# JuliaDiffusionBayes/ExtensibleMCMC.jl

Measured on NVIDIA B200. Metric: chain-steps x obs/sec, higher is better.
Workload: dtype f64

## Files before the change

extensiblemcmc.jl_b200/csrc/api.cu:

```cuda
#include <dlfcn.h>
#include <nccl.h>

#include <algorithm>
#include <cmath>
#include <cstdio>
#include <cstdlib>
#include <cstring>
#include <map>
#include <string>
#include <vector>

#include <cuda_runtime.h>

#include "../../include/extmcmc.h"
#include "dev_state.cuh"
#include "block_kernels.h"
#include "step_kernels.h"
#include "sweep.h"
#include "user_law.h"

using namespace extmcmc;

namespace {

std::string g_create_error;

struct NcclApi {
    void *lib = nullptr;
    ncclResult_t (*GetUniqueId)(ncclUniqueId *) = nullptr;
    ncclResult_t (*CommInitRank)(ncclComm_t *, int, ncclUniqueId, int) = nullptr;
    ncclResult_t (*AllReduce)(const void *, void *, size_t, ncclDataType_t, ncclRedOp_t, ncclComm_t,
                              cudaStream_t) = nullptr;
    ncclResult_t (*CommDestroy)(ncclComm_t) = nullptr;
    const char *(*GetErrorString)(ncclResult_t) = nullptr;
    bool load(std::string &err) {
        if (lib) return true;
        lib = dlopen("libnccl.so.2", RTLD_NOW | RTLD_GLOBAL);
        if (!lib) lib = dlopen("libnccl.so", RTLD_NOW | RTLD_GLOBAL);
        if (!lib) { err = std::string("cannot load libnccl: ") + dlerror(); return false; }
        GetUniqueId = (decltype(GetUniqueId))dlsym(lib, "ncclGetUniqueId");
        CommInitRank = (decltype(CommInitRank))dlsym(lib, "ncclCommInitRank");
        AllReduce = (decltype(AllReduce))dlsym(lib, "ncclAllReduce");
        CommDestroy = (decltype(CommDestroy))dlsym(lib, "ncclCommDestroy");
        GetErrorString = (decltype(GetErrorString))dlsym(lib, "ncclGetErrorString");
        if (!GetUniqueId || !CommInitRank || !AllReduce || !CommDestroy) {
            err = "libnccl lacks required symbols";
            return false;
        }
        return true;
    }
} g_nccl;

struct Slot {
    StepDesc *h_descs = nullptr;
    StepDesc *d_descs = nullptr;
    int cap = 0;
    cudaEvent_t done = nullptr;
    bool in_flight = false;
};

}

struct extmcmc_handle {
    extmcmc_config_t cfg{};
    int num_sms = 0;
    size_t l2_bytes = 0;
    cudaStream_t stream = nullptr;
    std::string err;
    DevState d{};
    std::vector<DevUpdate> upd_host;
    std::vector<bool> upd_set;
    bool upd_dirty = true;
    double *obs_dev = nullptr;
    int64_t n_obs_local = 0;
    int64_t n_obs_largest = 0;
    int64_t *goff_dev = nullptr, *glen_dev = nullptr;
    double *y_dev = nullptr;
    UserLaw ulaw;
    int logi_D = 0;
    unsigned int *tail_counter = nullptr;
    bool tail = false;
    bool grad_valid = false;
    bool dcache = false, dc_valid = false;
    double *dsum_buf[2] = {nullptr, nullptr};
    bool any_mala = false;
    bool state_set = false;
    SweepPlan plan{};
    bool plan_valid = false;
    Slot slot[2];
    int next_slot = 0;
    std::map<long long, cudaGraphExec_t> graphs;
    std::map<long long, int64_t> graph_launches;
    int64_t seq_next = 0;
    std::vector<int64_t> ra_iter;
    std::vector<int64_t> acc_tag;
    std::vector<int64_t> haario_M;
    std::vector<double> lambda;
    std::vector<extmcmc_lambda_fn> lambda_fn;
    std::vector<void *> lambda_user;
    int64_t xseq_next = 0;
    bool blk_planned = false;
    bool res_ok = false, obsblk_ok = false;
    TeamPlan res_plan{};
    ObsBlockPlan obsblk_plan{};
    unsigned long long *blk_go = nullptr;
    unsigned int *blk_counter = nullptr;
    unsigned int *team_sync = nullptr;
    long long *team_prof = nullptr;
    size_t team_sync_cap = 0;
    double *rp_prop = nullptr, *rp_exp = nullptr;
    size_t rp_prop_cap = 0, rp_exp_cap = 0;
    std::vector<std::pair<cudaEvent_t, cudaEvent_t>> ev_pending, ev_free;
    float sweep_ms = 0.f;
    int64_t sweep_launches = 0;
    cudaEvent_t t0 = nullptr, t1 = nullptr;
    std::vector<cudaEvent_t> ev_pool;
    int64_t launches = 0;
    double *flush_buf = nullptr;
    int64_t flush_n = 0;
    double *scratch_ll = nullptr;
    double *gsum = nullptr;
    cudaStream_t copy_stream = nullptr;
    cudaEvent_t fetch_ready = nullptr, fetch_done = nullptr;
    unsigned char *stage = nullptr;
    size_t stage_cap = 0;
    int64_t fetch_lo = 0, fetch_hi = 0;
    bool fetch_active = false;
    void *p2p_region = nullptr;
    std::vector<void *> p2p_opened;
    ncclComm_t comm = nullptr;
    int64_t *n_obs_dev = nullptr;
    bool n_total_known = false;
    std::vector<void *> allocs;
};

namespace {

#define CK(h, call)                                                                      \
    do {                                                                                 \
        cudaError_t e_ = (call);                                                         \
        if (e_ != cudaSuccess) {                                                         \
            (h)->err = std::string(#call) + ": " + cudaGetErrorString(e_);               \
            return e_ == cudaErrorMemoryAllocation ? EXTMCMC_EOOM : EXTMCMC_ECUDA;       \
        }                                                                                \
    } while (0)

#define NK(h, call)                                                                      \
    do {                                                                                 \
        ncclResult_t r_ = (call);                                                        \
        if (r_ != ncclSuccess) {                                                         \
            (h)->err = std::string(#call) + ": " +                                       \
                       (g_nccl.GetErrorString ? g_nccl.GetErrorString(r_) : "nccl error"); \
            return EXTMCMC_ENCCL;                                                        \
        }                                                                                \
    } while (0)

int32_t fail(extmcmc_t h, int32_t code, const std::string &msg) {
    if (h) h->err = msg; else g_create_error = msg;
    return code;
}

template <typename T>
int32_t dev_alloc(extmcmc_t h, T **out, size_t n) {
    void *p = nullptr;
    cudaError_t e = cudaMalloc(&p, std::max<size_t>(n, 1) * sizeof(T));
    if (e != cudaSuccess) {
        h->err = std::string("cudaMalloc: ") + cudaGetErrorString(e);
        return EXTMCMC_EOOM;
    }
    h->allocs.push_back(p);
    *out = (T *)p;
    return EXTMCMC_OK;
}

void invalidate_graphs(extmcmc_t h) {
    for (auto &kv : h->graphs) cudaGraphExecDestroy(kv.second);
    h->graphs.clear();
    h->graph_launches.clear();
}

bool obs_sharded(extmcmc_t h) {
    return h->cfg.shard_mode == EXTMCMC_SHARD_OBS && h->cfg.world_size > 1;
}

int32_t ensure_plan(extmcmc_t h) {
    if (h->plan_valid) return EXTMCMC_OK;
    if (h->cfg.law == EXTMCMC_LAW_GSN_IID_1D || h->cfg.law == EXTMCMC_LAW_HIER_NORMAL)
        h->plan = plan_sweep_gsn1d(h->d.C, h->n_obs_largest, h->cfg.sweep_variant, h->num_sms, h->d.G);
    else if (h->cfg.law == EXTMCMC_LAW_GSN_MV)
        h->plan = plan_sweep_gsnmv(h->cfg.obs_dim, h->d.C, h->n_obs_local, h->cfg.sweep_variant, h->num_sms);
    else if (h->cfg.law == EXTMCMC_LAW_LOGISTIC)
        h->plan = plan_sweep_logistic(h->cfg.obs_dim, h->d.C, h->n_obs_local, h->num_sms);
    else if (h->cfg.law == EXTMCMC_LAW_USER) {
        if (!h->ulaw.loaded) return fail(h, EXTMCMC_EINVAL, "no user law: call extmcmc_set_user_law first");
        h->plan = plan_sweep_user(h->ulaw, h->d.C, h->n_obs_local, h->cfg.sweep_variant, h->num_sms);
    } else
        return fail(h, EXTMCMC_EUNSUPPORTED, "law not implemented on the GPU path");
    h->d.S = h->plan.S;
    h->tail = h->cfg.law == EXTMCMC_LAW_GSN_IID_1D && h->plan.variant == SWEEP_VARIANT_OBS;
    if (const char *e = getenv("EXTMCMC_TAIL")) h->tail = h->tail && atoi(e) != 0;
    if (h->tail && !h->tail_counter) {
        int32_t rct = dev_alloc(h, &h->tail_counter, 1);
        if (rct) return rct;
        CK(h, cudaMemset(h->tail_counter, 0, sizeof(unsigned int)));
    }
    h->d.use_ssum = (obs_sharded(h) || law_self_finished(h->cfg.law) || h->tail) ? 1 : 0;
    size_t part_rows = law_self_finished(h->cfg.law) ? (size_t)h->plan.S * (h->cfg.n_params + 1)
                                                     : (size_t)2 * h->d.G * h->plan.S;
    part_rows = std::max(part_rows, (size_t)h->num_sms * 3);
    part_rows = std::max(part_rows, (size_t)2 * h->d.G * 4);
    int32_t rc = dev_alloc(h, &h->d.partial, part_rows * h->d.C);
    if (rc) return rc;
    if (obs_sharded(h) && !h->gsum &&
        (h->cfg.law == EXTMCMC_LAW_GSN_IID_1D || h->cfg.law == EXTMCMC_LAW_HIER_NORMAL))
        if ((rc = dev_alloc(h, &h->gsum, (size_t)2 * h->d.G * h->d.C))) return rc;
    {
        const char *e = getenv("EXTMCMC_DATA_CACHE");
        const bool on = !e || atoi(e) != 0;
        h->dcache = on && h->cfg.law == EXTMCMC_LAW_HIER_NORMAL && !obs_sharded(h) && h->d.G <= kDataCacheMaxG;
        if (h->dcache && !h->dsum_buf[0])
            if ((rc = dev_alloc(h, &h->dsum_buf[0], (size_t)2 * h->d.G * h->d.C)) ||
                (rc = dev_alloc(h, &h->dsum_buf[1], (size_t)2 * h->d.G * h->d.C)))
                return rc;
        h->d.dsum_cur = h->dcache ? h->dsum_buf[0] : nullptr;
        h->d.dsum_prop = h->dcache ? h->dsum_buf[1] : nullptr;
        h->dc_valid = false;
    }
    h->plan_valid = true;
    h->blk_planned = false;
    invalidate_graphs(h);
    return EXTMCMC_OK;
}

constexpr int kDataFree = 0x100;
int step_kind(extmcmc_t h, int u) {
    const DevUpdate &t = h->upd_host[u];
    int kind = t.kernel;
    if (h->dcache && kind != EXTMCMC_KERNEL_MALA && t.n_coords <= kMaxCoords) {
        bool moves_data = false;
        for (int i = 0; i < t.n_coords; ++i) moves_data = moves_data || t.coords[i] < h->d.G;
        if (!moves_data) kind |= kDataFree;
    }
    return kind;
}
inline bool kind_is_mala(int kind) { return (kind & 0xff) == EXTMCMC_KERNEL_MALA; }
int step_advance(bool dcache, int kind, bool &gv, bool &dc) {
    if (kind_is_mala(kind)) {
        const int mode = gv ? 0 : (dc ? 2 : 1);
        if (mode == 1 && dcache) dc = true;
        gv = true;
        return mode;
    }
    gv = false;
    if (kind & kDataFree) {
        const int mode = dc ? 1 : 2;
        dc = true;
        return mode;
    }
    dc = false;
    return 0;
}

int32_t plan_block_kernels(extmcmc_t h) {
    if (h->blk_planned) return EXTMCMC_OK;
    h->blk_planned = true;
    h->res_ok = h->obsblk_ok = false;
    const int sv = h->cfg.sweep_variant;
    if (sv != 0 && sv != 3 && sv != 4) return EXTMCMC_OK;
    if (const char *e = getenv("EXTMCMC_BLOCK_KERNELS")) if (atoi(e) == 0) return EXTMCMC_OK;
    const bool gsn1d = h->cfg.law == EXTMCMC_LAW_GSN_IID_1D || h->cfg.law == EXTMCMC_LAW_HIER_NORMAL;
    if (!gsn1d || h->d.n_haario > 0) return EXTMCMC_OK;
    bool all_unif = true, all_unif_or_mala = true;
    for (int u = 0; u < h->cfg.n_updates; ++u) {
        const int kk = h->upd_host[u].kernel;
        if (kk != EXTMCMC_KERNEL_RW_UNIFORM) all_unif = false;
        if (kk != EXTMCMC_KERNEL_RW_UNIFORM && kk != EXTMCMC_KERNEL_MALA) all_unif_or_mala = false;
    }
    if (all_unif_or_mala && !obs_sharded(h) && sv == 3) {
        h->res_ok = plan_team(h->d, h->upd_host.data(), h->num_sms, true, &h->res_plan);
        if (h->res_ok && getenv("EXTMCMC_TEAM_PROF") && !h->team_prof) {
            int32_t rc = dev_alloc(h, &h->team_prof, (size_t)h->res_plan.n_cta * 8);
            if (rc) return rc;
            CK(h, cudaMemset(h->team_prof, 0, sizeof(long long) * h->res_plan.n_cta * 8));
        }
        if (h->res_ok) {
            const size_t words = team_sync_words(h->res_plan);
            if (words > h->team_sync_cap) {
                int32_t rc = dev_alloc(h, &h->team_sync, words);
                if (rc) return rc;
                h->team_sync_cap = words;
            }
        }
    }
    const bool obs_auto = false;
    if (!h->res_ok && all_unif && h->cfg.law == EXTMCMC_LAW_GSN_IID_1D && h->d.C <= 32 && (sv == 4 || obs_auto) &&
        (!obs_sharded(h) || h->d.p2p)) {
        cudaError_t e = plan_obs_block(h->d, h->upd_host.data(), h->num_sms, h->n_obs_local, &h->obsblk_plan);
        if (e == cudaSuccess) {
            if (!h->blk_go) {
                int32_t rc;
                if ((rc = dev_alloc(h, &h->blk_go, 1)) || (rc = dev_alloc(h, &h->blk_counter, 1))) return rc;
                CK(h, cudaMemset(h->blk_go, 0, sizeof(unsigned long long)));
                CK(h, cudaMemset(h->blk_counter, 0, sizeof(unsigned int)));
            }
            h->obsblk_ok = true;
        } else {
            cudaGetLastError();
        }
    }
    return EXTMCMC_OK;
}

int32_t upload_updates(extmcmc_t h) {
    if (!h->upd_dirty) return EXTMCMC_OK;
    CK(h, cudaMemcpyAsync(h->d.upd, h->upd_host.data(), sizeof(DevUpdate) * h->upd_host.size(),
                          cudaMemcpyHostToDevice, h->stream));
    CK(h, cudaStreamSynchronize(h->stream));
    h->upd_dirty = false;
    return EXTMCMC_OK;
}

int32_t ensure_total_obs(extmcmc_t h) {
    if (h->n_total_known) return EXTMCMC_OK;
    if (h->cfg.shard_mode == EXTMCMC_SHARD_OBS && h->cfg.world_size > 1) {
        if (!h->comm) return fail(h, EXTMCMC_EINVAL, "EXTMCMC_SHARD_OBS needs extmcmc_comm_init first");
        int64_t n = h->n_obs_local;
        CK(h, cudaMemcpyAsync(h->n_obs_dev, &n, sizeof n, cudaMemcpyHostToDevice, h->stream));
        NK(h, g_nccl.AllReduce(h->n_obs_dev, h->n_obs_dev, 1, ncclInt64, ncclSum, h->comm, h->stream));
        CK(h, cudaMemcpyAsync(&n, h->n_obs_dev, sizeof n, cudaMemcpyDeviceToHost, h->stream));
        CK(h, cudaStreamSynchronize(h->stream));
        h->d.n_obs_total = n;
    } else {
        h->d.n_obs_total = h->n_obs_local;
    }
    h->n_total_known = true;
    invalidate_graphs(h);
    return EXTMCMC_OK;
}

int32_t enqueue_sweep(extmcmc_t h, bool instrument, bool grad = false, const double *src = nullptr,
                      double *ll_dst = nullptr, double *grad_dst = nullptr,
                      const StepDesc *d_descs = nullptr, int k = 0) {
    std::pair<cudaEvent_t, cudaEvent_t> ev{nullptr, nullptr};
    bool tail_done = false;
    if (instrument) {
        if (!h->ev_free.empty()) { ev = h->ev_free.back(); h->ev_free.pop_back(); }
        else { CK(h, cudaEventCreate(&ev.first)); CK(h, cudaEventCreate(&ev.second)); }
        CK(h, cudaEventRecord(ev.first, h->stream));
    }
    if (h->cfg.law == EXTMCMC_LAW_GSN_IID_1D || h->cfg.law == EXTMCMC_LAW_HIER_NORMAL) {
        Gsn1dArgs a{};
        a.obs = h->obs_dev; a.goff = h->goff_dev; a.glen = h->glen_dev; a.G = h->d.G;
        a.mu = h->cfg.law == EXTMCMC_LAW_HIER_NORMAL ? src : h->d.lawc;
        if (!a.mu) return fail(h, EXTMCMC_EINVAL, "internal: sweep without a source state");
        a.C = h->d.C; a.partial = h->d.partial; a.S = h->plan.S;
        tail_done = h->tail && !grad;
        if (tail_done) {
            const bool push = obs_sharded(h) && h->d.p2p && d_descs;
            a.tail_mode = push ? 2 : 1;
            a.tail_counter = h->tail_counter; a.ssum = h->d.ssum;
            a.peer_rx = h->d.peer_rx;
            a.rank = h->cfg.rank; a.world = h->cfg.world_size;
            a.descs = d_descs; a.k = k;
        }
        static const bool hint_on = [] { const char *e = getenv("EXTMCMC_L2_HINT"); return !e || atoi(e) != 0; }();
        a.stream_hint = hint_on && (size_t)h->n_obs_local * sizeof(double) > h->l2_bytes / 2 ? 1 : 0;
        launch_sweep_gsn1d(h->plan, a, grad, h->stream);
    } else if (h->cfg.law == EXTMCMC_LAW_LOGISTIC) {
        LogisticArgs a{h->obs_dev, h->y_dev, h->n_obs_local, src, h->cfg.obs_dim, h->d.C, h->d.partial,
                       h->d.partial + (size_t)h->plan.S * h->d.C, h->plan.S, h->plan.n_cta};
        launch_sweep_logistic(h->plan, a, ll_dst, grad_dst, h->stream);
        if (obs_sharded(h)) {
            NK(h, g_nccl.AllReduce(ll_dst, ll_dst, (size_t)h->d.C, ncclFloat64, ncclSum, h->comm, h->stream));
            if (grad_dst)
                NK(h, g_nccl.AllReduce(grad_dst, grad_dst, (size_t)h->cfg.obs_dim * h->d.C, ncclFloat64, ncclSum,
                                       h->comm, h->stream));
        }
        h->launches += h->plan.launches;
        if (instrument) {
            CK(h, cudaEventRecord(ev.second, h->stream));
            h->ev_pending.push_back(ev);
        }
        return EXTMCMC_OK;
    } else if (h->cfg.law == EXTMCMC_LAW_USER) {
        UserSweepArgs a{};
        a.obs = h->obs_dev; a.n_obs = h->n_obs_local; a.theta = src; a.C = h->d.C;
        a.ll_part = h->d.partial; a.g_part = h->d.partial + (size_t)h->plan.S * h->d.C;
        a.err_flag = h->d.err_flag; a.S = h->plan.S;
        CK(h, launch_sweep_user(h->plan, h->ulaw, a, grad, ll_dst, grad_dst, h->stream));
        h->launches += h->plan.launches;
        if (instrument) {
            CK(h, cudaEventRecord(ev.second, h->stream));
            h->ev_pending.push_back(ev);
        }
        return EXTMCMC_OK;
    } else {
        launch_sweep_gsnmv(h->plan, h->obs_dev, h->n_obs_local, h->d.lawc, h->d.C, h->d.partial, h->stream);
    }
    h->launches += h->plan.launches;
    if (instrument) {
        CK(h, cudaEventRecord(ev.second, h->stream));
        h->ev_pending.push_back(ev);
    }
    if (obs_sharded(h) && grad) {
        launch_reduce_group_sums(h->d, h->gsum, h->stream);
        h->launches += 1;
        NK(h, g_nccl.AllReduce(h->gsum, h->gsum, (size_t)2 * h->d.G * h->d.C, ncclFloat64, ncclSum, h->comm,
                               h->stream));
    } else if (obs_sharded(h)) {
        if (h->d.p2p && d_descs) {
            if (!tail_done) { launch_reduce_push(h->d, d_descs, k, h->stream); h->launches += 1; }
        } else {
            if (!tail_done) { launch_reduce_partials(h->d, h->stream); h->launches += 1; }
            NK(h, g_nccl.AllReduce(h->d.ssum, h->d.ssum, (size_t)h->d.C, ncclFloat64, ncclSum, h->comm,
                                   h->stream));
        }
    }
    return EXTMCMC_OK;
}

DevState grad_view(extmcmc_t h) {
    DevState v = h->d;
    if (obs_sharded(h) && !law_self_finished(h->cfg.law)) { v.partial = h->gsum; v.S = 1; }
    return v;
}

int32_t enqueue_steps(extmcmc_t h, const StepDesc *d_descs, const int *kinds, int n_steps,
                      bool instrument, bool &grad_valid, bool &dc_valid) {
    bool fused = false;
    bool cur_prepared = false;
    for (int k = 0; k < n_steps; ++k) {
        int32_t rc;
        const int dflags = step_deferral_flags(h->d, k, n_steps);
        const bool next_mala = k + 1 < n_steps && kind_is_mala(kinds[k + 1]);
        const bool next_rw = k + 1 < n_steps && !kind_is_mala(kinds[k + 1]);
        const int mode = step_advance(h->dcache, kinds[k], grad_valid, dc_valid);
        if (kind_is_mala(kinds[k])) {
            const bool logi = law_self_finished(h->cfg.law);
            int finalize_cur = 0;
            DevState gv = grad_view(h);
            if (mode == 1) {
                if (logi) {
                    if ((rc = enqueue_sweep(h, instrument, true, h->d.theta, h->scratch_ll, h->d.grad_cur))) return rc;
                } else {
                    const bool hier = h->cfg.law == EXTMCMC_LAW_HIER_NORMAL;
                    if (!cur_prepared && !hier) { launch_prepare_current(h->d, h->stream); h->launches += 1; }
                    if ((rc = enqueue_sweep(h, instrument, true, h->d.theta))) return rc;
                    finalize_cur = 1;
                }
            } else if (mode == 2) {
                gv.partial = h->d.dsum_cur; gv.S = 1;
                finalize_cur = 2;
            }
            launch_mala_propose(gv, d_descs, k, finalize_cur, h->scratch_ll, dflags, h->stream);
            gv = grad_view(h);
            if (logi) {
                if ((rc = enqueue_sweep(h, instrument, true, h->d.prop_full, h->d.ll_prop, h->d.grad_prop))) return rc;
            } else {
                if ((rc = enqueue_sweep(h, instrument, true, h->d.prop_full))) return rc;
            }
            fused = next_rw;
            launch_mala_accept(gv, d_descs, k, logi ? 0 : 1, fused ? 1 : 0, dflags, h->stream);
            h->launches += 2;
            cur_prepared = false;
        } else {
            if (!fused) { launch_propose(h->d, d_descs, k, h->stream); h->launches += 1; }
            const bool from_cache = mode != 0;
            if (mode == 2) {
                if ((rc = enqueue_sweep(h, instrument, true, h->d.theta))) return rc;
                launch_reduce_group_sums(h->d, h->d.dsum_cur, h->stream);
                h->launches += 1;
            }
            if (!from_cache)
                if ((rc = enqueue_sweep(h, instrument, false, h->d.prop_full, h->d.ssum, nullptr, d_descs, k))) return rc;
            fused = next_rw;
            cur_prepared = next_mala && !law_self_finished(h->cfg.law) && h->cfg.law != EXTMCMC_LAW_HIER_NORMAL;
            launch_accept(h->d, d_descs, k, fused ? 1 : (cur_prepared ? 2 : 0), dflags, h->stream, from_cache);
            h->launches += 1;
        }
    }
    CK(h, cudaGetLastError());
    return EXTMCMC_OK;
}

int32_t collect_events(extmcmc_t h) {
    for (auto &ev : h->ev_pending) {
        float ms = 0.f;
        CK(h, cudaEventElapsedTime(&ms, ev.first, ev.second));
        h->sweep_ms += ms;
        h->sweep_launches += 1;
        h->ev_free.push_back(ev);
    }
    h->ev_pending.clear();
    return EXTMCMC_OK;
}

int32_t run_block_impl(extmcmc_t h, const extmcmc_step_t *steps, int32_t n_steps, int rng_mode,
                       int32_t p_u_max, const double *proposals, const double *exp_draws) {
    if (!h) return EXTMCMC_EINVAL;
    if (n_steps < 0 || (n_steps > 0 && !steps)) return fail(h, EXTMCMC_EINVAL, "bad steps");
    if (n_steps == 0) return EXTMCMC_OK;
    if (!h->obs_dev) return fail(h, EXTMCMC_EINVAL, "no observations uploaded");
    if (!h->state_set) return fail(h, EXTMCMC_EINVAL, "extmcmc_set_state not called");
    for (int u = 0; u < h->cfg.n_updates; ++u)
        if (!h->upd_set[u]) return fail(h, EXTMCMC_EINVAL, "update " + std::to_string(u) + " not set");
    if (n_steps > h->cfg.history_window)
        return fail(h, EXTMCMC_EINVAL, "block longer than history_window");
    if (obs_sharded(h) && !h->comm) return fail(h, EXTMCMC_EINVAL, "EXTMCMC_SHARD_OBS needs extmcmc_comm_init first");
    if (h->cfg.law == EXTMCMC_LAW_USER && h->any_mala && h->ulaw.loaded && !h->ulaw.grad)
        return fail(h, EXTMCMC_EUNSUPPORTED, "MALA needs a user law with logpdf_grad (extmcmc_set_user_law with_grad = 1)");
    for (int s = 0; s < n_steps; ++s)
        if (steps[s].pidx < 0 || steps[s].pidx >= h->cfg.n_updates || steps[s].mcmciter < 1)
            return fail(h, EXTMCMC_EINVAL, "step out of range");
    CK(h, cudaSetDevice(h->cfg.device));
    int32_t rc;
    if ((rc = ensure_plan(h))) return rc;
    if ((rc = upload_updates(h))) return rc;
    if ((rc = ensure_total_obs(h))) return rc;
    if ((rc = plan_block_kernels(h))) return rc;
    if ((h->res_ok || h->obsblk_ok) && h->dcache) {
        h->dcache = h->dc_valid = false;
        h->d.dsum_cur = h->d.dsum_prop = nullptr;
    }
    if (h->fetch_active && h->seq_next + n_steps - h->d.H > h->fetch_lo)
        CK(h, cudaStreamWaitEvent(h->stream, h->fetch_done, 0));

    if (h->d.rng_mode != rng_mode) { h->d.rng_mode = rng_mode; invalidate_graphs(h); }
    if (rng_mode == EXTMCMC_RNG_REPLAY) {
        if (!proposals || !exp_draws || p_u_max < 1) return fail(h, EXTMCMC_EINVAL, "replay buffers missing");
        for (int s = 0; s < n_steps; ++s)
            if (h->upd_host[steps[s].pidx].n_coords > p_u_max)
                return fail(h, EXTMCMC_EINVAL, "p_u_max smaller than an update's n_coords");
        const size_t np = (size_t)n_steps * p_u_max * h->d.C, ne = (size_t)n_steps * h->d.C;
        CK(h, cudaStreamSynchronize(h->stream));
        if (np > h->rp_prop_cap) {
            if (h->rp_prop) cudaFree(h->rp_prop);
            CK(h, cudaMalloc(&h->rp_prop, np * sizeof(double)));
            h->rp_prop_cap = np;
        }
        if (ne > h->rp_exp_cap) {
            if (h->rp_exp) cudaFree(h->rp_exp);
            CK(h, cudaMalloc(&h->rp_exp, ne * sizeof(double)));
            h->rp_exp_cap = ne;
        }
        CK(h, cudaMemcpy(h->rp_prop, proposals, np * sizeof(double), cudaMemcpyHostToDevice));
        CK(h, cudaMemcpy(h->rp_exp, exp_draws, ne * sizeof(double), cudaMemcpyHostToDevice));
        h->d.rp_prop = h->rp_prop;
        h->d.rp_exp = h->rp_exp;
        h->d.p_u_max = p_u_max;
    }

    const int si = h->next_slot;
    Slot &sl = h->slot[si];
    h->next_slot ^= 1;
    if (sl.in_flight) { CK(h, cudaEventSynchronize(sl.done)); sl.in_flight = false; }
    if (sl.cap < n_steps) {
        if (sl.h_descs) cudaFreeHost(sl.h_descs);
        if (sl.d_descs) cudaFree(sl.d_descs);
        for (auto it = h->graphs.begin(); it != h->graphs.end();) {
            if ((it->first & 1) == si) { cudaGraphExecDestroy(it->second); it = h->graphs.erase(it); }
            else ++it;
        }
        const int cap = std::max(n_steps, 64);
        CK(h, cudaMallocHost(&sl.h_descs, sizeof(StepDesc) * cap));
        CK(h, cudaMalloc(&sl.d_descs, sizeof(StepDesc) * cap));
        sl.cap = cap;
    }
    const int W = h->d.W;
    int n_sweeps = 0;
    {
        bool gv = h->grad_valid, dc = h->dc_valid;
        for (int s = 0; s < n_steps; ++s) {
            StepDesc &sd = sl.h_descs[s];
            const int u = steps[s].pidx;
            const int64_t it = steps[s].mcmciter;
            sd.mcmciter = it;
            sd.seq = h->seq_next + s;
            sd.stat_n = sd.seq + 1;
            sd.xseq = h->xseq_next + s;
            sd.pidx = u;
            sd.first = steps[s].prev_pidx < 0 ? 1 : 0;
            const int64_t prev_it = it - 1 > 1 ? it - 1 : 1;
            sd.ra_prev_valid = (h->ra_iter[u] == prev_it && prev_it != it) ? 1 : 0;
            int64_t &tag = h->acc_tag[(size_t)u * W + (size_t)(it % W)];
            sd.acc_out_valid = (it > W && tag == it - W) ? 1 : 0;
            sd.replay_row = s;
            sd.haario_ready = 0;
            sd.lambda = h->lambda[u];
            sd.pad_ = 0;
            if (h->upd_host[u].adapt_kind == EXTMCMC_ADAPT_HAARIO) {
                if (++h->haario_M[u] >= h->upd_host[u].adapt_every_k) {
                    sd.haario_ready = 1;
                    h->haario_M[u] = 0;
                    if (h->lambda_fn[u]) h->lambda[u] = h->lambda_fn[u](h->lambda[u], sd.stat_n + 1, it, h->lambda_user[u]);
                }
            }
            const bool mala = h->upd_host[u].kernel == EXTMCMC_KERNEL_MALA;
            sd.need_cur_grad = (mala && !gv) ? 1 : 0;
            const int mode = step_advance(h->dcache, step_kind(h, u), gv, dc);
            n_sweeps += mala ? 1 + (mode == 1 ? 1 : 0) : (mode == 1 ? 0 : 1);
            h->ra_iter[u] = it;
            tag = it;
        }
    }

    std::vector<int> kinds(n_steps);
    unsigned long long hash = 1469598103934665603ull;
    for (int s = 0; s < n_steps; ++s) {
        kinds[s] = step_kind(h, steps[s].pidx);
        hash = (hash ^ (unsigned long long)kinds[s]) * 1099511628211ull;
    }
    hash = (hash ^ (unsigned long long)((h->grad_valid ? 7 : 3) + (h->dc_valid ? 16 : 0))) * 1099511628211ull;
    hash = (hash ^ (unsigned long long)n_steps) * 1099511628211ull;
    const bool instrument = h->cfg.instrument != 0;
    const bool use_graph = h->cfg.use_graphs && !instrument && rng_mode == EXTMCMC_RNG_PHILOX;
    if (h->res_ok || h->obsblk_ok) {
        CK(h, cudaMemcpyAsync(sl.d_descs, sl.h_descs, sizeof(StepDesc) * n_steps, cudaMemcpyHostToDevice, h->stream));
        std::pair<cudaEvent_t, cudaEvent_t> ev{nullptr, nullptr};
        if (instrument) {
            if (!h->ev_free.empty()) { ev = h->ev_free.back(); h->ev_free.pop_back(); }
            else { CK(h, cudaEventCreate(&ev.first)); CK(h, cudaEventCreate(&ev.second)); }
        }
        if (h->res_ok) {
            TeamArgs a{};
            a.d = h->d;
            a.d.dsum_cur = a.d.dsum_prop = nullptr;
            a.d.S = h->res_plan.ts;
            a.descs = sl.d_descs; a.n_steps = n_steps; a.n_sweeps = n_sweeps;
            a.obs = h->obs_dev; a.goff = h->goff_dev; a.glen = h->glen_dev; a.G = h->d.G;
            a.ll_scratch = h->scratch_ll;
            a.sync = h->team_sync;
            a.prof = h->team_prof;
            CK(h, cudaMemsetAsync(h->team_sync, 0, team_sync_words(h->res_plan) * sizeof(unsigned int), h->stream));
            if (instrument) CK(h, cudaEventRecord(ev.first, h->stream));
            CK(h, launch_team_block(h->res_plan, a, h->stream));
            h->launches += 1;
        } else {
            ObsBlockArgs a{};
            a.d = h->d;
            a.d.dsum_cur = a.d.dsum_prop = nullptr;
            a.descs = sl.d_descs; a.n_steps = n_steps;
            a.obs = h->obs_dev; a.n_obs = h->n_obs_local;
            a.go = h->blk_go; a.counter = h->blk_counter;
            if (instrument) CK(h, cudaEventRecord(ev.first, h->stream));
            CK(h, launch_obs_block(h->obsblk_plan, a, h->stream));
            h->launches += 1;
        }
        if (instrument) {
            CK(h, cudaEventRecord(ev.second, h->stream));
            h->ev_pending.push_back(ev);
        }
        h->grad_valid = kind_is_mala(kinds[n_steps - 1]);
        h->dc_valid = false;
    } else if (!use_graph) {
        CK(h, cudaMemcpyAsync(sl.d_descs, sl.h_descs, sizeof(StepDesc) * n_steps,
                              cudaMemcpyHostToDevice, h->stream));
        if ((rc = enqueue_steps(h, sl.d_descs, kinds.data(), n_steps, instrument, h->grad_valid, h->dc_valid))) return rc;
    } else {
        const long long key = (long long)((hash << 1) | (unsigned long long)si);
        auto it = h->graphs.find(key);
        if (it == h->graphs.end()) {
            const int64_t launches_before = h->launches;
            bool gv = h->grad_valid, dc = h->dc_valid;
            cudaGraph_t g = nullptr;
            CK(h, cudaStreamBeginCapture(h->stream, cudaStreamCaptureModeThreadLocal));
            cudaError_t e1 = cudaMemcpyAsync(sl.d_descs, sl.h_descs, sizeof(StepDesc) * n_steps,
                                             cudaMemcpyHostToDevice, h->stream);
            int32_t rc2 = e1 == cudaSuccess ? enqueue_steps(h, sl.d_descs, kinds.data(), n_steps, false, gv, dc) : EXTMCMC_ECUDA;
            cudaError_t e2 = cudaStreamEndCapture(h->stream, &g);
            h->graph_launches[key] = h->launches - launches_before;
            h->launches = launches_before;
            if (rc2 || e2 != cudaSuccess || !g) {
                if (g) cudaGraphDestroy(g);
                return fail(h, EXTMCMC_ECUDA, "CUDA graph capture failed: " + h->err);
            }
            cudaGraphExec_t ge = nullptr;
            cudaError_t e3 = cudaGraphInstantiate(&ge, g, 0);
            cudaGraphDestroy(g);
            if (e3 != cudaSuccess)
                return fail(h, EXTMCMC_ECUDA, std::string("cudaGraphInstantiate: ") + cudaGetErrorString(e3));
            it = h->graphs.emplace(key, ge).first;
        }
        CK(h, cudaGraphLaunch(it->second, h->stream));
        h->launches += h->graph_launches[key];
        for (int s = 0; s < n_steps; ++s) step_advance(h->dcache, kinds[s], h->grad_valid, h->dc_valid);
    }
    CK(h, cudaEventRecord(sl.done, h->stream));
    sl.in_flight = true;
    h->seq_next += n_steps;
    h->xseq_next += n_steps;
    return EXTMCMC_OK;
}

}

extern "C" {

int32_t extmcmc_abi_version(void) { return EXTMCMC_ABI_VERSION; }

const char *extmcmc_last_error(extmcmc_t h) { return h ? h->err.c_str() : g_create_error.c_str(); }

int32_t extmcmc_create(const extmcmc_config_t *cfg, extmcmc_t *out) {
    if (!cfg || !out) return fail(nullptr, EXTMCMC_EINVAL, "null argument");
    *out = nullptr;
    if (cfg->abi_version != EXTMCMC_ABI_VERSION) return fail(nullptr, EXTMCMC_EINVAL, "ABI version mismatch");
    if (cfg->n_chains < 1 || cfg->n_params < 1 || cfg->n_updates < 1 || cfg->history_window < 1)
        return fail(nullptr, EXTMCMC_EINVAL, "n_chains, n_params, n_updates, history_window must be >= 1");
    if (cfg->n_updates > 65535) return fail(nullptr, EXTMCMC_EINVAL, "n_updates must be < 65536");
    switch (cfg->law) {
    case EXTMCMC_LAW_GSN_IID_1D:
        if (cfg->obs_dim != 1 || cfg->n_params != 2)
            return fail(nullptr, EXTMCMC_EINVAL, "GSN_IID_1D needs obs_dim = 1, n_params = 2");
        break;
    case EXTMCMC_LAW_GSN_MV:
        if (cfg->obs_dim < 2 || cfg->obs_dim > kMaxObsDim)
            return fail(nullptr, EXTMCMC_EUNSUPPORTED, "GSN_MV on the GPU path needs 2 <= obs_dim <= 16 (d = 1: GSN_IID_1D)");
        if (cfg->n_params != cfg->obs_dim * (cfg->obs_dim + 1))
            return fail(nullptr, EXTMCMC_EINVAL, "GSN_MV needs n_params = d (d + 1)");
        break;
    case EXTMCMC_LAW_LOGISTIC:
        if (cfg->obs_dim != cfg->n_params || cfg->obs_dim < 1 || logistic_padded_dim(cfg->obs_dim) == 0)
            return fail(nullptr, EXTMCMC_EUNSUPPORTED, "LOGISTIC needs obs_dim = n_params = d with 1 <= d <= 256");
        break;
    case EXTMCMC_LAW_HIER_NORMAL:
        if (cfg->obs_dim != 1 || cfg->n_params < 3)
            return fail(nullptr, EXTMCMC_EINVAL, "HIER_NORMAL needs obs_dim = 1 and n_params = G + 2 >= 3");
        break;
    case EXTMCMC_LAW_USER:
        if (cfg->obs_dim < 1 || cfg->obs_dim > kUserMaxObsDim || cfg->n_params > kUserMaxParams)
            return fail(nullptr, EXTMCMC_EUNSUPPORTED, "USER needs 1 <= obs_dim <= 64 and 1 <= n_params <= 64");
        if (cfg->shard_mode == EXTMCMC_SHARD_OBS && cfg->world_size > 1)
            return fail(nullptr, EXTMCMC_EUNSUPPORTED, "user laws are not implemented under EXTMCMC_SHARD_OBS with several ranks");
        break;
    default:
        return fail(nullptr, EXTMCMC_EUNSUPPORTED, "target law not implemented on the GPU path");
    }
    if (cfg->stats_mode < 0 || cfg->stats_mode > 2) return fail(nullptr, EXTMCMC_EINVAL, "bad stats_mode");
    int ndev = 0;
    cudaError_t e = cudaGetDeviceCount(&ndev);
    if (e != cudaSuccess || ndev == 0)
        return fail(nullptr, EXTMCMC_ECUDA,
                    std::string("no CUDA device: ") + (e != cudaSuccess ? cudaGetErrorString(e) : "count = 0"));
    if (cfg->device < 0 || cfg->device >= ndev) return fail(nullptr, EXTMCMC_EINVAL, "bad device ordinal");

    extmcmc_handle *h = new extmcmc_handle();
    h->cfg = *cfg;
    auto bail = [&](int32_t rc) { g_create_error = h->err; extmcmc_destroy(h); return rc; };
#define CKC(call)                                                                        \
    do {                                                                                 \
        cudaError_t e_ = (call);                                                         \
        if (e_ != cudaSuccess) {                                                         \
            h->err = std::string(#call) + ": " + cudaGetErrorString(e_);                 \
            return bail(e_ == cudaErrorMemoryAllocation ? EXTMCMC_EOOM : EXTMCMC_ECUDA); \
        }                                                                                \
    } while (0)
    CKC(cudaSetDevice(cfg->device));
    cudaDeviceProp prop;
    CKC(cudaGetDeviceProperties(&prop, cfg->device));
    if (prop.major != 10) {
        h->err = "libextmcmc_cuda is built for sm_100a (B200) only; found sm_" +
                 std::to_string(prop.major) + std::to_string(prop.minor);
        return bail(EXTMCMC_EUNSUPPORTED);
    }
    h->num_sms = prop.multiProcessorCount;
    h->l2_bytes = (size_t)prop.l2CacheSize;
    CKC(cudaStreamCreateWithFlags(&h->stream, cudaStreamNonBlocking));
    CKC(cudaStreamCreateWithFlags(&h->copy_stream, cudaStreamNonBlocking));
    CKC(cudaEventCreateWithFlags(&h->fetch_ready, cudaEventDisableTiming));
    CKC(cudaEventCreateWithFlags(&h->fetch_done, cudaEventDisableTiming));
    CKC(cudaEventCreate(&h->t0));
    CKC(cudaEventCreate(&h->t1));
    for (auto &sl : h->slot) CKC(cudaEventCreateWithFlags(&sl.done, cudaEventDisableTiming));
    CKC(sweep_gsn1d_init());
    CKC(sweep_logistic_init());
    h->logi_D = cfg->law == EXTMCMC_LAW_LOGISTIC ? logistic_padded_dim(cfg->obs_dim) : 0;

    DevState &d = h->d;
    const int64_t C = cfg->n_chains;
    const int p = cfg->n_params, NU = cfg->n_updates;
    d.C = C; d.gC = C; d.g0 = 0; d.chain_offset = cfg->chain_offset; d.p = p; d.NU = NU;
    d.W = cfg->roll_window > 0 ? cfg->roll_window : 100;
    d.H = cfg->history_window;
    d.law = cfg->law; d.stats_mode = cfg->stats_mode; d.rng_mode = EXTMCMC_RNG_PHILOX;
    d.p_u_max = 1; d.seed = cfg->seed;
    d.obs_dim = cfg->obs_dim;
    d.G = cfg->law == EXTMCMC_LAW_HIER_NORMAL ? cfg->n_params - 2 : 1;
    d.lawc_k = cfg->law == EXTMCMC_LAW_GSN_IID_1D ? 3
             : law_self_finished(cfg->law) ? 1
             : cfg->law == EXTMCMC_LAW_HIER_NORMAL ? d.G
             : cfg->obs_dim + cfg->obs_dim * (cfg->obs_dim + 1) / 2 + 1;
    d.use_ssum = ((cfg->shard_mode == EXTMCMC_SHARD_OBS && cfg->world_size > 1) ||
                  law_self_finished(cfg->law)) ? 1 : 0;
    int32_t rc = 0;
    const size_t covn = cfg->stats_mode == 0 ? (size_t)p * p : (cfg->stats_mode == 1 ? (size_t)p : 0);
    if ((rc = dev_alloc(h, &d.theta, (size_t)p * C)) || (rc = dev_alloc(h, &d.ll, (size_t)C)) ||
        (rc = dev_alloc(h, &d.prop_loc, (size_t)kMaxCoords * C)) ||
        (rc = dev_alloc(h, &d.prop_full, (size_t)p * C)) ||
        (rc = dev_alloc(h, &d.lawc, (size_t)d.lawc_k * C)) ||
        (rc = dev_alloc(h, &d.n_used, (size_t)C)) || (rc = dev_alloc(h, &d.ssum, (size_t)C)) ||
        (rc = dev_alloc(h, &d.ll_prop, (size_t)C)) || (rc = dev_alloc(h, &d.grad_cur, (size_t)p * C)) ||
        (rc = dev_alloc(h, &d.grad_prop, (size_t)p * C)) ||
        (rc = dev_alloc(h, &h->goff_dev, (size_t)d.G)) || (rc = dev_alloc(h, &h->glen_dev, (size_t)d.G)) ||
        (rc = dev_alloc(h, &d.mean, (size_t)p * C)) || (rc = dev_alloc(h, &d.cov, covn * C)) ||
        (rc = dev_alloc(h, &d.h_theta, (size_t)d.H * p * C)) ||
        (rc = dev_alloc(h, &d.h_prop, (size_t)d.H * p * C)) ||
        (rc = dev_alloc(h, &d.h_ll, (size_t)d.H * C)) || (rc = dev_alloc(h, &d.h_llp, (size_t)d.H * C)) ||
        (rc = dev_alloc(h, &d.h_acc, (size_t)d.H * C)) || (rc = dev_alloc(h, &d.err_flag, 1)) ||
        (rc = dev_alloc(h, &d.upd, (size_t)NU)) || (rc = dev_alloc(h, &h->scratch_ll, (size_t)C)) ||
        (rc = dev_alloc(h, &h->n_obs_dev, 1)))
        return bail(rc);
    CKC(cudaMemset(d.err_flag, 0, sizeof(int32_t)));
    h->upd_host.assign(NU, DevUpdate{});
    h->upd_set.assign(NU, false);
    h->ra_iter.assign(NU, 0);
    h->acc_tag.assign((size_t)NU * d.W, 0);
    h->haario_M.assign(NU, 0);
    h->lambda.assign(NU, 0.0);
    h->lambda_fn.assign(NU, nullptr);
    h->lambda_user.assign(NU, nullptr);
    if (cfg->law == EXTMCMC_LAW_GSN_MV && (rc = dev_alloc(h, &d.mv_L, (size_t)cfg->obs_dim * cfg->obs_dim * C)))
        return bail(rc);
    {
        const char *e = getenv("EXTMCMC_P2P_TIMEOUT_MS");
        const double ms = e ? atof(e) : 30000.0;
        d.p2p_timeout_ns = (unsigned long long)((ms > 1.0 ? ms : 1.0) * 1e6);
    }
    *out = h;
    return EXTMCMC_OK;
#undef CKC
}

int32_t extmcmc_destroy(extmcmc_t h) {
    if (!h) return EXTMCMC_OK;
    cudaSetDevice(h->cfg.device);
    if (h->stream) cudaStreamSynchronize(h->stream);
    if (h->team_prof) {
        const int n = h->res_plan.n_cta;
        std::vector<long long> pr((size_t)n * 8);
        if (cudaMemcpy(pr.data(), h->team_prof, pr.size() * sizeof(long long), cudaMemcpyDeviceToHost) == cudaSuccess) {
            double s[7] = {0, 0, 0, 0, 0, 0, 0}, runs = 0, mx = 0, mn = 1e300;
            for (int b = 0; b < n; ++b) {
                double tot = 0;
                for (int i = 0; i < 7; ++i) { s[i] += (double)pr[(size_t)b * 8 + i]; tot += (double)pr[(size_t)b * 8 + i]; }
                runs += (double)pr[(size_t)b * 8 + 7];
                if (pr[(size_t)b * 8 + 7]) { const double t = tot / pr[(size_t)b * 8 + 7]; mx = std::max(mx, t); mn = std::min(mn, t); }
            }
            if (runs > 0)
                fprintf(stderr, "[extmcmc team kernel] cycles per launch per CTA: sweep %.0f, barrier-before %.0f, barrier-after %.0f, "
                                "propose %.0f, accept %.0f, cov+sync %.0f, ctx %.0f; total min %.0f max %.0f over CTAs; %d CTAs, ts %d, stages %d\n",
                        s[0] / runs, s[1] / runs, s[2] / runs, s[3] / runs, s[4] / runs, s[5] / runs, s[6] / runs, mn, mx, n,
                        h->res_plan.ts, h->res_plan.stages);
        }
    }
    invalidate_graphs(h);
    if (h->comm && g_nccl.CommDestroy) g_nccl.CommDestroy(h->comm);
    for (void *p : h->p2p_opened) cudaIpcCloseMemHandle(p);
    if (h->p2p_region) cudaFree(h->p2p_region);
    for (void *p : h->allocs) cudaFree(p);
    if (h->obs_dev) cudaFree(h->obs_dev);
    if (h->y_dev) cudaFree(h->y_dev);
    user_law_unload(h->ulaw);
    if (h->rp_prop) cudaFree(h->rp_prop);
    if (h->rp_exp) cudaFree(h->rp_exp);
    if (h->flush_buf) cudaFree(h->flush_buf);
    for (auto &sl : h->slot) {
        if (sl.h_descs) cudaFreeHost(sl.h_descs);
        if (sl.d_descs) cudaFree(sl.d_descs);
        if (sl.done) cudaEventDestroy(sl.done);
    }
    for (auto &ev : h->ev_pending) { cudaEventDestroy(ev.first); cudaEventDestroy(ev.second); }
    for (auto &ev : h->ev_free) { cudaEventDestroy(ev.first); cudaEventDestroy(ev.second); }
    if (h->t0) cudaEventDestroy(h->t0);
    if (h->t1) cudaEventDestroy(h->t1);
    for (cudaEvent_t e : h->ev_pool) if (e) cudaEventDestroy(e);
    if (h->copy_stream) { cudaStreamSynchronize(h->copy_stream); cudaStreamDestroy(h->copy_stream); }
    if (h->fetch_ready) cudaEventDestroy(h->fetch_ready);
    if (h->fetch_done) cudaEventDestroy(h->fetch_done);
    if (h->stage) cudaFreeHost(h->stage);
    if (h->stream) cudaStreamDestroy(h->stream);
    delete h;
    return EXTMCMC_OK;
}

static int32_t install_obs(extmcmc_t h, int64_t n_obs, const std::vector<int64_t> &glen) {
    if (h->obs_dev) { cudaFree(h->obs_dev); h->obs_dev = nullptr; }
    const int G = (int)glen.size();
    std::vector<int64_t> goff(G);
    int64_t tot = 0, largest = 0;
    for (int g = 0; g < G; ++g) {
        goff[g] = tot;
        tot += (glen[g] * h->cfg.obs_dim + 1) & ~(int64_t)1;
        largest = std::max(largest, glen[g]);
    }
    const size_t padded = (size_t)tot + 2;
    CK(h, cudaMalloc(&h->obs_dev, padded * sizeof(double)));
    CK(h, cudaMemsetAsync(h->obs_dev, 0, padded * sizeof(double), h->stream));
    CK(h, cudaMemcpyAsync(h->goff_dev, goff.data(), sizeof(int64_t) * G, cudaMemcpyHostToDevice, h->stream));
    CK(h, cudaMemcpyAsync(h->glen_dev, glen.data(), sizeof(int64_t) * G, cudaMemcpyHostToDevice, h->stream));
    CK(h, cudaStreamSynchronize(h->stream));
    h->n_obs_local = n_obs;
    h->n_obs_largest = largest;
    h->plan_valid = false;
    h->n_total_known = false;
    h->grad_valid = false;
    h->dc_valid = false;
    return EXTMCMC_OK;
}

int32_t extmcmc_upload_obs(extmcmc_t h, const double *obs, int64_t n_obs, int32_t obs_dim,
                           const double *y) {
    if (!h) return EXTMCMC_EINVAL;
    if (!obs || n_obs < 1) return fail(h, EXTMCMC_EINVAL, "need at least one observation");
    if (obs_dim != h->cfg.obs_dim) return fail(h, EXTMCMC_EINVAL, "obs_dim differs from the configuration");
    CK(h, cudaSetDevice(h->cfg.device));
    CK(h, cudaStreamSynchronize(h->stream));
    if (h->cfg.law == EXTMCMC_LAW_LOGISTIC) {
        if (!y) return fail(h, EXTMCMC_EINVAL, "LOGISTIC needs the responses y");
        const int D = h->logi_D;
        const size_t n_pad = ((size_t)n_obs + 15) & ~(size_t)15;
        if (h->obs_dev) { cudaFree(h->obs_dev); h->obs_dev = nullptr; }
        if (h->y_dev) { cudaFree(h->y_dev); h->y_dev = nullptr; }
        CK(h, cudaMalloc(&h->obs_dev, n_pad * D * sizeof(double)));
        CK(h, cudaMalloc(&h->y_dev, n_pad * sizeof(double)));
        CK(h, cudaMemsetAsync(h->obs_dev, 0, n_pad * D * sizeof(double), h->stream));
        CK(h, cudaMemsetAsync(h->y_dev, 0, n_pad * sizeof(double), h->stream));
        CK(h, cudaMemcpy2DAsync(h->obs_dev, (size_t)D * 8, obs, (size_t)obs_dim * 8, (size_t)obs_dim * 8,
                                (size_t)n_obs, cudaMemcpyHostToDevice, h->stream));
        CK(h, cudaMemcpyAsync(h->y_dev, y, (size_t)n_obs * sizeof(double), cudaMemcpyHostToDevice, h->stream));
        CK(h, cudaStreamSynchronize(h->stream));
        h->n_obs_local = n_obs;
        h->n_obs_largest = n_obs;
        h->plan_valid = false;
        h->n_total_known = false;
        h->grad_valid = false;
        h->dc_valid = false;
        return EXTMCMC_OK;
    }
    if (h->cfg.law == EXTMCMC_LAW_USER) {
        if (y) return fail(h, EXTMCMC_EINVAL, "USER takes no y: responses and covariates are columns of the rows");
        const size_t n_pad = ((size_t)n_obs + 1) & ~(size_t)1, nd = (size_t)n_obs * obs_dim;
        if (h->obs_dev) { cudaFree(h->obs_dev); h->obs_dev = nullptr; }
        CK(h, cudaMalloc(&h->obs_dev, n_pad * obs_dim * sizeof(double)));
        CK(h, cudaMemsetAsync(h->obs_dev, 0, n_pad * obs_dim * sizeof(double), h->stream));
        CK(h, cudaMemcpyAsync(h->obs_dev, obs, nd * sizeof(double), cudaMemcpyHostToDevice, h->stream));
        CK(h, cudaStreamSynchronize(h->stream));
        h->n_obs_local = n_obs;
        h->n_obs_largest = n_obs;
        h->plan_valid = false;
        h->n_total_known = false;
        h->grad_valid = false;
        h->dc_valid = false;
        return EXTMCMC_OK;
    }
    std::vector<int64_t> glen(h->d.G, 0);
    if (h->cfg.law == EXTMCMC_LAW_HIER_NORMAL) {
        if (!y) return fail(h, EXTMCMC_EINVAL, "HIER_NORMAL needs the group index of every observation in y");
        int64_t prev = 0;
        for (int64_t i = 0; i < n_obs; ++i) {
            const int64_t g = (int64_t)y[i];
            if (g < prev || g >= h->d.G || (double)g != y[i])
                return fail(h, EXTMCMC_EINVAL, "group indices must be integers in [0, G), sorted ascending");
            prev = g;
            ++glen[g];
        }
    } else {
        glen[0] = n_obs;
    }
    int32_t rc = install_obs(h, n_obs, glen);
    if (rc) return rc;
    int64_t src = 0, dst = 0;
    for (int g = 0; g < h->d.G; ++g) {
        const int64_t nd = glen[g] * obs_dim;
        if (nd) CK(h, cudaMemcpyAsync(h->obs_dev + dst, obs + src, (size_t)nd * sizeof(double), cudaMemcpyHostToDevice, h->stream));
        src += nd;
        dst += (nd + 1) & ~(int64_t)1;
    }
    CK(h, cudaStreamSynchronize(h->stream));
    return EXTMCMC_OK;
}

int32_t extmcmc_generate_obs_normal(extmcmc_t h, int64_t first, int64_t n_obs, double mean, double sd,
                                    uint64_t seed) {
    if (!h) return EXTMCMC_EINVAL;
    if (n_obs < 1 || first < 0 || !(sd > 0.0)) return fail(h, EXTMCMC_EINVAL, "bad generate_obs arguments");
    if (h->cfg.law != EXTMCMC_LAW_GSN_IID_1D) return fail(h, EXTMCMC_EUNSUPPORTED, "generate_obs_normal needs the GSN_IID_1D law");
    CK(h, cudaSetDevice(h->cfg.device));
    CK(h, cudaStreamSynchronize(h->stream));
    int32_t rc = install_obs(h, n_obs, std::vector<int64_t>{n_obs});
    if (rc) return rc;
    launch_generate_obs_normal(h->obs_dev, first, n_obs, mean, sd, seed, h->num_sms, h->stream);
    h->launches += 1;
    CK(h, cudaGetLastError());
    CK(h, cudaStreamSynchronize(h->stream));
    return EXTMCMC_OK;
}

static int32_t ensure_gw_scratch(extmcmc_t h, int n) {
    if (n <= h->d.gw_n) return EXTMCMC_OK;
    CK(h, cudaStreamSynchronize(h->stream));
    double *p = nullptr;
    int32_t rc = dev_alloc(h, &p, (size_t)3 * n * h->d.C);
    if (rc) return rc;
    h->d.gw = p;
    h->d.gw_n = n;
    invalidate_graphs(h);
    return EXTMCMC_OK;
}

int32_t extmcmc_set_update(extmcmc_t h, int32_t u, const extmcmc_update_t *upd) {
    if (!h || !upd) return EXTMCMC_EINVAL;
    if (u < 0 || u >= h->cfg.n_updates) return fail(h, EXTMCMC_EINVAL, "update index out of range");
    const bool gauss = upd->kernel == EXTMCMC_KERNEL_RW_GAUSS || upd->kernel == EXTMCMC_KERNEL_RW_GAUSS_MIX;
    const bool mala = upd->kernel == EXTMCMC_KERNEL_MALA;
    const bool mix = upd->kernel == EXTMCMC_KERNEL_RW_GAUSS_MIX;
    const bool haario = upd->adapt.kind == EXTMCMC_ADAPT_HAARIO;
    if (upd->kernel != EXTMCMC_KERNEL_RW_UNIFORM && !gauss && !mala)
        return fail(h, EXTMCMC_EUNSUPPORTED, "transition kernel not implemented on the GPU path");
    if (mala) {
        if (h->cfg.law != EXTMCMC_LAW_GSN_IID_1D && h->cfg.law != EXTMCMC_LAW_HIER_NORMAL &&
            h->cfg.law != EXTMCMC_LAW_LOGISTIC && h->cfg.law != EXTMCMC_LAW_USER)
            return fail(h, EXTMCMC_EUNSUPPORTED, "MALA needs a law with a device gradient (GSN_IID_1D, HIER_NORMAL, LOGISTIC, USER)");
        if (h->cfg.law == EXTMCMC_LAW_USER && h->ulaw.loaded && !h->ulaw.grad)
            return fail(h, EXTMCMC_EUNSUPPORTED, "MALA needs a user law with logpdf_grad (extmcmc_set_user_law with_grad = 1)");
        if (upd->prior != EXTMCMC_PRIOR_IMPROPER && upd->prior != EXTMCMC_PRIOR_NORMAL)
            return fail(h, EXTMCMC_EUNSUPPORTED, "MALA supports ImproperPrior and Normal priors only");
        if (upd->pos)
            for (int i = 0; i < upd->n_coords; ++i)
                if (upd->pos[i]) return fail(h, EXTMCMC_EUNSUPPORTED, "MALA on positivity-constrained coordinates is not implemented");
    }
    if (upd->prior < EXTMCMC_PRIOR_IMPROPER || upd->prior > EXTMCMC_PRIOR_MVNORMAL)
        return fail(h, EXTMCMC_EUNSUPPORTED, "prior not implemented on the GPU path");
    if (upd->n_coords < 1 || upd->n_coords > (mala ? std::min(h->cfg.n_params, 32768) : kMaxCoords))
        return fail(h, EXTMCMC_EUNSUPPORTED, mala ? "1 <= n_coords <= min(n_params, 32768) for MALA"
                                                  : "1 <= n_coords <= 32 for random-walk updates on the GPU path");
    if (!upd->coords || !upd->step) return fail(h, EXTMCMC_EINVAL, "coords/step missing");
    const int nc = upd->n_coords, nn = nc * nc;
    if (upd->prior == EXTMCMC_PRIOR_PRODUCT) {
        if (upd->n_prior_params < 1 || !upd->prior_params) return fail(h, EXTMCMC_EINVAL, "ProductPrior parameters missing");
        const int K = (int)upd->prior_params[0];
        if (K < 1 || K > kMaxPriorFactors || upd->n_prior_params != 1 + 4 * K)
            return fail(h, EXTMCMC_EUNSUPPORTED, "ProductPrior: 1 <= factors <= 16");
        int tot = 0;
        for (int k = 0; k < K; ++k) {
            const int kind = (int)upd->prior_params[1 + 4 * k], dim = (int)upd->prior_params[2 + 4 * k];
            if (kind < EXTMCMC_PRIOR_IMPROPER || kind > EXTMCMC_PRIOR_CAUCHY || kind == EXTMCMC_PRIOR_PRODUCT || dim < 1)
                return fail(h, EXTMCMC_EUNSUPPORTED, "ProductPrior factor not implemented on the GPU path");
            tot += dim;
        }
        if (tot != nc) return fail(h, EXTMCMC_EINVAL, "ProductPrior dims must add up to length(coords)");
    } else if (upd->prior == EXTMCMC_PRIOR_MVNORMAL) {
        if (upd->n_prior_params != nc + nn || !upd->prior_params)
            return fail(h, EXTMCMC_EINVAL, "MvNormal prior needs {mu[p_u], L[p_u * p_u]}");
        for (int i = 0; i < nc; ++i)
            if (!(upd->prior_params[nc + i + i * nc] > 0.0))
                return fail(h, EXTMCMC_EINVAL, "MvNormal prior: the Cholesky factor must have a positive diagonal");
    } else {
        if (upd->n_prior_params > kMaxPriorParams || (upd->n_prior_params > 0 && !upd->prior_params))
            return fail(h, EXTMCMC_EINVAL, "bad prior parameters");
        const int pk = upd->prior;
        const int need = (pk == EXTMCMC_PRIOR_IMPROPER || pk == EXTMCMC_PRIOR_IMPROPER_POS) ? 0
                       : pk == EXTMCMC_PRIOR_EXPONENTIAL ? 1 : 2;
        if (upd->n_prior_params < need) return fail(h, EXTMCMC_EINVAL, "prior parameters missing");
    }
    if (!(upd->adapt.kind == EXTMCMC_ADAPT_NONE ||
          (upd->adapt.kind == EXTMCMC_ADAPT_MALA && mala) ||
          (upd->adapt.kind == EXTMCMC_ADAPT_UNIF_RW && upd->kernel == EXTMCMC_KERNEL_RW_UNIFORM) ||
          (upd->adapt.kind == EXTMCMC_ADAPT_HAARIO && mix)))
        return fail(h, EXTMCMC_EUNSUPPORTED, "adaptation not implemented for this transition kernel");
    if (upd->adapt.kind != EXTMCMC_ADAPT_NONE && upd->adapt.adapt_every_k_steps < 1)
        return fail(h, EXTMCMC_EINVAL, "adapt_every_k_steps must be >= 1");
    for (int i = 0; i < nc; ++i) {
        if (upd->coords[i] < 0 || upd->coords[i] >= h->cfg.n_params)
            return fail(h, EXTMCMC_EINVAL, "coordinate out of range");
        if (!gauss && !mala && !(upd->step[i] > 0.0))
            return fail(h, EXTMCMC_EINVAL, "eps must be > 0");
    }
    if (mix && !(upd->step[2 * nn] >= 0.0 && upd->step[2 * nn] <= 1.0))
        return fail(h, EXTMCMC_EINVAL, "lambda must be in [0, 1]");
    if (mala && !(upd->step[0] > 0.0)) return fail(h, EXTMCMC_EINVAL, "MALA step tau must be > 0");
    const bool fresh = !h->upd_set[u];
    {
        const DevUpdate &cur = h->upd_host[u];
        if (!fresh && cur.n_coords != nc) return fail(h, EXTMCMC_EINVAL, "cannot change n_coords of an update");
        if (!fresh && ((mix && !cur.sigB) || (gauss && !cur.sigA) || (haario && !cur.hmean) ||
                       (upd->prior == EXTMCMC_PRIOR_MVNORMAL && !cur.prior_dev)))
            return fail(h, EXTMCMC_EINVAL, "cannot change the kernel or prior family of an update");
    }

    CK(h, cudaSetDevice(h->cfg.device));
    const int64_t C = h->d.C;
    const int W = h->d.W;
    DevUpdate t = h->upd_host[u];
    t.kernel = upd->kernel; t.n_coords = nc; t.prior = upd->prior;
    t.adapt_kind = upd->adapt.kind;
    for (int i = 0; i < nc && i < kMaxCoords; ++i) {
        t.coords[i] = upd->coords[i];
        t.pos[i] = upd->pos ? upd->pos[i] : 0;
    }
    const bool mvn = upd->prior == EXTMCMC_PRIOR_MVNORMAL;
    for (int i = 0; i < kMaxPriorParams; ++i)
        t.prior_params[i] = (!mvn && i < upd->n_prior_params) ? upd->prior_params[i] : 0.0;
    t.adapt_every_k = upd->adapt.adapt_every_k_steps;
    t.target = upd->adapt.target_accpt_rate; t.scale = upd->adapt.scale;
    t.vmin = upd->adapt.min; t.vmax = upd->adapt.max; t.offset = upd->adapt.offset;
    int32_t rc = 0;
    if (fresh) {
        double *pd = nullptr;
        if ((rc = dev_alloc(h, &t.coords_dev, (size_t)nc)) ||
            (rc = dev_alloc(h, &t.eps, (size_t)nc * C)) ||
            (rc = dev_alloc(h, &t.adapt_prop, (size_t)C)) || (rc = dev_alloc(h, &t.adapt_acc, (size_t)C)) ||
            (rc = dev_alloc(h, &t.tot_prop, (size_t)C)) || (rc = dev_alloc(h, &t.tot_acc, (size_t)C)) ||
            (rc = dev_alloc(h, &t.ra_val, (size_t)C)) || (rc = dev_alloc(h, &t.acc_ring, (size_t)W * C)))
            return rc;
        if (gauss && ((rc = dev_alloc(h, &t.sigA, (size_t)nn)) || (rc = dev_alloc(h, &t.LA, (size_t)nn)))) return rc;
        if (mix && ((rc = dev_alloc(h, &t.sigB, (size_t)nn * C)) || (rc = dev_alloc(h, &t.LB, (size_t)nn * C)))) return rc;
        if (haario && ((rc = dev_alloc(h, &t.hmean, (size_t)nc * C)) || (rc = dev_alloc(h, &t.hcov, (size_t)nn * C)))) return rc;
        if (mvn) { if ((rc = dev_alloc(h, &pd, (size_t)(nc + nn)))) return rc; t.prior_dev = pd; }
    }
    if ((gauss || haario || mvn) && (rc = ensure_gw_scratch(h, nc))) return rc;
    CK(h, cudaStreamSynchronize(h->stream));
    CK(h, cudaMemcpy(t.coords_dev, upd->coords, sizeof(int32_t) * nc, cudaMemcpyHostToDevice));
    if (mvn) CK(h, cudaMemcpy(const_cast<double *>(t.prior_dev), upd->prior_params, sizeof(double) * (nc + nn), cudaMemcpyHostToDevice));
    if (mala) {
        std::vector<double> tau0((size_t)C, upd->step[0]);
        CK(h, cudaMemcpy(t.eps, tau0.data(), tau0.size() * sizeof(double), cudaMemcpyHostToDevice));
    } else if (!gauss) {
        std::vector<double> eps0((size_t)nc * C);
        for (int i = 0; i < nc; ++i) std::fill_n(eps0.begin() + (size_t)i * C, C, upd->step[i]);
        CK(h, cudaMemcpy(t.eps, eps0.data(), eps0.size() * sizeof(double), cudaMemcpyHostToDevice));
    } else {
        CK(h, cudaMemcpy(t.sigA, upd->step, sizeof(double) * nn, cudaMemcpyHostToDevice));
        launch_chol_factor(t.sigA, t.LA, nc, 1, 1, h->stream);
        if (mix) {
            std::vector<double> sb((size_t)nn * C);
            for (int k = 0; k < nn; ++k) std::fill_n(sb.begin() + (size_t)k * C, C, upd->step[nn + k]);
            CK(h, cudaMemcpy(t.sigB, sb.data(), sb.size() * sizeof(double), cudaMemcpyHostToDevice));
            launch_chol_factor(t.sigB, t.LB, nc, C, C, h->stream);
        }
        CK(h, cudaGetLastError());
        CK(h, cudaStreamSynchronize(h->stream));
        if (haario) {
            CK(h, cudaMemset(t.hmean, 0, sizeof(double) * nc * C));
            CK(h, cudaMemset(t.hcov, 0, sizeof(double) * nn * C));
        }
    }
    CK(h, cudaMemset(t.adapt_prop, 0, sizeof(int32_t) * C));
    CK(h, cudaMemset(t.adapt_acc, 0, sizeof(int32_t) * C));
    CK(h, cudaMemset(t.tot_prop, 0, sizeof(int64_t) * C));
    CK(h, cudaMemset(t.tot_acc, 0, sizeof(int64_t) * C));
    CK(h, cudaMemset(t.ra_val, 0, sizeof(double) * C));
    CK(h, cudaMemset(t.acc_ring, 0, (size_t)W * C));
    h->upd_host[u] = t;
    h->lambda[u] = mix ? upd->step[2 * nn] : 0.0;
    h->haario_M[u] = 0;
    h->upd_set[u] = true;
    h->upd_dirty = true;
    h->blk_planned = false;
    int nh = 0;
    h->any_mala = false;
    for (int v = 0; v < h->cfg.n_updates; ++v) {
        if (h->upd_set[v] && h->upd_host[v].kernel == EXTMCMC_KERNEL_MALA) h->any_mala = true;
        if (h->upd_set[v] && h->upd_host[v].adapt_kind == EXTMCMC_ADAPT_HAARIO) ++nh;
    }
    if (nh != h->d.n_haario) { h->d.n_haario = nh; invalidate_graphs(h); }
    static const bool lean_on = [] { const char *e = getenv("EXTMCMC_LEAN"); return !e || atoi(e) != 0; }();
    int lean = lean_on ? 1 : 0;
    for (int v = 0; v < h->cfg.n_updates; ++v) {
        if (!h->upd_set[v]) continue;
        const DevUpdate &w = h->upd_host[v];
        if ((w.kernel != EXTMCMC_KERNEL_RW_UNIFORM && w.kernel != EXTMCMC_KERNEL_MALA) || !lean_prior(w.prior) ||
            w.adapt_kind == EXTMCMC_ADAPT_HAARIO)
            lean = 0;
    }
    if (lean != h->d.lean) { h->d.lean = lean; invalidate_graphs(h); }
    return EXTMCMC_OK;
}

int32_t extmcmc_set_seed(extmcmc_t h, uint64_t seed) {
    if (!h) return EXTMCMC_EINVAL;
    h->cfg.seed = seed;
    h->d.seed = seed;
    invalidate_graphs(h);
    return EXTMCMC_OK;
}

int32_t extmcmc_set_lambda_fn(extmcmc_t h, int32_t u, extmcmc_lambda_fn f, void *user) {
    if (!h) return EXTMCMC_EINVAL;
    if (u < 0 || u >= h->cfg.n_updates) return fail(h, EXTMCMC_EINVAL, "update index out of range");
    h->lambda_fn[u] = f;
    h->lambda_user[u] = user;
    return EXTMCMC_OK;
}

int32_t extmcmc_set_state(extmcmc_t h, const double *theta) {
    if (!h || !theta) return EXTMCMC_EINVAL;
    CK(h, cudaSetDevice(h->cfg.device));
    CK(h, cudaStreamSynchronize(h->stream));
    const DevState &d = h->d;
    const int64_t C = d.C;
    CK(h, cudaMemcpy(d.theta, theta, sizeof(double) * d.p * C, cudaMemcpyHostToDevice));
    std::vector<double> ninf((size_t)C, -INFINITY);
    CK(h, cudaMemcpy(d.ll, ninf.data(), sizeof(double) * C, cudaMemcpyHostToDevice));
    CK(h, cudaMemset(d.mean, 0, sizeof(double) * d.p * C));
    const size_t covn = d.stats_mode == 0 ? (size_t)d.p * d.p : (d.stats_mode == 1 ? (size_t)d.p : 0);
    if (covn) CK(h, cudaMemset(d.cov, 0, sizeof(double) * covn * C));
    CK(h, cudaMemset(d.err_flag, 0, sizeof(int32_t)));
    for (int u = 0; u < h->cfg.n_updates; ++u) {
        if (!h->upd_set[u]) continue;
        DevUpdate &t = h->upd_host[u];
        CK(h, cudaMemset(t.adapt_prop, 0, sizeof(int32_t) * C));
        CK(h, cudaMemset(t.adapt_acc, 0, sizeof(int32_t) * C));
        CK(h, cudaMemset(t.tot_prop, 0, sizeof(int64_t) * C));
        CK(h, cudaMemset(t.tot_acc, 0, sizeof(int64_t) * C));
        CK(h, cudaMemset(t.ra_val, 0, sizeof(double) * C));
        CK(h, cudaMemset(t.acc_ring, 0, (size_t)d.W * C));
        if (t.hmean) {
            CK(h, cudaMemset(t.hmean, 0, sizeof(double) * t.n_coords * C));
            CK(h, cudaMemset(t.hcov, 0, sizeof(double) * t.n_coords * t.n_coords * C));
        }
    }
    std::fill(h->haario_M.begin(), h->haario_M.end(), 0);
    h->seq_next = 0;
    h->grad_valid = false;
    h->dc_valid = false;
    if (h->fetch_active) { cudaEventSynchronize(h->fetch_done); h->fetch_active = false; }
    std::fill(h->ra_iter.begin(), h->ra_iter.end(), 0);
    std::fill(h->acc_tag.begin(), h->acc_tag.end(), 0);
    h->state_set = true;
    return EXTMCMC_OK;
}

int32_t extmcmc_user_law_check(const char *source, int32_t n_params, int32_t obs_dim, int32_t with_grad,
                               char *log, int64_t log_bytes) {
    if (log && log_bytes > 0) log[0] = 0;
    if (!source) return fail(nullptr, EXTMCMC_EINVAL, "null source");
    if (n_params < 1 || n_params > kUserMaxParams || obs_dim < 1 || obs_dim > kUserMaxObsDim)
        return fail(nullptr, EXTMCMC_EUNSUPPORTED, "user laws need 1 <= n_params <= 64 and 1 <= obs_dim <= 64");
    std::string lg, cubin;
    const int32_t rc = user_law_compile(source, n_params, obs_dim, with_grad != 0, lg, cubin, nullptr);
    if (log && log_bytes > 0) {
        const size_t n = std::min(lg.size(), (size_t)log_bytes - 1);
        std::memcpy(log, lg.data(), n);
        log[n] = 0;
    }
    if (rc) g_create_error = lg;
    return rc;
}

int32_t extmcmc_set_user_law(extmcmc_t h, const char *source, int32_t with_grad) {
    if (!h) return EXTMCMC_EINVAL;
    if (h->cfg.law != EXTMCMC_LAW_USER) return fail(h, EXTMCMC_EINVAL, "extmcmc_set_user_law needs a handle of law EXTMCMC_LAW_USER");
    if (!source) return fail(h, EXTMCMC_EINVAL, "null source");
    std::string log, cubin;
    uint64_t hash = 0;
    const int32_t rc = user_law_compile(source, h->cfg.n_params, h->cfg.obs_dim, with_grad != 0, log, cubin, &hash);
    if (rc == EXTMCMC_EINVAL) return fail(h, rc, "the user law does not compile:\n" + log);
    if (rc) return fail(h, rc, log);
    CK(h, cudaSetDevice(h->cfg.device));
    CK(h, cudaStreamSynchronize(h->stream));
    invalidate_graphs(h);
    const cudaError_t e = user_law_load(h->ulaw, cubin, h->cfg.n_params, h->cfg.obs_dim, with_grad != 0, hash);
    if (e != cudaSuccess) {
        user_law_unload(h->ulaw);
        return fail(h, EXTMCMC_ECUDA, std::string("loading the user law: ") + cudaGetErrorString(e));
    }
    h->plan_valid = false;
    h->grad_valid = false;
    return EXTMCMC_OK;
}

}
namespace {
struct CkptHeader {
    uint64_t magic;
    int64_t C, seq_next;
    int32_t abi, p, NU, W, stats_mode, law, grad_valid, pad;
};
constexpr uint64_t kCkptMagic = 0x32544b434d435845ull;

template <class F>
int32_t ckpt_walk(extmcmc_t h, F fn) {
    const DevState &d = h->d;
    const size_t C = (size_t)d.C, p = (size_t)d.p;
    const size_t covn = d.stats_mode == 0 ? p * p : (d.stats_mode == 1 ? p : 0);
    int32_t rc;
    if ((rc = fn(d.theta, nullptr, 8 * p * C)) || (rc = fn(d.ll, nullptr, 8 * C))) return rc;
    if (d.stats_mode != 2 && ((rc = fn(d.mean, nullptr, 8 * p * C)) || (rc = fn(d.cov, nullptr, 8 * covn * C)))) return rc;
    if ((rc = fn(nullptr, h->ra_iter.data(), 8 * h->ra_iter.size())) || (rc = fn(nullptr, h->acc_tag.data(), 8 * h->acc_tag.size())) ||
        (rc = fn(nullptr, h->haario_M.data(), 8 * h->haario_M.size())) || (rc = fn(nullptr, h->lambda.data(), 8 * h->lambda.size())))
        return rc;
    for (int u = 0; u < h->cfg.n_updates; ++u) {
        const DevUpdate &t = h->upd_host[u];
        const size_t n = (size_t)t.n_coords, nn = n * n;
        const size_t eps_rows = t.kernel == EXTMCMC_KERNEL_MALA ? 1 : n;
        if ((rc = fn(t.eps, nullptr, 8 * eps_rows * C)) || (rc = fn(t.adapt_prop, nullptr, 4 * C)) ||
            (rc = fn(t.adapt_acc, nullptr, 4 * C)) || (rc = fn(t.tot_prop, nullptr, 8 * C)) || (rc = fn(t.tot_acc, nullptr, 8 * C)) ||
            (rc = fn(t.ra_val, nullptr, 8 * C)) || (rc = fn(t.acc_ring, nullptr, (size_t)d.W * C)))
            return rc;
        if (t.sigB && ((rc = fn(t.sigB, nullptr, 8 * nn * C)) || (rc = fn(t.LB, nullptr, 8 * nn * C)))) return rc;
        if (t.hmean && ((rc = fn(t.hmean, nullptr, 8 * n * C)) || (rc = fn(t.hcov, nullptr, 8 * nn * C)))) return rc;
    }
    return EXTMCMC_OK;
}
}
extern "C" {

int32_t extmcmc_checkpoint_size(extmcmc_t h, int64_t *bytes_out) {
    if (!h || !bytes_out) return EXTMCMC_EINVAL;
    for (int u = 0; u < h->cfg.n_updates; ++u)
        if (!h->upd_set[u]) return fail(h, EXTMCMC_EINVAL, "update " + std::to_string(u) + " not set");
    if (h->cfg.law == EXTMCMC_LAW_USER && !h->ulaw.loaded) return fail(h, EXTMCMC_EINVAL, "no user law: call extmcmc_set_user_law first");
    size_t tot = sizeof(CkptHeader) + (h->cfg.law == EXTMCMC_LAW_USER ? sizeof(uint64_t) : 0);
    ckpt_walk(h, [&](void *, void *, size_t b) { tot += b; return EXTMCMC_OK; });
    *bytes_out = (int64_t)tot;
    return EXTMCMC_OK;
}

int32_t extmcmc_checkpoint_save(extmcmc_t h, void *blob, int64_t bytes) {
    int64_t need = 0;
    int32_t rc = extmcmc_checkpoint_size(h, &need);
    if (rc) return rc;
    if (!blob || bytes < need) return fail(h, EXTMCMC_EINVAL, "checkpoint buffer too small");
    if (!h->state_set) return fail(h, EXTMCMC_EINVAL, "nothing to save: extmcmc_set_state not called");
    CK(h, cudaSetDevice(h->cfg.device));
    CK(h, cudaStreamSynchronize(h->stream));
    CkptHeader hd{kCkptMagic, h->d.C, h->seq_next, EXTMCMC_ABI_VERSION, h->d.p, h->d.NU, h->d.W, h->d.stats_mode, h->d.law,
                  h->grad_valid ? 1 : 0, 0};
    char *out = (char *)blob;
    std::memcpy(out, &hd, sizeof hd);
    out += sizeof hd;
    if (h->cfg.law == EXTMCMC_LAW_USER) { std::memcpy(out, &h->ulaw.hash, sizeof(uint64_t)); out += sizeof(uint64_t); }
    return ckpt_walk(h, [&](void *dev, void *host, size_t b) -> int32_t {
        if (dev) { CK(h, cudaMemcpy(out, dev, b, cudaMemcpyDeviceToHost)); }
        else std::memcpy(out, host, b);
        out += b;
        return EXTMCMC_OK;
    });
}

int32_t extmcmc_checkpoint_load(extmcmc_t h, const void *blob, int64_t bytes) {
    int64_t need = 0;
    int32_t rc = extmcmc_checkpoint_size(h, &need);
    if (rc) return rc;
    if (!blob || bytes < need) return fail(h, EXTMCMC_EINVAL, "checkpoint blob too small for this configuration");
    CkptHeader hd;
    std::memcpy(&hd, blob, sizeof hd);
    if (hd.magic != kCkptMagic || hd.abi != EXTMCMC_ABI_VERSION || hd.C != h->d.C || hd.p != h->d.p || hd.NU != h->d.NU ||
        hd.W != h->d.W || hd.stats_mode != h->d.stats_mode || hd.law != h->d.law)
        return fail(h, EXTMCMC_EINVAL, "checkpoint does not match this handle (chains, parameters, updates, windows, law)");
    const char *in = (const char *)blob + sizeof hd;
    if (h->cfg.law == EXTMCMC_LAW_USER) {
        uint64_t hash;
        std::memcpy(&hash, in, sizeof hash);
        if (hash != h->ulaw.hash) return fail(h, EXTMCMC_EINVAL, "checkpoint was written under another user law");
        in += sizeof hash;
    }
    CK(h, cudaSetDevice(h->cfg.device));
    CK(h, cudaStreamSynchronize(h->stream));
    rc = ckpt_walk(h, [&](void *dev, void *host, size_t b) -> int32_t {
        if (dev) { CK(h, cudaMemcpy(dev, in, b, cudaMemcpyHostToDevice)); }
        else std::memcpy(host, in, b);
        in += b;
        return EXTMCMC_OK;
    });
    if (rc) return rc;
    h->seq_next = hd.seq_next;
    h->dc_valid = false;
    h->grad_valid = false;
    h->state_set = true;
    h->fetch_active = false;
    CK(h, cudaMemset(h->d.err_flag, 0, sizeof(int32_t)));
    return EXTMCMC_OK;
}

int32_t extmcmc_comm_unique_id(uint8_t id_out[128]) {
    std::string err;
    if (!id_out) return EXTMCMC_EINVAL;
    if (!g_nccl.load(err)) return fail(nullptr, EXTMCMC_ENCCL, err);
    ncclUniqueId id;
    static_assert(sizeof(ncclUniqueId) == 128, "ncclUniqueId is 128 bytes");
    if (g_nccl.GetUniqueId(&id) != ncclSuccess) return fail(nullptr, EXTMCMC_ENCCL, "ncclGetUniqueId failed");
    std::memcpy(id_out, &id, 128);
    return EXTMCMC_OK;
}

int32_t extmcmc_comm_init(extmcmc_t h, const uint8_t id_in[128]) {
    if (!h || !id_in) return EXTMCMC_EINVAL;
    if (h->comm) return fail(h, EXTMCMC_EINVAL, "communicator already initialised");
    if (!g_nccl.load(h->err)) return EXTMCMC_ENCCL;
    CK(h, cudaSetDevice(h->cfg.device));
    ncclUniqueId id;
    std::memcpy(&id, id_in, 128);
    NK(h, g_nccl.CommInitRank(&h->comm, h->cfg.world_size, id, h->cfg.rank));
    h->n_total_known = false;
    return EXTMCMC_OK;
}

static size_t p2p_region_bytes(extmcmc_t h) {
    const size_t W = (size_t)h->cfg.world_size;
    return 2 * W * (size_t)h->d.C * 2 * sizeof(unsigned long long);
}

int32_t extmcmc_p2p_export(extmcmc_t h, uint8_t handle_out[64]) {
    if (!h || !handle_out) return EXTMCMC_EINVAL;
    if (!obs_sharded(h)) return fail(h, EXTMCMC_EINVAL, "peer exchange is for EXTMCMC_SHARD_OBS with world_size > 1");
    if (h->cfg.law != EXTMCMC_LAW_GSN_IID_1D && h->cfg.law != EXTMCMC_LAW_GSN_MV)
        return fail(h, EXTMCMC_EUNSUPPORTED, "peer exchange is implemented for the Gaussian laws");
    static_assert(sizeof(cudaIpcMemHandle_t) == 64, "cudaIpcMemHandle_t is 64 bytes");
    CK(h, cudaSetDevice(h->cfg.device));
    if (!h->p2p_region) {
        CK(h, cudaMalloc(&h->p2p_region, p2p_region_bytes(h)));
        CK(h, cudaMemset(h->p2p_region, 0, p2p_region_bytes(h)));
    }
    cudaIpcMemHandle_t hd;
    CK(h, cudaIpcGetMemHandle(&hd, h->p2p_region));
    std::memcpy(handle_out, &hd, 64);
    return EXTMCMC_OK;
}

int32_t extmcmc_p2p_import(extmcmc_t h, const uint8_t *handles) {
    if (!h || !handles) return EXTMCMC_EINVAL;
    if (!h->p2p_region) return fail(h, EXTMCMC_EINVAL, "call extmcmc_p2p_export first");
    CK(h, cudaSetDevice(h->cfg.device));
    const int W = h->cfg.world_size;
    std::vector<unsigned long long *> rx(W);
    for (int q = 0; q < W; ++q) {
        void *base = nullptr;
        if (q == h->cfg.rank) {
            base = h->p2p_region;
        } else {
            cudaIpcMemHandle_t hd;
            std::memcpy(&hd, handles + 64 * (size_t)q, 64);
            CK(h, cudaIpcOpenMemHandle(&base, hd, cudaIpcMemLazyEnablePeerAccess));
            h->p2p_opened.push_back(base);
        }
        rx[q] = (unsigned long long *)base;
    }
    int32_t rc;
    if ((rc = dev_alloc(h, &h->d.peer_rx, (size_t)W))) return rc;
    CK(h, cudaMemcpy(h->d.peer_rx, rx.data(), sizeof(unsigned long long *) * W, cudaMemcpyHostToDevice));
    h->d.my_rx = rx[h->cfg.rank];
    h->d.rank = h->cfg.rank;
    h->d.world = W;
    h->d.p2p = 1;
    invalidate_graphs(h);
    return EXTMCMC_OK;
}

int32_t extmcmc_run_block(extmcmc_t h, const extmcmc_step_t *steps, int32_t n_steps) {
    return run_block_impl(h, steps, n_steps, EXTMCMC_RNG_PHILOX, 0, nullptr, nullptr);
}

int32_t extmcmc_run_block_replay(extmcmc_t h, const extmcmc_step_t *steps, int32_t n_steps,
                                 int32_t p_u_max, const double *proposals, const double *exp_draws) {
    return run_block_impl(h, steps, n_steps, EXTMCMC_RNG_REPLAY, p_u_max, proposals, exp_draws);
}

int32_t extmcmc_sync(extmcmc_t h) {
    if (!h) return EXTMCMC_EINVAL;
    CK(h, cudaSetDevice(h->cfg.device));
    CK(h, cudaStreamSynchronize(h->stream));
    int32_t rc = collect_events(h);
    if (rc) return rc;
    int32_t flag = 0;
    CK(h, cudaMemcpy(&flag, h->d.err_flag, sizeof flag, cudaMemcpyDeviceToHost));
    if (flag == 2)
        return fail(h, EXTMCMC_ENCCL, "peer exchange timed out: a rank did not deliver its partial sums; "
                                      "no step has been committed since (extmcmc_set_state to start over)");
    if (flag == 3)
        return fail(h, EXTMCMC_ECUDA, "a persistent block kernel timed out waiting for its own CTAs (EXTMCMC_P2P_TIMEOUT_MS); "
                                      "the chain state is undefined (extmcmc_set_state to start over)");
    if (flag) {
        CK(h, cudaMemset(h->d.err_flag, 0, sizeof flag));
        return fail(h, EXTMCMC_EDOMAIN,
                    "a chain proposed parameters outside the law's domain (e.g. variance <= 0); "
                    "the proposal was rejected");
    }
    return EXTMCMC_OK;
}

int32_t extmcmc_get_state(extmcmc_t h, double *theta, double *ll) {
    if (!h) return EXTMCMC_EINVAL;
    CK(h, cudaSetDevice(h->cfg.device));
    CK(h, cudaStreamSynchronize(h->stream));
    if (theta) CK(h, cudaMemcpy(theta, h->d.theta, sizeof(double) * h->d.p * h->d.C, cudaMemcpyDeviceToHost));
    if (ll) CK(h, cudaMemcpy(ll, h->d.ll, sizeof(double) * h->d.C, cudaMemcpyDeviceToHost));
    return EXTMCMC_OK;
}

int32_t extmcmc_get_history(extmcmc_t h, int64_t seq_lo, int64_t seq_hi, double *theta,
                            double *theta_prop, double *ll, double *ll_prop, uint8_t *accepted) {
    if (!h) return EXTMCMC_EINVAL;
    if (seq_lo < 0 || seq_hi < seq_lo || seq_hi > h->seq_next) return fail(h, EXTMCMC_EINVAL, "bad history range");
    if (seq_lo < h->seq_next - h->d.H) return fail(h, EXTMCMC_ESTALE, "history rows already overwritten");
    CK(h, cudaSetDevice(h->cfg.device));
    CK(h, cudaStreamSynchronize(h->stream));
    const DevState &d = h->d;
    const int64_t C = d.C, H = d.H;
    int64_t row = 0;
    for (int64_t s = seq_lo; s < seq_hi;) {
        const int64_t slot = s % H;
        const int64_t n = std::min<int64_t>(seq_hi - s, H - slot);
        const size_t rp = (size_t)d.p * C;
        if (theta) CK(h, cudaMemcpy(theta + row * rp, d.h_theta + slot * rp, sizeof(double) * n * rp, cudaMemcpyDeviceToHost));
        if (theta_prop) CK(h, cudaMemcpy(theta_prop + row * rp, d.h_prop + slot * rp, sizeof(double) * n * rp, cudaMemcpyDeviceToHost));
        if (ll) CK(h, cudaMemcpy(ll + row * C, d.h_ll + slot * C, sizeof(double) * n * C, cudaMemcpyDeviceToHost));
        if (ll_prop) CK(h, cudaMemcpy(ll_prop + row * C, d.h_llp + slot * C, sizeof(double) * n * C, cudaMemcpyDeviceToHost));
        if (accepted) CK(h, cudaMemcpy(accepted + row * C, d.h_acc + slot * C, (size_t)n * C, cudaMemcpyDeviceToHost));
        s += n;
        row += n;
    }
    return EXTMCMC_OK;
}

static int32_t copy_ring_rows(extmcmc_t h, void *dst, const void *ring, size_t row_bytes, int64_t lo,
                              int64_t hi, cudaStream_t st) {
    const int64_t H = h->d.H;
    int64_t row = 0;
    for (int64_t s = lo; s < hi;) {
        const int64_t slot = s % H;
        const int64_t n = std::min<int64_t>(hi - s, H - slot);
        CK(h, cudaMemcpyAsync((char *)dst + row * row_bytes, (const char *)ring + slot * row_bytes,
                              (size_t)n * row_bytes, cudaMemcpyDeviceToHost, st));
        s += n;
        row += n;
    }
    return EXTMCMC_OK;
}

int32_t extmcmc_history_fetch_begin(extmcmc_t h, int64_t seq_lo, int64_t seq_hi) {
    if (!h) return EXTMCMC_EINVAL;
    if (h->fetch_active) return fail(h, EXTMCMC_EINVAL, "a history fetch is already outstanding");
    if (seq_lo < 0 || seq_hi < seq_lo || seq_hi > h->seq_next) return fail(h, EXTMCMC_EINVAL, "bad history range");
    if (seq_lo < h->seq_next - h->d.H) return fail(h, EXTMCMC_ESTALE, "history rows already overwritten");
    CK(h, cudaSetDevice(h->cfg.device));
    const DevState &d = h->d;
    const size_t n = (size_t)(seq_hi - seq_lo), C = (size_t)d.C, rp = (size_t)d.p * C * 8;
    const size_t need = n * (2 * rp + 2 * C * 8 + C);
    if (need > h->stage_cap) {
        CK(h, cudaStreamSynchronize(h->copy_stream));
        if (h->stage) cudaFreeHost(h->stage);
        h->stage = nullptr; h->stage_cap = 0;
        CK(h, cudaMallocHost(&h->stage, need));
        h->stage_cap = need;
    }
    CK(h, cudaEventRecord(h->fetch_ready, h->stream));
    CK(h, cudaStreamWaitEvent(h->copy_stream, h->fetch_ready, 0));
    unsigned char *st = h->stage;
    int32_t rc;
    if ((rc = copy_ring_rows(h, st, d.h_theta, rp, seq_lo, seq_hi, h->copy_stream))) return rc;
    if ((rc = copy_ring_rows(h, st + n * rp, d.h_prop, rp, seq_lo, seq_hi, h->copy_stream))) return rc;
    if ((rc = copy_ring_rows(h, st + 2 * n * rp, d.h_ll, C * 8, seq_lo, seq_hi, h->copy_stream))) return rc;
    if ((rc = copy_ring_rows(h, st + 2 * n * rp + n * C * 8, d.h_llp, C * 8, seq_lo, seq_hi, h->copy_stream))) return rc;
    if ((rc = copy_ring_rows(h, st + 2 * n * rp + 2 * n * C * 8, d.h_acc, C, seq_lo, seq_hi, h->copy_stream))) return rc;
    CK(h, cudaEventRecord(h->fetch_done, h->copy_stream));
    h->fetch_lo = seq_lo; h->fetch_hi = seq_hi;
    h->fetch_active = true;
    return EXTMCMC_OK;
}

int32_t extmcmc_history_fetch_end(extmcmc_t h, double *theta, double *theta_prop, double *ll,
                                  double *ll_prop, uint8_t *accepted) {
    if (!h) return EXTMCMC_EINVAL;
    if (!h->fetch_active) return fail(h, EXTMCMC_EINVAL, "no history fetch outstanding");
    CK(h, cudaEventSynchronize(h->fetch_done));
    h->fetch_active = false;
    const DevState &d = h->d;
    const size_t n = (size_t)(h->fetch_hi - h->fetch_lo), C = (size_t)d.C, rp = (size_t)d.p * C * 8;
    const unsigned char *st = h->stage;
    if (theta) std::memcpy(theta, st, n * rp);
    if (theta_prop) std::memcpy(theta_prop, st + n * rp, n * rp);
    if (ll) std::memcpy(ll, st + 2 * n * rp, n * C * 8);
    if (ll_prop) std::memcpy(ll_prop, st + 2 * n * rp + n * C * 8, n * C * 8);
    if (accepted) std::memcpy(accepted, st + 2 * n * rp + 2 * n * C * 8, n * C);
    return EXTMCMC_OK;
}

int32_t extmcmc_get_stats(extmcmc_t h, double *mean, double *cov, double *rolling_ar,
                          int64_t *n_accept, int64_t *n_prop) {
    if (!h) return EXTMCMC_EINVAL;
    CK(h, cudaSetDevice(h->cfg.device));
    CK(h, cudaStreamSynchronize(h->stream));
    const DevState &d = h->d;
    const int64_t C = d.C;
    if (mean) {
        if (d.stats_mode == 2) return fail(h, EXTMCMC_EINVAL, "running moments disabled (stats_mode = 2)");
        CK(h, cudaMemcpy(mean, d.mean, sizeof(double) * d.p * C, cudaMemcpyDeviceToHost));
    }
    if (cov) {
        if (d.stats_mode == 2) return fail(h, EXTMCMC_EINVAL, "running moments disabled (stats_mode = 2)");
        const size_t covn = d.stats_mode == 0 ? (size_t)d.p * d.p : (size_t)d.p;
        CK(h, cudaMemcpy(cov, d.cov, sizeof(double) * covn * C, cudaMemcpyDeviceToHost));
    }
    for (int u = 0; u < h->cfg.n_updates; ++u) {
        if (!h->upd_set[u]) return fail(h, EXTMCMC_EINVAL, "update not set");
        const DevUpdate &t = h->upd_host[u];
        if (rolling_ar) CK(h, cudaMemcpy(rolling_ar + (size_t)u * C, t.ra_val, sizeof(double) * C, cudaMemcpyDeviceToHost));
        if (n_accept) CK(h, cudaMemcpy(n_accept + (size_t)u * C, t.tot_acc, sizeof(int64_t) * C, cudaMemcpyDeviceToHost));
        if (n_prop) CK(h, cudaMemcpy(n_prop + (size_t)u * C, t.tot_prop, sizeof(int64_t) * C, cudaMemcpyDeviceToHost));
    }
    return EXTMCMC_OK;
}

int32_t extmcmc_get_eps(extmcmc_t h, int32_t u, double *eps) {
    if (!h || !eps) return EXTMCMC_EINVAL;
    if (u < 0 || u >= h->cfg.n_updates || !h->upd_set[u]) return fail(h, EXTMCMC_EINVAL, "update not set");
    CK(h, cudaSetDevice(h->cfg.device));
    CK(h, cudaStreamSynchronize(h->stream));
    const DevUpdate &t = h->upd_host[u];
    if (t.kernel == EXTMCMC_KERNEL_RW_UNIFORM)
        CK(h, cudaMemcpy(eps, t.eps, sizeof(double) * t.n_coords * h->d.C, cudaMemcpyDeviceToHost));
    else if (t.kernel == EXTMCMC_KERNEL_MALA)
        CK(h, cudaMemcpy(eps, t.eps, sizeof(double) * h->d.C, cudaMemcpyDeviceToHost));
    else if (t.kernel == EXTMCMC_KERNEL_RW_GAUSS_MIX)
        CK(h, cudaMemcpy(eps, t.sigB, sizeof(double) * t.n_coords * t.n_coords * h->d.C, cudaMemcpyDeviceToHost));
    else
        return fail(h, EXTMCMC_EINVAL, "this transition kernel has no per-chain step-size state");
    return EXTMCMC_OK;
}

int32_t extmcmc_get_adapt_state(extmcmc_t h, int32_t u, double *mean, double *cov) {
    if (!h) return EXTMCMC_EINVAL;
    if (u < 0 || u >= h->cfg.n_updates || !h->upd_set[u]) return fail(h, EXTMCMC_EINVAL, "update not set");
    const DevUpdate &t = h->upd_host[u];
    if (t.adapt_kind != EXTMCMC_ADAPT_HAARIO) return fail(h, EXTMCMC_EINVAL, "update has no Haario adaptation");
    CK(h, cudaSetDevice(h->cfg.device));
    CK(h, cudaStreamSynchronize(h->stream));
    if (mean) CK(h, cudaMemcpy(mean, t.hmean, sizeof(double) * t.n_coords * h->d.C, cudaMemcpyDeviceToHost));
    if (cov) CK(h, cudaMemcpy(cov, t.hcov, sizeof(double) * t.n_coords * t.n_coords * h->d.C, cudaMemcpyDeviceToHost));
    return EXTMCMC_OK;
}

int32_t extmcmc_eval_loglik(extmcmc_t h, double *ll_out) {
    if (!h || !ll_out) return EXTMCMC_EINVAL;
    if (!h->obs_dev || !h->state_set) return fail(h, EXTMCMC_EINVAL, "observations and state required");
    CK(h, cudaSetDevice(h->cfg.device));
    int32_t rc;
    if ((rc = ensure_plan(h))) return rc;
    if ((rc = ensure_total_obs(h))) return rc;
    if (law_self_finished(h->cfg.law)) {
        if ((rc = enqueue_sweep(h, h->cfg.instrument != 0, false, h->d.theta, h->scratch_ll, nullptr))) return rc;
    } else {
        launch_prepare_current(h->d, h->stream);
        if ((rc = enqueue_sweep(h, h->cfg.instrument != 0, false, h->d.theta))) return rc;
        if (!obs_sharded(h) && !h->tail) { launch_reduce_partials(h->d, h->stream); h->launches += 1; }
        launch_finalize_loglik(h->d, h->scratch_ll, h->stream);
        h->launches += 2;
    }
    CK(h, cudaGetLastError());
    CK(h, cudaMemcpyAsync(ll_out, h->scratch_ll, sizeof(double) * h->d.C, cudaMemcpyDeviceToHost, h->stream));
    CK(h, cudaStreamSynchronize(h->stream));
    return EXTMCMC_OK;
}

int32_t extmcmc_eval_grad(extmcmc_t h, double *ll_out, double *grad_out) {
    if (!h || !grad_out) return EXTMCMC_EINVAL;
    if (!h->obs_dev || !h->state_set) return fail(h, EXTMCMC_EINVAL, "observations and state required");
    if ((h->cfg.law != EXTMCMC_LAW_GSN_IID_1D && h->cfg.law != EXTMCMC_LAW_HIER_NORMAL &&
         h->cfg.law != EXTMCMC_LAW_LOGISTIC && h->cfg.law != EXTMCMC_LAW_USER) ||
        (h->cfg.law == EXTMCMC_LAW_USER && h->ulaw.loaded && !h->ulaw.grad))
        return fail(h, EXTMCMC_EUNSUPPORTED, "this law has no device gradient");
    if (obs_sharded(h) && !h->comm) return fail(h, EXTMCMC_EINVAL, "EXTMCMC_SHARD_OBS needs extmcmc_comm_init first");
    CK(h, cudaSetDevice(h->cfg.device));
    int32_t rc;
    if ((rc = ensure_plan(h))) return rc;
    if ((rc = ensure_total_obs(h))) return rc;
    if (law_self_finished(h->cfg.law)) {
        if ((rc = enqueue_sweep(h, h->cfg.instrument != 0, true, h->d.theta, h->scratch_ll, h->d.grad_cur))) return rc;
    } else {
        launch_prepare_current(h->d, h->stream);
        if ((rc = enqueue_sweep(h, h->cfg.instrument != 0, true, h->d.theta))) return rc;
        launch_grad_finalize(grad_view(h), h->d.theta, h->scratch_ll, h->d.grad_cur, h->stream);
        h->launches += 2;
    }
    h->grad_valid = true;
    CK(h, cudaGetLastError());
    if (ll_out) CK(h, cudaMemcpyAsync(ll_out, h->scratch_ll, sizeof(double) * h->d.C, cudaMemcpyDeviceToHost, h->stream));
    CK(h, cudaMemcpyAsync(grad_out, h->d.grad_cur, sizeof(double) * h->d.p * h->d.C, cudaMemcpyDeviceToHost, h->stream));
    CK(h, cudaStreamSynchronize(h->stream));
    return EXTMCMC_OK;
}

int32_t extmcmc_timer_start(extmcmc_t h) {
    if (!h) return EXTMCMC_EINVAL;
    CK(h, cudaEventRecord(h->t0, h->stream));
    return EXTMCMC_OK;
}

int32_t extmcmc_timer_stop(extmcmc_t h, float *ms_out) {
    if (!h || !ms_out) return EXTMCMC_EINVAL;
    CK(h, cudaEventRecord(h->t1, h->stream));
    CK(h, cudaEventSynchronize(h->t1));
    CK(h, cudaEventElapsedTime(ms_out, h->t0, h->t1));
    return EXTMCMC_OK;
}

int32_t extmcmc_event_record(extmcmc_t h, int32_t idx) {
    if (!h) return EXTMCMC_EINVAL;
    if (idx < 0 || idx >= 8192) return fail(h, EXTMCMC_EINVAL, "event index out of range");
    if ((size_t)idx >= h->ev_pool.size()) h->ev_pool.resize((size_t)idx + 1, nullptr);
    if (!h->ev_pool[idx]) CK(h, cudaEventCreate(&h->ev_pool[idx]));
    CK(h, cudaEventRecord(h->ev_pool[idx], h->stream));
    return EXTMCMC_OK;
}

int32_t extmcmc_event_elapsed(extmcmc_t h, int32_t i0, int32_t i1, float *ms_out) {
    if (!h || !ms_out) return EXTMCMC_EINVAL;
    if (i0 < 0 || i1 < 0 || (size_t)i0 >= h->ev_pool.size() || (size_t)i1 >= h->ev_pool.size() ||
        !h->ev_pool[i0] || !h->ev_pool[i1])
        return fail(h, EXTMCMC_EINVAL, "event not recorded");
    CK(h, cudaEventSynchronize(h->ev_pool[i1]));
    CK(h, cudaEventElapsedTime(ms_out, h->ev_pool[i0], h->ev_pool[i1]));
    return EXTMCMC_OK;
}

int32_t extmcmc_get_sweep_time(extmcmc_t h, float *ms_total, int64_t *n_launches) {
    if (!h) return EXTMCMC_EINVAL;
    CK(h, cudaStreamSynchronize(h->stream));
    int32_t rc = collect_events(h);
    if (rc) return rc;
    if (ms_total) *ms_total = h->sweep_ms;
    if (n_launches) *n_launches = h->sweep_launches;
    h->sweep_ms = 0.f;
    h->sweep_launches = 0;
    return EXTMCMC_OK;
}

int64_t extmcmc_launch_count(extmcmc_t h) { return h ? h->launches : 0; }

int32_t extmcmc_flush_l2(extmcmc_t h) {
    if (!h) return EXTMCMC_EINVAL;
    CK(h, cudaSetDevice(h->cfg.device));
    if (!h->flush_buf) {
        h->flush_n = (int64_t)(320ll << 20) / 8;
        CK(h, cudaMalloc(&h->flush_buf, (size_t)h->flush_n * 8));
    }
    launch_flush_l2(h->flush_buf, h->flush_n, h->num_sms, h->stream);
    CK(h, cudaGetLastError());
    return EXTMCMC_OK;
}

int32_t extmcmc_measure_fp64_peak(extmcmc_t h, double *tflops_out) {
    if (!h || !tflops_out) return EXTMCMC_EINVAL;
    CK(h, cudaSetDevice(h->cfg.device));
    const int iters = 16000;
    double best = 0.0;
    for (int rep = 0; rep < 4; ++rep) {
        CK(h, cudaEventRecord(h->t0, h->stream));
        launch_fp64_peak(h->scratch_ll, iters, h->num_sms, h->stream);
        CK(h, cudaEventRecord(h->t1, h->stream));
        CK(h, cudaEventSynchronize(h->t1));
        float ms = 0.f;
        CK(h, cudaEventElapsedTime(&ms, h->t0, h->t1));
        const double flops = (double)h->num_sms * 8 * 256 * 16.0 * iters * 2.0;
        if (rep > 0) best = std::max(best, flops / (ms * 1e-3) / 1e12);
    }
    *tflops_out = best;
    return EXTMCMC_OK;
}

int32_t extmcmc_measure_dmma_peak(extmcmc_t h, double *tflops_out) {
    if (!h || !tflops_out) return EXTMCMC_EINVAL;
    CK(h, cudaSetDevice(h->cfg.device));
    const int iters = 4000;
    double best = 0.0;
    for (int rep = 0; rep < 4; ++rep) {
        CK(h, cudaEventRecord(h->t0, h->stream));
        launch_dmma_peak(h->scratch_ll, iters, h->num_sms, h->stream);
        CK(h, cudaEventRecord(h->t1, h->stream));
        CK(h, cudaEventSynchronize(h->t1));
        float ms = 0.f;
        CK(h, cudaEventElapsedTime(&ms, h->t0, h->t1));
        const double flops = (double)h->num_sms * 8 * 8  * 8.0 * iters * 512.0;
        if (rep > 0) best = std::max(best, flops / (ms * 1e-3) / 1e12);
    }
    *tflops_out = best;
    return EXTMCMC_OK;
}

const char *extmcmc_sweep_variant_name(extmcmc_t h) {
    if (!h) return "";
    if (!h->plan_valid && h->obs_dev) ensure_plan(h);
    if (!h->plan_valid) return "unplanned";
    bool all_set = true;
    for (int u = 0; u < h->cfg.n_updates; ++u) all_set = all_set && h->upd_set[u];
    if (all_set && plan_block_kernels(h) == EXTMCMC_OK) {
        if (h->res_ok) {
            static const char *rn[] = {"", "", "", "", "team_block_R4", "team_block_R5", "team_block_R6", "team_block_R7", "team_block_R8"};
            return rn[h->res_plan.R];
        }
        if (h->obsblk_ok) {
            const int64_t C = h->d.C;
            return C <= 1 ? "obs_block_C1" : C <= 2 ? "obs_block_C2" : C <= 4 ? "obs_block_C4"
                 : C <= 8 ? "obs_block_C8" : C <= 16 ? "obs_block_C16" : "obs_block_C32";
        }
    }
    return h->plan.name;
}

}
```

extensiblemcmc.jl_b200/csrc/step_device.cuh:

```cuda
#pragma once
#include <cmath>
#include <cstdint>
#include <cuda_runtime.h>
#include "dev_state.cuh"
#include "philox.cuh"
#include "exchange.cuh"

namespace extmcmc {

constexpr double kLog2Pi = 1.8378770664093454835606594728112;
constexpr double kLogPi = 1.1447298858494001741434273513531;

struct StrideGet {
    const double *p;
    int64_t stride;
    __device__ __forceinline__ double operator()(int i) const { return p[(int64_t)i * stride]; }
};
struct CoordGet {
    const double *col;
    const int32_t *coords;
    int64_t C;
    __device__ __forceinline__ double operator()(int i) const { return col[(int64_t)coords[i] * C]; }
};
template <class G>
struct OffsetGet {
    G g;
    int off;
    __device__ __forceinline__ double operator()(int i) const { return g(off + i); }
};
struct MatRef {
    double *p;
    int64_t stride;
    __device__ __forceinline__ double get(int idx) const { return p[(int64_t)idx * stride]; }
    __device__ __forceinline__ void set(int idx, double v) const { p[(int64_t)idx * stride] = v; }
};

struct SpecAny {
    static constexpr int kLaw = -1;
    static constexpr bool kLean = false;
};
template <int LAW>
struct SpecLean {
    static constexpr int kLaw = LAW;
    static constexpr bool kLean = true;
};
template <class SP> __device__ __forceinline__ int sp_law(const DevState &d) { return SP::kLaw >= 0 ? SP::kLaw : d.law; }
template <class SP> __device__ __forceinline__ int sp_rw_kernel(const DevUpdate &u) {
    return SP::kLean ? (int)EXTMCMC_KERNEL_RW_UNIFORM : u.kernel;
}

template <bool LEAN = false, class Get>
__device__ __forceinline__ double log_prior_family(int kind, const double *pp, Get get, int n) {
    switch (kind) {
    case EXTMCMC_PRIOR_IMPROPER: return 0.0;
    case EXTMCMC_PRIOR_IMPROPER_POS: {
        double s = 0.0;
        for (int i = 0; i < n; ++i) s += log(get(i));
        return -s;
    }
    case EXTMCMC_PRIOR_NORMAL: {
        const double m = pp[0], sd = pp[1];
        double s = 0.0;
        for (int i = 0; i < n; ++i) {
            const double z = (get(i) - m) / sd;
            s += -(z * z + kLog2Pi) / 2.0 - log(sd);
        }
        return s;
    }
    case EXTMCMC_PRIOR_GAMMA: {
        if (LEAN) break;
        const double k = pp[0], sc = pp[1];
        double s = 0.0;
        for (int i = 0; i < n; ++i) {
            const double x = get(i);
            if (!(x > 0.0)) return -INFINITY;
            s += -lgamma(k) - k * log(sc) + (k - 1.0) * log(x) - x / sc;
        }
        return s;
    }
    case EXTMCMC_PRIOR_UNIFORM: {
        if (LEAN) break;
        const double a = pp[0], b = pp[1];
        double s = 0.0;
        for (int i = 0; i < n; ++i) {
            const double x = get(i);
            if (!(x >= a && x <= b)) return -INFINITY;
            s += -log(b - a);
        }
        return s;
    }
    case EXTMCMC_PRIOR_EXPONENTIAL: {
        if (LEAN) break;
        const double rate = 1.0 / pp[0];
        double s = 0.0;
        for (int i = 0; i < n; ++i) {
            const double x = get(i);
            if (!(x >= 0.0)) return -INFINITY;
            s += log(rate) - rate * x;
        }
        return s;
    }
    case EXTMCMC_PRIOR_INV_GAMMA: {
        if (LEAN) break;
        const double a = pp[0], sc = pp[1];
        double s = 0.0;
        for (int i = 0; i < n; ++i) {
            const double x = get(i);
            if (!(x > 0.0)) return -INFINITY;
            s += a * log(sc) - lgamma(a) - (a + 1.0) * log(x) - sc / x;
        }
        return s;
    }
    case EXTMCMC_PRIOR_BETA: {
        if (LEAN) break;
        const double a = pp[0], b = pp[1];
        const double lbeta = lgamma(a) + lgamma(b) - lgamma(a + b);
        double s = 0.0;
        for (int i = 0; i < n; ++i) {
            const double x = get(i);
            if (!(x > 0.0 && x < 1.0)) return -INFINITY;
            s += (a - 1.0) * log(x) + (b - 1.0) * log1p(-x) - lbeta;
        }
        return s;
    }
    case EXTMCMC_PRIOR_LOGNORMAL: {
        if (LEAN) break;
        const double m = pp[0], sd = pp[1];
        double s = 0.0;
        for (int i = 0; i < n; ++i) {
            const double x = get(i);
            if (!(x > 0.0)) return -INFINITY;
            const double lx = log(x), z = (lx - m) / sd;
            s += (-(z * z + kLog2Pi) / 2.0 - log(sd)) - lx;
        }
        return s;
    }
    case EXTMCMC_PRIOR_CAUCHY: {
        if (LEAN) break;
        const double m = pp[0], sc = pp[1];
        double s = 0.0;
        for (int i = 0; i < n; ++i) {
            const double z = (get(i) - m) / sc;
            s += -(log1p(z * z) + kLogPi + log(sc));
        }
        return s;
    }
    }
    return NAN;
}

template <class MuGet, class XGet>
__device__ __forceinline__ double mvn_logpdf_chol(const MatRef &L, int n, MuGet mu, XGet x, double *zs,
                                                  int64_t zstride) {
    double sq = 0.0, logdet = 0.0;
    for (int r = 0; r < n; ++r) {
        double a = x(r) - mu(r);
        for (int k = 0; k < r; ++k) a -= L.get(r + k * n) * zs[(int64_t)k * zstride];
        const double lrr = L.get(r + r * n);
        const double zr = a / lrr;
        zs[(int64_t)r * zstride] = zr;
        sq += zr * zr;
        logdet += log(lrr);
    }
    return -((double)n * kLog2Pi + 2.0 * logdet) / 2.0 - sq / 2.0;
}

template <class SP = SpecAny, class Get>
__device__ __forceinline__ double log_prior(const DevState &d, const DevUpdate &u, Get get, int64_t c) {
    if (SP::kLean) return log_prior_family<true>(u.prior, u.prior_params, get, u.n_coords);
    if (u.prior == EXTMCMC_PRIOR_MVNORMAL) {
        const int n = u.n_coords;
        const MatRef L{const_cast<double *>(u.prior_dev) + n, 1};
        return mvn_logpdf_chol(L, n, StrideGet{u.prior_dev, 1}, get, d.gw + c, d.C);
    }
    if (u.prior != EXTMCMC_PRIOR_PRODUCT) return log_prior_family(u.prior, u.prior_params, get, u.n_coords);
    const int K = (int)u.prior_params[0];
    double lp = 0.0;
    int off = 0;
    for (int k = 0; k < K; ++k) {
        const double *f = u.prior_params + 1 + 4 * k;
        const int dim = (int)f[1];
        lp += log_prior_family((int)f[0], f + 2, OffsetGet<Get>{get, off}, dim);
        off += dim;
    }
    return lp;
}

template <class EpsGet, class ToGet>
__device__ __forceinline__ double log_q_unif(const DevUpdate &u, EpsGet eps, ToGet to) {
    double s = 0.0;
    for (int i = 0; i < u.n_coords; ++i) {
        const double t = u.pos[i] ? (-log(2.0 * eps(i)) - log(to(i))) : 0.0;
        s = (i == 0) ? t : s + t;
    }
    return s;
}


__device__ __forceinline__ bool chol_lower_sym_upper(const MatRef &S, int n, const MatRef &L) {
    for (int j = 0; j < n; ++j) {
        double s = S.get(j + j * n);
        for (int k = 0; k < j; ++k) { const double l = L.get(j + k * n); s -= l * l; }
        if (!(s > 0.0) || isinf(s)) { L.set(0, NAN); return false; }
        const double ljj = sqrt(s);
        L.set(j + j * n, ljj);
        for (int i = j + 1; i < n; ++i) {
            double a = S.get(j + i * n);
            for (int k = 0; k < j; ++k) a -= L.get(i + k * n) * L.get(j + k * n);
            L.set(i + j * n, a / ljj);
        }
    }
    return true;
}

template <class G>
struct LogPosGet {
    G g;
    const uint8_t *pos;
    __device__ __forceinline__ double operator()(int i) const { const double x = g(i); return pos[i] ? log(x) : x; }
};

template <class FromGet, class ToGet>
__device__ __forceinline__ double log_q_gauss(const DevState &d, const DevUpdate &u, const MatRef &L, FromGet from,
                                              ToGet to, int64_t c) {
    const int n = u.n_coords;
    double s = 0.0;
    for (int i = 0; i < n; ++i) if (u.pos[i]) s += log(to(i));
    const double logJ = -s;
    return mvn_logpdf_chol(L, n, LogPosGet<FromGet>{from, u.pos}, LogPosGet<ToGet>{to, u.pos}, d.gw + c, d.C) + logJ;
}

__device__ __forceinline__ MatRef mat_LA(const DevUpdate &u) { return MatRef{u.LA, 1}; }
__device__ __forceinline__ MatRef mat_LB(const DevUpdate &u, int64_t C, int64_t c) { return MatRef{u.LB + c, C}; }

template <class FromGet, class ToGet>
__device__ __forceinline__ double log_q_gauss_any(const DevState &d, const DevUpdate &u, double lambda, FromGet from,
                                                  ToGet to, int64_t c) {
    const double lpA = log_q_gauss(d, u, mat_LA(u), from, to, c);
    if (u.kernel == EXTMCMC_KERNEL_RW_GAUSS) return lpA;
    const double lpB = log_q_gauss(d, u, mat_LB(u, d.C, c), from, to, c);
    return log((1.0 - lambda) * exp(lpA) + lambda * exp(lpB));
}

template <class SP = SpecAny>
__device__ __forceinline__ void law_prepare(const DevState &d, int64_t c, const double *full,
                                            int64_t stride) {
    const int law = sp_law<SP>(d);
    if (law == EXTMCMC_LAW_GSN_IID_1D) {
        const double mu = full[0], var = full[stride];
        double c0, inv2;
        if (!(var > 0.0) || isinf(var)) {
            c0 = NAN; inv2 = NAN;
            *d.err_flag = 1;
        } else {
            c0 = -(kLog2Pi + 2.0 * log(sqrt(var))) / 2.0;
            inv2 = 0.5 / var;
        }
        d.lawc[c] = mu;
        d.lawc[d.C + c] = c0;
        d.lawc[2 * d.C + c] = inv2;
    } else if (law == EXTMCMC_LAW_HIER_NORMAL) {
        const double tau = full[(int64_t)(d.G + 1) * stride];
        if (!(tau > 0.0) || isinf(tau)) *d.err_flag = 1;
    } else if (law == EXTMCMC_LAW_GSN_MV) {
        const int n = d.obs_dim;
        const int64_t C = d.C;
        double *L = d.mv_L + c;
        double *W = d.lawc + (int64_t)n * C + c;
        bool bad = false;
        for (int j = 0; j < n && !bad; ++j) {
            double s = full[(int64_t)(n + j + j * n) * stride];
            for (int k = 0; k < j; ++k) { const double l = L[(int64_t)(j * n + k) * C]; s -= l * l; }
            if (!(s > 0.0) || isinf(s)) { bad = true; break; }
            const double ljj = sqrt(s);
            L[(int64_t)(j * n + j) * C] = ljj;
            for (int i = j + 1; i < n; ++i) {
                double a = full[(int64_t)(n + j + i * n) * stride];
                for (int k = 0; k < j; ++k) a -= L[(int64_t)(i * n + k) * C] * L[(int64_t)(j * n + k) * C];
                L[(int64_t)(i * n + j) * C] = a / ljj;
            }
        }
        double logdet = 0.0;
        if (!bad) {
            for (int j = 0; j < n; ++j) {
                const double ljj = L[(int64_t)(j * n + j) * C];
                W[(int64_t)(j * (j + 1) / 2 + j) * C] = 1.0 / ljj;
                for (int i = j + 1; i < n; ++i) {
                    double a = 0.0;
                    for (int k = j; k < i; ++k) a -= L[(int64_t)(i * n + k) * C] * W[(int64_t)(k * (k + 1) / 2 + j) * C];
                    W[(int64_t)(i * (i + 1) / 2 + j) * C] = a / L[(int64_t)(i * n + i) * C];
                }
                logdet += log(ljj);
            }
        } else {
            *d.err_flag = 1;
            for (int w = 0; w < n * (n + 1) / 2; ++w) W[(int64_t)w * C] = NAN;
        }
        for (int j = 0; j < n; ++j) d.lawc[(int64_t)j * C + c] = full[(int64_t)j * stride];
        d.lawc[(int64_t)(d.lawc_k - 1) * C + c] = bad ? NAN : -((double)n * kLog2Pi + 2.0 * logdet) / 2.0;
    }
}

template <class SP = SpecAny>
__device__ __forceinline__ double law_finalize(const DevState &d, int64_t c, double S, const double *th) {
    const int law = sp_law<SP>(d);
    if (law_self_finished(law)) return S;
    if (law == EXTMCMC_LAW_GSN_IID_1D)
        return (double)d.n_obs_total * d.lawc[d.C + c] - S * d.lawc[2 * d.C + c];
    if (law == EXTMCMC_LAW_HIER_NORMAL) {
        const int G = d.G;
        const double mu = th[(int64_t)G * d.C], tau = th[(int64_t)(G + 1) * d.C];
        if (!(tau > 0.0) || isinf(tau)) return NAN;
        double dev2 = 0.0;
        for (int g = 0; g < G; ++g) { const double dv = th[(int64_t)g * d.C] - mu; dev2 += dv * dv; }
        return -0.5 * (double)d.n_obs_total * kLog2Pi - S / 2.0 +
               (double)G * (-0.5 * kLog2Pi - log(tau)) - dev2 / (2.0 * tau * tau);
    }
    return (double)d.n_obs_total * d.lawc[(int64_t)(d.lawc_k - 1) * d.C + c] - S / 2.0;
}

struct StepCtx {
    StepDesc sd;
    DevUpdate u;
};
template <class Sync>
__device__ __forceinline__ void load_step_ctx(StepCtx *ctx, const DevState &d, const StepDesc *descs, int k,
                                              int tid, int nthreads, Sync sync) {
    static_assert(sizeof(StepDesc) % 4 == 0 && sizeof(DevUpdate) % 4 == 0, "word copies");
    const uint32_t *src = reinterpret_cast<const uint32_t *>(descs + k);
    uint32_t *dst = reinterpret_cast<uint32_t *>(&ctx->sd);
    for (int i = tid; i < (int)(sizeof(StepDesc) / 4); i += nthreads) dst[i] = src[i];
    sync();
    const uint32_t *us = reinterpret_cast<const uint32_t *>(d.upd + ctx->sd.pidx);
    uint32_t *ud = reinterpret_cast<uint32_t *>(&ctx->u);
    for (int i = tid; i < (int)(sizeof(DevUpdate) / 4); i += nthreads) ud[i] = us[i];
    sync();
}
struct CtaSync { __device__ __forceinline__ void operator()() const { __syncthreads(); } };

template <class SP = SpecAny>
__device__ __forceinline__ void propose_draw(const DevState &d, const StepDesc &sd, const DevUpdate &u, int64_t c) {
    const int kern = sp_rw_kernel<SP>(u);
    const int n = u.n_coords;
    const int64_t C = d.C;
    const CoordGet th{d.theta + c, u.coords, C};
    const StrideGet prop{d.prop_loc + c, C};
    double *pl = d.prop_loc + c;

    uint32_t used = 0;
    if (d.rng_mode == EXTMCMC_RNG_REPLAY) {
        for (int i = 0; i < n; ++i) pl[(int64_t)i * C] = d.rp_prop[((int64_t)sd.replay_row * d.p_u_max + i) * d.gC + d.g0 + c];
    } else {
        ChainStepStream rng(d.seed, (uint64_t)(d.chain_offset + c), sd.mcmciter, sd.pidx);
        for (;;) {
            if (kern == EXTMCMC_KERNEL_RW_UNIFORM) {
                for (int i = 0; i < n; ++i) {
                    const double r = rng.next();
                    const double e = u.eps[(int64_t)i * C + c];
                    const double a = -e, b = e;
                    const double U = a + (b - a) * r;
                    const double t = th(i);
                    pl[(int64_t)i * C] = u.pos[i] ? t * exp(U) : t + U;
                }
            } else {
                bool useB = false;
                if (kern == EXTMCMC_KERNEL_RW_GAUSS_MIX) useB = rng.next() <= sd.lambda;
                double *z = d.gw + c;
                for (int q = 0; q < n; q += 2) {
                    const double u1 = rng.next(), u2 = rng.next();
                    const double rad = sqrt(-2.0 * log(u1));
                    double sn, cs;
                    sincospi(2.0 * u2, &sn, &cs);
                    z[(int64_t)q * C] = rad * cs;
                    if (q + 1 < n) z[(int64_t)(q + 1) * C] = rad * sn;
                }
                const MatRef L = useB ? mat_LB(u, C, c) : mat_LA(u);
                if (isnan(L.get(0))) {
                    *d.err_flag = 1;
                    for (int i = 0; i < n; ++i) pl[(int64_t)i * C] = NAN;
                    break;
                }
                for (int i = 0; i < n; ++i) {
                    const double x = th(i);
                    double t = u.pos[i] ? log(x) : x;
                    double a = 0.0;
                    for (int k = 0; k <= i; ++k) a += L.get(i + k * n) * z[(int64_t)k * C];
                    t = a + t;
                    pl[(int64_t)i * C] = u.pos[i] ? exp(t) : t;
                }
            }
            if (!(log_prior<SP>(d, u, prop, c) == -INFINITY)) break;
            if (rng.j > 60000u) break;
        }
        used = rng.j;
    }
    d.n_used[c] = used;
}

template <class SP = SpecAny>
__device__ __forceinline__ void propose_set(const DevState &d, const DevUpdate &u, int64_t c) {
    const int n = u.n_coords;
    const int64_t C = d.C;
    const double *pl = d.prop_loc + c;
    for (int j0 = 0; j0 < d.p; j0 += 4) {
        double t[4];
#pragma unroll
        for (int q = 0; q < 4; ++q) if (j0 + q < d.p) t[q] = d.theta[(int64_t)(j0 + q) * C + c];
#pragma unroll
        for (int q = 0; q < 4; ++q) if (j0 + q < d.p) d.prop_full[(int64_t)(j0 + q) * C + c] = t[q];
    }
    for (int i = 0; i < n; ++i) d.prop_full[(int64_t)u.coords[i] * C + c] = pl[(int64_t)i * C];
    law_prepare<SP>(d, c, d.prop_full + c, C);
}

template <class SP = SpecAny>
__device__ __forceinline__ void propose_chain(const DevState &d, const StepDesc &sd, const DevUpdate &u, int64_t c) {
    propose_draw<SP>(d, sd, u, c);
    propose_set<SP>(d, u, c);
}

constexpr int kCoopP = 32;
struct CoopStage {
    double *t;
    double *m;
    double *mn;
    int nch, ch;
};

__device__ __forceinline__ void update_cov_coop(const DevState &d, int64_t N, int64_t c0, int nch, const double *sh_t,
                                                const double *sh_m, const double *sh_n, int tid, int nt) {
    const int p = d.p;
    const int64_t C = d.C;
    const double f_old = (double)(N - 1) / (double)N;
    const double f_new = (double)(N + 1) / (double)N;
    if (nt % nch != 0) {
        const int total = nch * p * p;
        for (int i = tid; i < total; i += nt) {
            const int ch = i % nch, e = i / nch;
            if (c0 + ch >= C) continue;
            const int a = e % p, b = e / p;
            const double ta = sh_t[a * nch + ch], tb = sh_t[b * nch + ch];
            const double ma_old = sh_m[a * nch + ch], mb_old = sh_m[b * nch + ch];
            const double ma_new = sh_n[a * nch + ch], mb_new = sh_n[b * nch + ch];
            const double old_sum_sq = f_old * d.cov[(int64_t)e * C + c0 + ch] + ma_old * mb_old;
            const double new_sum_sq = old_sum_sq + (ta * tb) / (double)N;
            d.cov[(int64_t)e * C + c0 + ch] = new_sum_sq - f_new * (ma_new * mb_new);
        }
        return;
    }
    const int ch = tid % nch, es = nt / nch, tri = p * (p + 1) / 2;
    const bool live = c0 + ch < C;
    int e = tid / nch, a = e, b = 0;
    while (a > b) { a -= b + 1; ++b; }
    for (; e < tri; ) {
        double cv[4];
        int ea[4], eb[4], ee[4];
#pragma unroll
        for (int q = 0; q < 4; ++q) {
            ee[q] = e; ea[q] = a; eb[q] = b;
            cv[q] = (e < tri && live) ? d.cov[(int64_t)(a + b * p) * C + c0 + ch] : 0.0;
            e += es; a += es;
            while (a > b) { a -= b + 1; ++b; }
        }
#pragma unroll
        for (int q = 0; q < 4; ++q) {
            if (ee[q] < tri && live) {
                const double ta = sh_t[ea[q] * nch + ch], tb = sh_t[eb[q] * nch + ch];
                const double ma_old = sh_m[ea[q] * nch + ch], mb_old = sh_m[eb[q] * nch + ch];
                const double ma_new = sh_n[ea[q] * nch + ch], mb_new = sh_n[eb[q] * nch + ch];
                const double old_sum_sq = f_old * cv[q] + ma_old * mb_old;
                const double new_sum_sq = old_sum_sq + (ta * tb) / (double)N;
                const double v = new_sum_sq - f_new * (ma_new * mb_new);
                d.cov[(int64_t)(ea[q] + eb[q] * p) * C + c0 + ch] = v;
                if (ea[q] != eb[q]) d.cov[(int64_t)(eb[q] + ea[q] * p) * C + c0 + ch] = v;
            }
        }
    }
}

template <class SP = SpecAny, bool HIST = true, bool MOM = true>
__device__ __forceinline__ void post_decision_moments(const DevState &d, const StepDesc &sd, int64_t c, bool accepted,
                                                      double ll_new, double ll_prop, const CoopStage *cs = nullptr,
                                                      int grp = 0, int n_grp = 1) {
    const int64_t C = d.C;
    if (HIST && grp == 0) d.ll[c] = ll_new;
    const int64_t slot = sd.seq % d.H;
    const int64_t hc = d.g0 + c;
    const int64_t N = sd.stat_n;
    const double f_old = (double)(N - 1) / (double)N;
    const double f_mean = (double)N / (double)(N + 1);
    const double f_new = (double)(N + 1) / (double)N;
    const bool coop_full = MOM && cs && cs->m;
    const bool diag = MOM && d.stats_mode == 1;
    for (int j0 = 4 * grp; j0 < d.p; j0 += 4 * n_grp) {
        double t[4], pr[4], m[4], cv[4];
#pragma unroll
        for (int q = 0; q < 4; ++q)
            if (j0 + q < d.p) {
                t[q] = d.theta[(int64_t)(j0 + q) * C + c];
                if (HIST) pr[q] = d.prop_full[(int64_t)(j0 + q) * C + c];
                if (coop_full || diag) m[q] = d.mean[(int64_t)(j0 + q) * C + c];
                if (diag) cv[q] = d.cov[(int64_t)(j0 + q) * C + c];
            }
#pragma unroll
        for (int q = 0; q < 4; ++q)
            if (j0 + q < d.p) {
                const int j = j0 + q;
                if (HIST) {
                    d.h_theta[(slot * d.p + j) * d.gC + hc] = t[q];
                    d.h_prop[(slot * d.p + j) * d.gC + hc] = pr[q];
                }
                if (MOM && cs) cs->t[j * cs->nch + cs->ch] = t[q];
                if (coop_full || diag) {
                    const double m_new = m[q] * f_mean + t[q] / (double)(N + 1);
                    if (coop_full) { cs->m[j * cs->nch + cs->ch] = m[q]; cs->mn[j * cs->nch + cs->ch] = m_new; }
                    if (diag) {
                        const double old_sum_sq = f_old * cv[q] + m[q] * m[q];
                        const double new_sum_sq = old_sum_sq + (t[q] * t[q]) / (double)N;
                        d.cov[(int64_t)j * C + c] = new_sum_sq - f_new * (m_new * m_new);
                    }
                    d.mean[(int64_t)j * C + c] = m_new;
                }
            }
    }
    if (HIST && grp == 0) {
        d.h_ll[slot * d.gC + hc] = ll_new;
        d.h_llp[slot * d.gC + hc] = ll_prop;
        d.h_acc[slot * d.gC + hc] = accepted ? 1 : 0;
    }

    if (MOM && d.stats_mode == 0 && !coop_full && grp == 0) {
        const int p = d.p;
        for (int b = 0; b < p; ++b) {
            const double tb = d.theta[(int64_t)b * C + c];
            const double mb_old = d.mean[(int64_t)b * C + c];
            const double mb_new = mb_old * f_mean + tb / (double)(N + 1);
            for (int a = 0; a < p; ++a) {
                const double ta = d.theta[(int64_t)a * C + c];
                const double ma_old = d.mean[(int64_t)a * C + c];
                const double ma_new = ma_old * f_mean + ta / (double)(N + 1);
                const int64_t idx = ((int64_t)(a + b * p)) * C + c;
                const double old_sum_sq = f_old * d.cov[idx] + ma_old * mb_old;
                const double new_sum_sq = old_sum_sq + (ta * tb) / (double)N;
                d.cov[idx] = new_sum_sq - f_new * (ma_new * mb_new);
            }
        }
        for (int a = 0; a < p; ++a) {
            const int64_t idx = (int64_t)a * C + c;
            d.mean[idx] = d.mean[idx] * f_mean + d.theta[idx] / (double)(N + 1);
        }
    }
}

template <class SP = SpecAny>
__device__ __forceinline__ void post_decision_counters(const DevState &d, const StepDesc &sd, const DevUpdate &u,
                                                       int64_t c, bool accepted, int n_eps) {
    const int64_t C = d.C;
    const int64_t N = sd.stat_n;
    {
        const int W = d.W;
        const double ra_prev = sd.ra_prev_valid ? u.ra_val[c] : 0.0;
        const int64_t rslot = sd.mcmciter % W;
        const int acc_out = sd.acc_out_valid ? (int)u.acc_ring[rslot * C + c] : 0;
        const int64_t mn = (int64_t)W < N ? (int64_t)W : N;
        u.ra_val[c] = (ra_prev * (double)W + (double)((int)accepted - acc_out)) / (double)mn;
        u.acc_ring[rslot * C + c] = accepted ? 1 : 0;
    }

    u.tot_prop[c] += 1;
    u.tot_acc[c] += accepted ? 1 : 0;
    if (u.adapt_kind == EXTMCMC_ADAPT_UNIF_RW || u.adapt_kind == EXTMCMC_ADAPT_MALA) {
        int32_t prop_n = u.adapt_prop[c] + 1;
        int32_t acc_n = u.adapt_acc[c] + (accepted ? 1 : 0);
        if (prop_n >= u.adapt_every_k) {
            const double r = (double)sd.mcmciter / (double)u.adapt_every_k - u.offset;
            const double delta = u.scale / sqrt(r > 1.0 ? r : 1.0);
            const double a_r = (double)acc_n / (double)prop_n;
            prop_n = 0; acc_n = 0;
            const double sgn = (a_r > u.target) ? 1.0 : -1.0;
            for (int i = 0; i < n_eps; ++i) {
                double e = u.eps[(int64_t)i * C + c] + sgn * delta;
                e = e < u.vmax ? e : u.vmax;
                e = e > u.vmin ? e : u.vmin;
                u.eps[(int64_t)i * C + c] = e;
            }
        }
        u.adapt_prop[c] = prop_n;
        u.adapt_acc[c] = acc_n;
    }
    if (!SP::kLean && d.n_haario > 0) {
        for (int v = 0; v < d.NU; ++v) {
            const DevUpdate &w = (v == sd.pidx) ? u : d.upd[v];
            if (w.adapt_kind != EXTMCMC_ADAPT_HAARIO) continue;
            const int m = w.n_coords;
            double *t = d.gw + (int64_t)d.gw_n * C + c;
            double *om = d.gw + (int64_t)2 * d.gw_n * C + c;
            const int64_t hn = sd.stat_n;
            const double hf_old = (double)(hn - 1) / (double)hn, hf_mean = (double)hn / (double)(hn + 1);
            const double hf_new = (double)(hn + 1) / (double)hn;
            for (int i = 0; i < m; ++i) {
                const double x = d.theta[(int64_t)w.coords[i] * C + c];
                const double ti = w.pos[i] ? log(x) : x;
                const double omi = w.hmean[(int64_t)i * C + c];
                t[(int64_t)i * C] = ti;
                om[(int64_t)i * C] = omi;
                w.hmean[(int64_t)i * C + c] = omi * hf_mean + ti / (double)(hn + 1);
            }
            const bool ready = (v == sd.pidx) && sd.haario_ready;
            for (int b = 0; b < m; ++b)
                for (int a = 0; a < m; ++a) {
                    const int64_t idx = (int64_t)(a + b * m) * C + c;
                    const double old_sum_sq = hf_old * w.hcov[idx] + om[(int64_t)a * C] * om[(int64_t)b * C];
                    const double new_sum_sq = old_sum_sq + (t[(int64_t)a * C] * t[(int64_t)b * C]) / (double)hn;
                    const double cv = new_sum_sq - hf_new * (w.hmean[(int64_t)a * C + c] * w.hmean[(int64_t)b * C + c]);
                    w.hcov[idx] = cv;
                    if (ready) w.sigB[idx] = (2.38 * 2.38) / (double)m * cv;
                }
            if (ready) chol_lower_sym_upper(MatRef{w.sigB + c, C}, m, MatRef{w.LB + c, C});
        }
    }
}

template <class SP = SpecAny>
__device__ __forceinline__ void post_decision(const DevState &d, const StepDesc &sd, const DevUpdate &u,
                                              int64_t c, bool accepted, double ll_new, double ll_prop,
                                              int n_eps, const CoopStage *cs = nullptr) {
    post_decision_moments<SP>(d, sd, c, accepted, ll_new, ll_prop, cs);
    post_decision_counters<SP>(d, sd, u, c, accepted, n_eps);
}

__device__ __forceinline__ double draw_exp(const DevState &d, const StepDesc &sd, int64_t c) {
    if (d.rng_mode == EXTMCMC_RNG_REPLAY) return d.rp_exp[(int64_t)sd.replay_row * d.gC + d.g0 + c];
    ChainStepStream rng(d.seed, (uint64_t)(d.chain_offset + c), sd.mcmciter, sd.pidx, d.n_used[c]);
    return -log(rng.next());
}

struct RwPre {
    double ll_cur, q_back, q_fwd, lp_prop, lp_cur, E;
};

template <class SP = SpecAny>
__device__ __forceinline__ RwPre rw_accept_prologue(const DevState &d, const StepDesc &sd, const DevUpdate &u,
                                                    int64_t c) {
    const int kern = sp_rw_kernel<SP>(u);
    const int64_t C = d.C;
    const CoordGet th{d.theta + c, u.coords, C};
    const StrideGet prop{d.prop_loc + c, C};
    RwPre r;
    r.ll_cur = sd.first ? -INFINITY : d.ll[c];
    if (kern == EXTMCMC_KERNEL_RW_UNIFORM) {
        const StrideGet eps{u.eps + c, C};
        r.q_back = log_q_unif(u, eps, th);
        r.q_fwd = log_q_unif(u, eps, prop);
    } else {
        const bool ok = !isnan(u.LA[0]) && (kern != EXTMCMC_KERNEL_RW_GAUSS_MIX || !isnan(u.LB[c]));
        if (!ok) {
            *d.err_flag = 1;
            r.q_back = NAN;
            r.q_fwd = 0.0;
        } else {
            r.q_back = log_q_gauss_any(d, u, sd.lambda, prop, th, c);
            r.q_fwd = log_q_gauss_any(d, u, sd.lambda, th, prop, c);
        }
    }
    r.lp_prop = log_prior<SP>(d, u, prop, c);
    r.lp_cur = log_prior<SP>(d, u, th, c);
    r.E = draw_exp(d, sd, c);
    return r;
}

struct Decision {
    bool accepted;
    double ll_new, ll_prop;
};
template <class SP = SpecAny>
__device__ __forceinline__ Decision rw_decide_commit(const DevState &d, const DevUpdate &u, int64_t c, const RwPre &r,
                                                     double S) {
    const int64_t C = d.C;
    const int n = u.n_coords;
    const double ll_prop = law_finalize<SP>(d, c, S, d.prop_full + c);
    double llr = ll_prop - r.ll_cur;
    llr = llr + r.q_back;
    llr = llr - r.q_fwd;
    llr = llr + r.lp_prop;
    llr = llr - r.lp_cur;
    const bool accepted = r.E > -llr;
    const double ll_new = accepted ? ll_prop : r.ll_cur;
    if (accepted)
        for (int i = 0; i < n; ++i) d.theta[(int64_t)u.coords[i] * C + c] = d.prop_loc[(int64_t)i * C + c];
    return Decision{accepted, ll_new, ll_prop};
}
template <class SP = SpecAny>
__device__ __forceinline__ int rw_n_eps(const DevUpdate &u) {
    return sp_rw_kernel<SP>(u) == EXTMCMC_KERNEL_RW_UNIFORM ? u.n_coords : 0;
}
template <class SP = SpecAny>
__device__ __forceinline__ bool rw_accept_finish(const DevState &d, const StepDesc &sd, const DevUpdate &u, int64_t c,
                                                 const RwPre &r, double S, const CoopStage *cs = nullptr) {
    const Decision dec = rw_decide_commit<SP>(d, u, c, r, S);
    post_decision<SP>(d, sd, u, c, dec.accepted, dec.ll_new, dec.ll_prop, rw_n_eps<SP>(u), cs);
    return dec.accepted;
}

template <class SP = SpecAny>
__device__ __forceinline__ void grad_finalize_chain(const DevState &d, int64_t c, const double *__restrict__ src,
                                                    double *__restrict__ ll_out, double *__restrict__ grad_out) {
    const int law = sp_law<SP>(d);
    const int64_t C = d.C, PC = d.gC;
    const double *part = d.partial + d.g0 + c;
    const int G = d.G, S = d.S;
    const int64_t rows = (int64_t)G * S;
    if (law == EXTMCMC_LAW_GSN_IID_1D) {
        double s2 = 0.0, s1 = 0.0;
        for (int i = 0; i < S; ++i) { s2 += __ldcg(part + (int64_t)i * PC); s1 += __ldcg(part + (rows + i) * PC); }
        const double var = src[C + c];
        ll_out[c] = law_finalize<SP>(d, c, s2, src + c);
        grad_out[c] = s1 / var;
        grad_out[C + c] = -(double)d.n_obs_total / (2.0 * var) + s2 / (2.0 * var * var);
    } else if (law == EXTMCMC_LAW_HIER_NORMAL) {
        const double mu = src[(int64_t)G * C + c], tau = src[(int64_t)(G + 1) * C + c];
        if (!(tau > 0.0) || isinf(tau)) *d.err_flag = 1;
        const double it2 = 1.0 / (tau * tau);
        double s2_tot = 0.0, dmu = 0.0, dev2 = 0.0;
        for (int g = 0; g < G; ++g) {
            double s2 = 0.0, s1 = 0.0;
            for (int i = 0; i < S; ++i) {
                s2 += __ldcg(part + ((int64_t)g * S + i) * PC);
                s1 += __ldcg(part + (rows + (int64_t)g * S + i) * PC);
            }
            s2_tot += s2;
            const double dv = src[(int64_t)g * C + c] - mu;
            grad_out[(int64_t)g * C + c] = s1 - dv * it2;
            dmu += dv * it2;
            dev2 += dv * dv;
        }
        grad_out[(int64_t)G * C + c] = dmu;
        grad_out[(int64_t)(G + 1) * C + c] = -(double)G / tau + dev2 * it2 / tau;
        ll_out[c] = law_finalize<SP>(d, c, s2_tot, src + c);
    }
}

__device__ __forceinline__ double prior_grad(const DevUpdate &u, double th) {
    if (u.prior == EXTMCMC_PRIOR_NORMAL) return -(th - u.prior_params[0]) / (u.prior_params[1] * u.prior_params[1]);
    return 0.0;
}
__device__ __forceinline__ double prior_logpdf1(const DevUpdate &u, double th) {
    if (u.prior == EXTMCMC_PRIOR_NORMAL) {
        const double z = (th - u.prior_params[0]) / u.prior_params[1];
        return -(z * z + kLog2Pi) / 2.0 - log(u.prior_params[1]);
    }
    return 0.0;
}

template <class SP = SpecAny>
__device__ __forceinline__ void mala_propose_chain(const DevState &d, const StepDesc &sd, const DevUpdate &u, int64_t c) {
    const int64_t C = d.C;
    const int n = u.n_coords;
    const double tau = u.eps[c], h2 = tau * tau / 2.0;
    for (int j0 = 0; j0 < d.p; j0 += 4) {
        double t[4];
#pragma unroll
        for (int q = 0; q < 4; ++q) if (j0 + q < d.p) t[q] = d.theta[(int64_t)(j0 + q) * C + c];
#pragma unroll
        for (int q = 0; q < 4; ++q) if (j0 + q < d.p) d.prop_full[(int64_t)(j0 + q) * C + c] = t[q];
    }
    if (d.rng_mode == EXTMCMC_RNG_REPLAY) {
        for (int i = 0; i < n; ++i)
            d.prop_full[(int64_t)u.coords_dev[i] * C + c] = d.rp_prop[((int64_t)sd.replay_row * d.p_u_max + i) * d.gC + d.g0 + c];
        d.n_used[c] = 0;
    } else {
        ChainStepStream rng(d.seed, (uint64_t)(d.chain_offset + c), sd.mcmciter, sd.pidx);
        for (int i = 0; i < n; i += 2) {
            const double u1 = rng.next(), u2 = rng.next();
            const double rad = sqrt(-2.0 * log(u1));
            double sn, cs;
            sincospi(2.0 * u2, &sn, &cs);
#pragma unroll
            for (int q = 0; q < 2; ++q) {
                if (i + q >= n) break;
                const int64_t j = u.coords_dev[i + q];
                const double th = d.theta[j * C + c];
                const double g = d.grad_cur[j * C + c] + prior_grad(u, th);
                d.prop_full[j * C + c] = th + h2 * g + tau * (rad * (q ? sn : cs));
            }
        }
        d.n_used[c] = rng.j;
    }
    law_prepare<SP>(d, c, d.prop_full + c, C);
}

template <class SP = SpecAny, bool HANDOVER = true>
__device__ __forceinline__ Decision mala_decide_commit(const DevState &d, const StepDesc &sd, const DevUpdate &u, int64_t c) {
    const int64_t C = d.C;
    const int n = u.n_coords;
    const double tau = u.eps[c], h2 = tau * tau / 2.0;
    double qf = 0.0, qb = 0.0, lp_prop = 0.0, lp_cur = 0.0;
    for (int i0 = 0; i0 < n; i0 += 2) {
        double a[2], b[2], ga[2], gb[2];
#pragma unroll
        for (int q = 0; q < 2; ++q)
            if (i0 + q < n) {
                const int64_t j = u.coords_dev[i0 + q];
                a[q] = d.theta[j * C + c];
                b[q] = d.prop_full[j * C + c];
                ga[q] = d.grad_cur[j * C + c];
                gb[q] = d.grad_prop[j * C + c];
            }
#pragma unroll
        for (int q = 0; q < 2; ++q)
            if (i0 + q < n) {
                const double gaq = ga[q] + prior_grad(u, a[q]);
                const double gbq = gb[q] + prior_grad(u, b[q]);
                const double rf = b[q] - a[q] - h2 * gaq, rb = a[q] - b[q] - h2 * gbq;
                qf += rf * rf;
                qb += rb * rb;
                lp_prop += prior_logpdf1(u, b[q]);
                lp_cur += prior_logpdf1(u, a[q]);
            }
    }
    const double inv = 1.0 / (2.0 * tau * tau);
    qf = -qf * inv;
    qb = -qb * inv;
    const double ll_prop = d.ll_prop[c];
    const double ll_cur = sd.first ? -INFINITY : d.ll[c];
    double llr = ll_prop - ll_cur;
    llr = llr + qb;
    llr = llr - qf;
    llr = llr + lp_prop;
    llr = llr - lp_cur;
    const double E = draw_exp(d, sd, c);
    const bool accepted = E > -llr;
    const double ll_new = accepted ? ll_prop : ll_cur;
    if (accepted) {
        for (int i = 0; i < n; ++i) {
            const int64_t j = u.coords_dev[i];
            d.theta[j * C + c] = d.prop_full[j * C + c];
        }
        for (int j0 = 0; HANDOVER && j0 < d.p; j0 += 4) {
            double g[4];
#pragma unroll
            for (int q = 0; q < 4; ++q) if (j0 + q < d.p) g[q] = d.grad_prop[(int64_t)(j0 + q) * C + c];
#pragma unroll
            for (int q = 0; q < 4; ++q) if (j0 + q < d.p) d.grad_cur[(int64_t)(j0 + q) * C + c] = g[q];
        }
        if (HANDOVER && d.dsum_cur) {
            const int rows = 2 * d.G;
            for (int r0 = 0; r0 < rows; r0 += 4) {
                double g[4];
#pragma unroll
                for (int q = 0; q < 4; ++q) if (r0 + q < rows) g[q] = d.dsum_prop[(int64_t)(r0 + q) * C + c];
#pragma unroll
                for (int q = 0; q < 4; ++q) if (r0 + q < rows) d.dsum_cur[(int64_t)(r0 + q) * C + c] = g[q];
            }
        }
    }
    return Decision{accepted, ll_new, ll_prop};
}
__device__ __forceinline__ void mala_handover_coop(const DevState &d, int64_t c0, int nch, const uint8_t *acc,
                                                   int tid, int s0, int ns) {
    const int ch = tid % nch, slice = tid / nch - s0;
    const int64_t C = d.C, c = c0 + ch;
    if (slice < 0 || slice >= ns || c >= C || !acc[ch]) return;
    const int rows = d.p + (d.dsum_cur ? 2 * d.G : 0);
#pragma unroll 2
    for (int r = slice; r < rows; r += ns) {
        if (r < d.p) d.grad_cur[(int64_t)r * C + c] = d.grad_prop[(int64_t)r * C + c];
        else d.dsum_cur[(int64_t)(r - d.p) * C + c] = d.dsum_prop[(int64_t)(r - d.p) * C + c];
    }
}
template <class SP = SpecAny>
__device__ __forceinline__ void mala_decide(const DevState &d, const StepDesc &sd, const DevUpdate &u, int64_t c,
                                            const CoopStage *cs) {
    const Decision dec = mala_decide_commit<SP>(d, sd, u, c);
    post_decision<SP>(d, sd, u, c, dec.accepted, dec.ll_new, dec.ll_prop, 1, cs);
}

}
```

extensiblemcmc.jl_b200/csrc/step_kernels.cu:

```cuda
#include <cmath>
#include <cstdint>
#include <cuda_runtime.h>
#include "dev_state.cuh"
#include "philox.cuh"
#include "step_device.cuh"
#include "step_kernels.h"
#include "tma.cuh"
#include "exchange.cuh"
#include "sweep.h"

namespace extmcmc {

__device__ __forceinline__ bool exchange_failed(const DevState &d) {
    return *reinterpret_cast<volatile int32_t *>(d.err_flag) == 2;
}

template <class SP>
__global__ void __launch_bounds__(256)
propose_kernel(DevState d, const StepDesc *__restrict__ descs, int k) {
    __shared__ StepCtx ctx;
    load_step_ctx(&ctx, d, descs, k, threadIdx.x, blockDim.x, CtaSync{});
    const int64_t c = (int64_t)blockIdx.x * blockDim.x + threadIdx.x;
    if (c >= d.C || exchange_failed(d)) return;
    propose_chain<SP>(d, ctx.sd, ctx.u, c);
}

__global__ void __launch_bounds__(256) prepare_current_kernel(DevState d) {
    const int64_t c = (int64_t)blockIdx.x * blockDim.x + threadIdx.x;
    if (c >= d.C) return;
    law_prepare(d, c, d.theta + c, d.C);
}

__global__ void chol_factor_kernel(double *S, double *L, int n, int64_t stride, int64_t count) {
    const int64_t c = (int64_t)blockIdx.x * blockDim.x + threadIdx.x;
    if (c >= count) return;
    chol_lower_sym_upper(MatRef{S + c, stride}, n, MatRef{L + c, stride});
}

constexpr int kRedThreads = 256;

template <int kRedSlices>
__device__ __forceinline__ double reduce_segments(const DevState &d, double *sh ) {
    constexpr int kRedChains = kRedThreads / kRedSlices;
    const int lane_c = threadIdx.x % kRedChains;
    const int slice = threadIdx.x / kRedChains;
    const int64_t c = (int64_t)blockIdx.x * kRedChains + lane_c;
    double s = 0.0;
    if (c < d.C) {
        const double *p = d.partial + c;
        const int nrows = d.S * d.G;
        int i = slice;
        for (; i + 7 * kRedSlices < nrows; i += 8 * kRedSlices) {
            double a[8];
#pragma unroll
            for (int q = 0; q < 8; ++q) a[q] = p[(int64_t)(i + q * kRedSlices) * d.C];
#pragma unroll
            for (int q = 0; q < 8; ++q) s += a[q];
        }
        for (; i < nrows; i += kRedSlices) s += p[(int64_t)i * d.C];
    }
    if (kRedSlices == 1) return s;
    sh[slice * kRedChains + lane_c] = s;
    __syncthreads();
    double tot = 0.0;
    if (slice == 0) {
#pragma unroll
        for (int j = 0; j < kRedSlices; ++j) tot += sh[j * kRedChains + lane_c];
    }
    return tot;
}

__global__ void __launch_bounds__(256) reduce_group_sums_kernel(DevState d, double *__restrict__ out) {
    const int64_t idx = (int64_t)blockIdx.x * blockDim.x + threadIdx.x;
    const int64_t C = d.C;
    if (idx >= (int64_t)2 * d.G * C) return;
    const int64_t r = idx / C, c = idx % C;
    const double *p = d.partial + (r * d.S) * C + c;
    double s = 0.0;
    int i = 0;
    for (; i + 3 < d.S; i += 4) {
        double a[4];
#pragma unroll
        for (int q = 0; q < 4; ++q) a[q] = p[(int64_t)(i + q) * C];
#pragma unroll
        for (int q = 0; q < 4; ++q) s += a[q];
    }
    for (; i < d.S; ++i) s += p[(int64_t)i * C];
    out[idx] = s;
}

template <int SL>
__global__ void __launch_bounds__(256) reduce_partials_kernel(DevState d) {
    __shared__ double sh[kRedThreads];
    constexpr int kRedChains = kRedThreads / SL;
    const double tot = reduce_segments<SL>(d, sh);
    const int64_t c = (int64_t)blockIdx.x * kRedChains + (threadIdx.x % kRedChains);
    if ((threadIdx.x / kRedChains) == 0 && c < d.C) d.ssum[c] = tot;
}

template <int SL>
__global__ void __launch_bounds__(256)
reduce_push_kernel(DevState d, const StepDesc *__restrict__ descs, int k) {
    __shared__ double sh[kRedThreads];
    constexpr int kRedChains = kRedThreads / SL;
    griddep_launch_dependents();
    const StepDesc sd = descs[k];
    const int parity = (int)(sd.xseq & 1);
    griddep_wait();
    const double tot = reduce_segments<SL>(d, sh);
    const int64_t c = (int64_t)blockIdx.x * kRedChains + (threadIdx.x % kRedChains);
    if ((threadIdx.x / kRedChains) == 0 && c < d.C) {
        const int64_t cell = ll_cell(parity, d.world, d.rank, d.C, c);
        const uint32_t tag = (uint32_t)(sd.xseq + 1);
        for (int q = 0; q < d.world; ++q) ll_store(d.peer_rx[q] + cell, tot, tag);
    }
}

__device__ __forceinline__ double wait_and_combine(const DevState &d, const StepDesc &sd, int64_t c, bool reader, bool &ok) {
    const int parity = (int)(sd.xseq & 1);
    const uint32_t tag = (uint32_t)(sd.xseq + 1);
    double s = 0.0;
    int mine = 1;
    if (reader && c < d.C) {
        const unsigned long long t0 = global_timer_ns();
        for (int r = 0; r < d.world && mine; ++r) {
            double v;
            if (ll_load(d.my_rx + ll_cell(parity, d.world, r, d.C, c), tag, v, t0, d.p2p_timeout_ns)) s += v;
            else { atomicExch(d.err_flag, 2); mine = 0; }
        }
    }
    ok = __syncthreads_and(mine) != 0;
    return s;
}

__global__ void __launch_bounds__(256) finalize_loglik_kernel(DevState d, double *ll_out) {
    const int64_t c = (int64_t)blockIdx.x * blockDim.x + threadIdx.x;
    if (c >= d.C) return;
    ll_out[c] = law_finalize(d, c, d.ssum[c], d.theta + c);
}

constexpr int kFlagConsume = 1, kFlagDefer = 2;
constexpr int kFlagNoSweep = 4;

template <class SP>
__device__ __forceinline__ void run_deferred(const DevState &d, const StepCtx &prev, int64_t c0, int nch, bool stage,
                                             double *sh_t, double *sh_m, double *sh_n) {
    const int tid = threadIdx.x, lane = tid & 31, w = tid >> 5;
    const int64_t c = c0 + (tid % nch);
    const bool lane_ok = lane < nch && c < d.C;
    const bool coop = stage && d.stats_mode == 0;
    const CoopStage cs{sh_t, coop ? sh_m : nullptr, sh_n, nch, tid % nch};
    const bool multi = coop || d.stats_mode != 0;
    const int nw = (int)(blockDim.x >> 5);
    if (w >= 3 && lane_ok && (multi || w == 3)) {
        post_decision_moments<SP, false, true>(d, prev.sd, c, false, 0.0, 0.0, stage ? &cs : nullptr,
                                               multi ? w - 3 : 0, multi ? nw - 3 : 1);
    } else if (w == 2 && lane_ok) {
        const bool acc = d.h_acc[(prev.sd.seq % d.H) * d.gC + d.g0 + c] != 0;
        const int n_eps = prev.u.kernel == EXTMCMC_KERNEL_MALA ? 1 : prev.u.n_coords;
        post_decision_counters<SP>(d, prev.sd, prev.u, c, acc, n_eps);
    }
    if (coop) {
        __syncthreads();
        update_cov_coop(d, prev.sd.stat_n, c0, nch, sh_t, sh_m, sh_n, tid, blockDim.x);
    }
    __syncthreads();
}

template <int SL, class SP>
__global__ void __launch_bounds__(256)
accept_kernel(DevState d, const StepDesc *__restrict__ descs, int k, int fuse_next, int flags) {
    constexpr int kRedChains = kRedThreads / SL;
    __shared__ double sh[kRedThreads];
    __shared__ StepCtx ctx, ctx_next, ctx_prev;
    constexpr int kStage = SL >= 8 ? kCoopP * kRedChains : 1;
    __shared__ double sh_t[kStage], sh_m[kStage], sh_n[kStage];
    griddep_launch_dependents();
    constexpr bool kCanDefer = SL >= 8 && SP::kLean;
    const bool may_defer = kCanDefer && (flags & kFlagDefer), may_consume = kCanDefer && (flags & kFlagConsume);
    load_step_ctx(&ctx, d, descs, k, threadIdx.x, blockDim.x, CtaSync{});
    if (fuse_next == 1 || may_defer) load_step_ctx(&ctx_next, d, descs, k + 1, threadIdx.x, blockDim.x, CtaSync{});
    if (may_consume) load_step_ctx(&ctx_prev, d, descs, k - 1, threadIdx.x, blockDim.x, CtaSync{});
    const int64_t c = (int64_t)blockIdx.x * kRedChains + (threadIdx.x % kRedChains);
    if (flags & kFlagNoSweep) griddep_wait();
    const bool dead = exchange_failed(d);
    const bool worker = (threadIdx.x / kRedChains) == 0 && c < d.C && !dead;
    const StepDesc &sd = ctx.sd;
    const DevUpdate &u = ctx.u;
    const bool stage = SL >= 8 && d.p > 4 && d.p <= kCoopP;
    const bool coop = stage && d.stats_mode == 0;
    RwPre pre{};
    if (worker) pre = rw_accept_prologue<SP>(d, sd, u, c);
    if (may_consume && !dead && ctx_prev.sd.pidx != sd.pidx)
        run_deferred<SP>(d, ctx_prev, (int64_t)blockIdx.x * kRedChains, kRedChains, stage, sh_t, sh_m, sh_n);

    griddep_wait();
    if (dead) return;
    double S;
    if (d.p2p) {
        bool ok;
        S = wait_and_combine(d, ctx.sd, c, (threadIdx.x / kRedChains) == 0 && !dead, ok);
        if (!ok) return;
    } else if (d.use_ssum) {
        S = c < d.C ? d.ssum[c] : 0.0;
    } else {
        S = reduce_segments<SL>(d, sh);
    }
    const CoopStage cs{sh_t, coop ? sh_m : nullptr, sh_n, kRedChains, (int)(threadIdx.x % kRedChains)};
    const bool split = SL >= 8 && SP::kLean && fuse_next == 1 && ctx_next.sd.pidx != sd.pidx;
    const bool defer = may_defer && ctx_next.sd.pidx != sd.pidx;
    if (defer) {
        const bool prop_lane = fuse_next == 1 && (threadIdx.x >> 5) == 1 && (threadIdx.x & 31) < kRedChains && c < d.C;
        Decision dec{};
        if (worker) dec = rw_decide_commit<SP>(d, u, c, pre, S);
        __syncthreads();
        const int wv = threadIdx.x >> 5, n_grp = (int)(blockDim.x >> 5) - 1;
        const bool hist_lane = wv >= 2 && (threadIdx.x & 31) < kRedChains && c < d.C;
        if (worker) post_decision_moments<SP, true, false>(d, sd, c, dec.accepted, dec.ll_new, dec.ll_prop, nullptr, 0, n_grp);
        else if (prop_lane) propose_draw<SP>(d, ctx_next.sd, ctx_next.u, c);
        else if (hist_lane) post_decision_moments<SP, true, false>(d, sd, c, false, 0.0, 0.0, nullptr, wv - 1, n_grp);
        if (fuse_next == 1) {
            __syncthreads();
            if (prop_lane) propose_set<SP>(d, ctx_next.u, c);
        } else if (fuse_next == 2 && worker) {
            law_prepare<SP>(d, c, d.theta + c, d.C);
        }
        return;
    }
    if (split) {
        const bool lane_ok = (threadIdx.x & 31) < kRedChains && c < d.C;
        const bool prop_lane = (threadIdx.x >> 5) == 1 && lane_ok;
        const bool cnt_lane = (threadIdx.x >> 5) == 2 && lane_ok;
        __shared__ uint8_t sh_acc[kRedChains];
        Decision dec{};
        if (worker) {
            dec = rw_decide_commit<SP>(d, u, c, pre, S);
            sh_acc[threadIdx.x % kRedChains] = dec.accepted ? 1 : 0;
        }
        __syncthreads();
        if (worker) post_decision_moments<SP>(d, sd, c, dec.accepted, dec.ll_new, dec.ll_prop, stage ? &cs : nullptr);
        else if (prop_lane) propose_draw<SP>(d, ctx_next.sd, ctx_next.u, c);
        else if (cnt_lane) post_decision_counters<SP>(d, sd, u, c, sh_acc[threadIdx.x % kRedChains] != 0, rw_n_eps<SP>(u));
        __syncthreads();
        if (prop_lane) propose_set<SP>(d, ctx_next.u, c);
        if (coop)
            update_cov_coop(d, sd.stat_n, (int64_t)blockIdx.x * kRedChains, kRedChains, sh_t, sh_m, sh_n, threadIdx.x, blockDim.x);
        return;
    }
    if (worker) rw_accept_finish<SP>(d, sd, u, c, pre, S, stage ? &cs : nullptr);
    if (coop) {
        __syncthreads();
        update_cov_coop(d, sd.stat_n, (int64_t)blockIdx.x * kRedChains, kRedChains, sh_t, sh_m, sh_n, threadIdx.x, blockDim.x);
    }
    if (!worker) return;
    if (fuse_next == 2) law_prepare<SP>(d, c, d.theta + c, d.C);
    else if (fuse_next) propose_chain<SP>(d, ctx_next.sd, ctx_next.u, c);
}

constexpr int kMalaChains = 32, kMalaSlices = 8;
constexpr int kCoopG = 16;
static_assert(kCoopG == kDataCacheMaxG, "the data-sum cache is filled by grad_finalize_coop");
template <class SP>
__device__ __forceinline__ void grad_finalize_coop(const DevState &d, int64_t c0, const double *__restrict__ src,
                                                   double *__restrict__ ll_out, double *__restrict__ grad_out,
                                                   double *sh2, double *sh1 ,
                                                   double *__restrict__ dsum_out = nullptr ) {
    const int ch = threadIdx.x % kMalaChains, slice = threadIdx.x / kMalaChains;
    const int64_t c = c0 + ch, C = d.C;
    const int G = d.G, S = d.S;
    if (sp_law<SP>(d) != EXTMCMC_LAW_HIER_NORMAL || G > kCoopG) {
        if (slice == 0 && c < C) grad_finalize_chain<SP>(d, c, src, ll_out, grad_out);
        return;
    }
    const int64_t rows = (int64_t)G * S;
    if (c < C)
        for (int g = slice; g < G; g += kMalaSlices) {
            const double *p2 = d.partial + ((int64_t)g * S) * C + c;
            const double *p1 = d.partial + (rows + (int64_t)g * S) * C + c;
            double s2 = 0.0, s1 = 0.0;
            int i = 0;
            for (; i + 3 < S; i += 4) {
                double a[4], b[4];
#pragma unroll
                for (int q = 0; q < 4; ++q) { a[q] = p2[(int64_t)(i + q) * C]; b[q] = p1[(int64_t)(i + q) * C]; }
#pragma unroll
                for (int q = 0; q < 4; ++q) { s2 += a[q]; s1 += b[q]; }
            }
            for (; i < S; ++i) { s2 += p2[(int64_t)i * C]; s1 += p1[(int64_t)i * C]; }
            sh2[g * kMalaChains + ch] = s2;
            sh1[g * kMalaChains + ch] = s1;
            if (dsum_out) { dsum_out[(int64_t)g * C + c] = s2; dsum_out[((int64_t)G + g) * C + c] = s1; }
        }
    __syncthreads();
    if (slice != 0 || c >= C) return;
    const double mu = src[(int64_t)G * C + c], tau = src[(int64_t)(G + 1) * C + c];
    if (!(tau > 0.0) || isinf(tau)) *d.err_flag = 1;
    const double it2 = 1.0 / (tau * tau);
    double s2_tot = 0.0, dmu = 0.0, dev2 = 0.0;
    for (int g = 0; g < G; ++g) {
        s2_tot += sh2[g * kMalaChains + ch];
        const double dv = src[(int64_t)g * C + c] - mu;
        grad_out[(int64_t)g * C + c] = sh1[g * kMalaChains + ch] - dv * it2;
        dmu += dv * it2;
        dev2 += dv * dv;
    }
    grad_out[(int64_t)G * C + c] = dmu;
    grad_out[(int64_t)(G + 1) * C + c] = -(double)G / tau + dev2 * it2 / tau;
    ll_out[c] = law_finalize<SP>(d, c, s2_tot, src + c);
}

__global__ void __launch_bounds__(128)
grad_finalize_kernel(DevState d, const double *__restrict__ src, double *__restrict__ ll_out,
                     double *__restrict__ grad_out) {
    const int64_t c = (int64_t)blockIdx.x * blockDim.x + threadIdx.x;
    if (c >= d.C) return;
    grad_finalize_chain(d, c, src, ll_out, grad_out);
}

template <class SP>
__global__ void __launch_bounds__(kMalaChains * kMalaSlices)
mala_propose_kernel(DevState d, const StepDesc *__restrict__ descs, int k, int finalize_cur,
                    double *__restrict__ ll_scratch, int flags) {
    __shared__ StepCtx ctx, ctx_prev;
    __shared__ double sh2[kCoopG * kMalaChains], sh1[kCoopG * kMalaChains];
    __shared__ double sh_t[kCoopP * kMalaChains], sh_m[kCoopP * kMalaChains], sh_n[kCoopP * kMalaChains];
    griddep_launch_dependents();
    load_step_ctx(&ctx, d, descs, k, threadIdx.x, blockDim.x, CtaSync{});
    const int64_t c0 = (int64_t)blockIdx.x * kMalaChains;
    const int64_t c = c0 + threadIdx.x % kMalaChains;
    const bool may_consume = SP::kLean && (flags & kFlagConsume);
    if (may_consume) load_step_ctx(&ctx_prev, d, descs, k - 1, threadIdx.x, blockDim.x, CtaSync{});
    const bool consume = may_consume && ctx_prev.sd.pidx != ctx.sd.pidx;
    const bool behind_sweep = finalize_cur == 1;
    if (consume && behind_sweep) run_deferred<SP>(d, ctx_prev, c0, kMalaChains, d.p <= kCoopP, sh_t, sh_m, sh_n);
    griddep_wait();
    if (consume && !behind_sweep) run_deferred<SP>(d, ctx_prev, c0, kMalaChains, d.p <= kCoopP, sh_t, sh_m, sh_n);
    if (finalize_cur)
        grad_finalize_coop<SP>(d, c0, d.theta, ll_scratch, d.grad_cur, sh2, sh1, behind_sweep ? d.dsum_cur : nullptr);
    if (SP::kLean && d.rng_mode != EXTMCMC_RNG_REPLAY) {
        if (finalize_cur) __syncthreads();
        const int slice = threadIdx.x / kMalaChains;
        const DevUpdate &u = ctx.u;
        const StepDesc &sd = ctx.sd;
        const int n = u.n_coords;
        const int64_t C = d.C;
        const bool live = c < C;
        if (live)
            for (int j = slice; j < d.p; j += kMalaSlices) d.prop_full[(int64_t)j * C + c] = d.theta[(int64_t)j * C + c];
        __syncthreads();
        const double tau = live ? u.eps[c] : 1.0, h2 = tau * tau / 2.0;
        const int n_pairs = (n + 1) / 2;
        if (live)
            for (int q = slice; q < n_pairs; q += kMalaSlices) {
                ChainStepStream rng(d.seed, (uint64_t)(d.chain_offset + c), sd.mcmciter, sd.pidx, (uint32_t)(2 * q));
                const double u1 = rng.next(), u2 = rng.next();
                const double rad = sqrt(-2.0 * log(u1));
                double sn, cs;
                sincospi(2.0 * u2, &sn, &cs);
#pragma unroll
                for (int e = 0; e < 2; ++e) {
                    const int i = 2 * q + e;
                    if (i >= n) break;
                    const int64_t j = u.coords_dev[i];
                    const double th = d.theta[j * C + c];
                    const double g = d.grad_cur[j * C + c] + prior_grad(u, th);
                    d.prop_full[j * C + c] = th + h2 * g + tau * (rad * (e ? sn : cs));
                }
            }
        __syncthreads();
        if (slice != 0 || !live) return;
        d.n_used[c] = (uint32_t)(2 * n_pairs);
        law_prepare<SP>(d, c, d.prop_full + c, C);
        return;
    }
    if (threadIdx.x >= kMalaChains || c >= d.C) return;
    mala_propose_chain<SP>(d, ctx.sd, ctx.u, c);
}

template <class SP>
__global__ void __launch_bounds__(kMalaChains * kMalaSlices)
mala_accept_kernel(DevState d, const StepDesc *__restrict__ descs, int k, int finalize_prop, int fuse_next, int flags) {
    __shared__ StepCtx ctx, ctx_next;
    __shared__ double sh2[kCoopG * kMalaChains], sh1[kCoopG * kMalaChains];
    __shared__ double sh_t[kCoopP * kMalaChains], sh_m[kCoopP * kMalaChains], sh_n[kCoopP * kMalaChains];
    griddep_launch_dependents();
    const bool may_defer = SP::kLean && (flags & kFlagDefer);
    load_step_ctx(&ctx, d, descs, k, threadIdx.x, blockDim.x, CtaSync{});
    if (fuse_next || may_defer) load_step_ctx(&ctx_next, d, descs, k + 1, threadIdx.x, blockDim.x, CtaSync{});
    griddep_wait();
    const int64_t c0 = (int64_t)blockIdx.x * kMalaChains;
    const int ch = threadIdx.x % kMalaChains;
    const int64_t c = c0 + ch;
    if (finalize_prop) grad_finalize_coop<SP>(d, c0, d.prop_full, d.ll_prop, d.grad_prop, sh2, sh1, d.dsum_prop);
    const bool worker = threadIdx.x < kMalaChains && c < d.C;
    const bool stage = d.p <= kCoopP;
    const bool coop = stage && d.stats_mode == 0;
    const CoopStage cs{sh_t, coop ? sh_m : nullptr, sh_n, kMalaChains, ch};
    __shared__ uint8_t sh_acc[kMalaChains];
    if (may_defer && ctx_next.sd.pidx != ctx.sd.pidx) {
        const bool prop_lane = fuse_next && (threadIdx.x >> 5) == 1 && c < d.C;
        Decision dec{};
        if (worker) {
            dec = mala_decide_commit<SP, false>(d, ctx.sd, ctx.u, c);
            sh_acc[ch] = dec.accepted ? 1 : 0;
        }
        __syncthreads();
        const int wv = threadIdx.x >> 5;
        if (worker) post_decision_moments<SP, true, false>(d, ctx.sd, c, dec.accepted, dec.ll_new, dec.ll_prop, nullptr, 0, kMalaSlices - 1);
        else if (prop_lane) propose_draw<SP>(d, ctx_next.sd, ctx_next.u, c);
        else {
            if (wv >= 2 && c < d.C)
                post_decision_moments<SP, true, false>(d, ctx.sd, c, false, 0.0, 0.0, nullptr, wv - 1, kMalaSlices - 1);
            mala_handover_coop(d, c0, kMalaChains, sh_acc, threadIdx.x, 3, kMalaSlices - 3);
        }
        if (fuse_next) {
            __syncthreads();
            if (prop_lane) propose_set<SP>(d, ctx_next.u, c);
        }
        return;
    }
    if (SP::kLean && fuse_next) {
        const bool prop_lane = (threadIdx.x >> 5) == 1 && c < d.C;
        const bool cnt_lane = (threadIdx.x >> 5) == 2 && c < d.C;
        Decision dec{};
        if (worker) {
            dec = mala_decide_commit<SP, false>(d, ctx.sd, ctx.u, c);
            sh_acc[ch] = dec.accepted ? 1 : 0;
        }
        __syncthreads();
        if (worker) post_decision_moments<SP>(d, ctx.sd, c, dec.accepted, dec.ll_new, dec.ll_prop, stage ? &cs : nullptr);
        else if (prop_lane) propose_draw<SP>(d, ctx_next.sd, ctx_next.u, c);
        else if (cnt_lane) post_decision_counters<SP>(d, ctx.sd, ctx.u, c, sh_acc[ch] != 0, 1);
        else mala_handover_coop(d, c0, kMalaChains, sh_acc, threadIdx.x, 3, kMalaSlices - 3);
        __syncthreads();
        if (prop_lane) propose_set<SP>(d, ctx_next.u, c);
        if (coop) update_cov_coop(d, ctx.sd.stat_n, c0, kMalaChains, sh_t, sh_m, sh_n, threadIdx.x, blockDim.x);
        return;
    }
    if (worker) mala_decide<SP>(d, ctx.sd, ctx.u, c, stage ? &cs : nullptr);
    if (coop) {
        __syncthreads();
        update_cov_coop(d, ctx.sd.stat_n, c0, kMalaChains, sh_t, sh_m, sh_n, threadIdx.x, blockDim.x);
    }
    if (worker && fuse_next) propose_chain<SP>(d, ctx_next.sd, ctx_next.u, c);
}

__global__ void generate_obs_normal_kernel(double *obs, int64_t first, int64_t n, double mean,
                                           double sd, uint64_t seed) {
    const int64_t pair0 = first >> 1;
    const int64_t n_pairs = ((first + n + 1) >> 1) - pair0;
    for (int64_t q = (int64_t)blockIdx.x * blockDim.x + threadIdx.x; q < n_pairs;
         q += (int64_t)gridDim.x * blockDim.x) {
        const uint64_t pair = (uint64_t)(pair0 + q);
        const Philox4 w = philox4x32_10((uint32_t)pair, (uint32_t)(pair >> 32), 0x0B5E0B5Eu, 0u,
                                        (uint32_t)seed, (uint32_t)(seed >> 32));
        const double u1 = u52_to_unit(w.w[0], w.w[1]), u2 = u52_to_unit(w.w[2], w.w[3]);
        const double rad = sqrt(-2.0 * log(u1));
        double sn, cs;
        sincospi(2.0 * u2, &sn, &cs);
        const int64_t i0 = (int64_t)(pair << 1), i1 = i0 + 1;
        if (i0 >= first && i0 < first + n) obs[i0 - first] = mean + sd * (rad * cs);
        if (i1 >= first && i1 < first + n) obs[i1 - first] = mean + sd * (rad * sn);
    }
}

__global__ void flush_l2_kernel(double *buf, int64_t n, double v) {
    for (int64_t i = (int64_t)blockIdx.x * blockDim.x + threadIdx.x; i < n;
         i += (int64_t)gridDim.x * blockDim.x)
        buf[i] = v;
}

__global__ void fp64_peak_kernel(double *out, int iters, double a, double b) {
    double acc[16];
#pragma unroll
    for (int i = 0; i < 16; ++i) acc[i] = (double)(threadIdx.x + i);
#pragma unroll 1
    for (int it = 0; it < iters; it += 8) {
#pragma unroll
        for (int q = 0; q < 8; ++q) {
#pragma unroll
            for (int i = 0; i < 16; ++i) acc[i] = fma(acc[i], a, b);
        }
    }
    double s = 0.0;
#pragma unroll
    for (int i = 0; i < 16; ++i) s += acc[i];
    if (s == 123.456) out[0] = s;
}

__global__ void dmma_peak_kernel(double *out, int iters, double a, double b) {
    double c[8][2];
#pragma unroll
    for (int i = 0; i < 8; ++i) { c[i][0] = (double)threadIdx.x; c[i][1] = (double)i; }
    for (int it = 0; it < iters; ++it) {
#pragma unroll
        for (int i = 0; i < 8; ++i)
            asm volatile("mma.sync.aligned.m8n8k4.row.col.f64.f64.f64.f64 {%0,%1}, {%2}, {%3}, {%0,%1};"
                         : "+d"(c[i][0]), "+d"(c[i][1])
                         : "d"(a), "d"(b));
    }
    double s = 0.0;
#pragma unroll
    for (int i = 0; i < 8; ++i) s += c[i][0] + c[i][1];
    if (s == 123.456) out[0] = s;
}

static inline int blocks_for(int64_t C) { return (int)((C + 255) / 256); }

template <class F>
static inline void with_spec(const DevState &d, F f) {
    if (d.lean && d.law == EXTMCMC_LAW_GSN_IID_1D) f(SpecLean<EXTMCMC_LAW_GSN_IID_1D>{});
    else if (d.lean && d.law == EXTMCMC_LAW_HIER_NORMAL) f(SpecLean<EXTMCMC_LAW_HIER_NORMAL>{});
    else if (d.lean && law_self_finished(d.law)) f(SpecLean<EXTMCMC_LAW_LOGISTIC>{});
    else f(SpecAny{});
}
void launch_propose(const DevState &d, const StepDesc *descs, int k, cudaStream_t st) {
    with_spec(d, [&](auto sp) { propose_kernel<decltype(sp)><<<blocks_for(d.C), 256, 0, st>>>(d, descs, k); });
}
static inline int red_blocks_for(int64_t C, int sl) {
    const int ch = kRedThreads / sl;
    return (int)((C + ch - 1) / ch);
}
static inline int slices_for(const DevState &d) {
    const bool stage = d.p > 4 && d.p <= kCoopP;
    if (!stage && (d.use_ssum || d.S * d.G <= 16) && d.C >= 32768) return 1;
    return d.C <= 8 ? 32 : 8;
}
int step_deferral_flags(const DevState &d, int k, int n_steps) {
    static const bool on = [] { const char *e = getenv("EXTMCMC_DEFER"); return !e || atoi(e) != 0; }();
    if (!(on && d.lean && slices_for(d) >= 8)) return 0;
    return (k > 0 ? kFlagConsume : 0) | (k + 1 < n_steps ? kFlagDefer : 0);
}
void launch_accept(const DevState &d0, const StepDesc *descs, int k, int fuse_next, int flags, cudaStream_t st,
                   bool from_cache) {
    DevState d = d0;
    if (from_cache) { d.partial = d0.dsum_cur; d.S = 1; d.use_ssum = 0; d.p2p = 0; flags |= kFlagNoSweep; }
    cudaLaunchConfig_t cfg{};
    cfg.blockDim = dim3(256);
    cfg.stream = st;
    cudaLaunchAttribute attr[1];
    attr[0].id = cudaLaunchAttributeProgrammaticStreamSerialization;
    attr[0].val.programmaticStreamSerializationAllowed = (pdl_mask() >> 1) & 1;
    cfg.attrs = attr;
    cfg.numAttrs = 1;
    const int sl = slices_for(d0);
    cfg.gridDim = dim3(red_blocks_for(d.C, sl));
    with_spec(d, [&](auto sp) {
        using SP = decltype(sp);
        if (sl == 32) cudaLaunchKernelEx(&cfg, accept_kernel<32, SP>, d, descs, k, fuse_next, flags);
        else if (sl == 8) cudaLaunchKernelEx(&cfg, accept_kernel<8, SP>, d, descs, k, fuse_next, flags);
        else cudaLaunchKernelEx(&cfg, accept_kernel<1, SP>, d, descs, k, fuse_next, flags);
    });
}
void launch_grad_finalize(const DevState &d, const double *src, double *ll_out, double *grad_out,
                          cudaStream_t st) {
    grad_finalize_kernel<<<(int)((d.C + 127) / 128), 128, 0, st>>>(d, src, ll_out, grad_out);
}
void launch_mala_propose(const DevState &d, const StepDesc *descs, int k, int finalize_cur, double *ll_scratch,
                         int flags, cudaStream_t st) {
    cudaLaunchConfig_t cfg{};
    cfg.gridDim = dim3((unsigned)((d.C + kMalaChains - 1) / kMalaChains));
    cfg.blockDim = dim3(kMalaChains * kMalaSlices);
    cfg.stream = st;
    cudaLaunchAttribute attr[1];
    attr[0].id = cudaLaunchAttributeProgrammaticStreamSerialization;
    attr[0].val.programmaticStreamSerializationAllowed = (pdl_mask() >> 1) & 1;
    cfg.attrs = attr;
    cfg.numAttrs = 1;
    with_spec(d, [&](auto sp) { cudaLaunchKernelEx(&cfg, mala_propose_kernel<decltype(sp)>, d, descs, k, finalize_cur, ll_scratch, flags); });
}
void launch_mala_accept(const DevState &d, const StepDesc *descs, int k, int finalize_prop, int fuse_next,
                        int flags, cudaStream_t st) {
    cudaLaunchConfig_t cfg{};
    cfg.gridDim = dim3((unsigned)((d.C + kMalaChains - 1) / kMalaChains));
    cfg.blockDim = dim3(kMalaChains * kMalaSlices);
    cfg.stream = st;
    cudaLaunchAttribute attr[1];
    attr[0].id = cudaLaunchAttributeProgrammaticStreamSerialization;
    attr[0].val.programmaticStreamSerializationAllowed = (pdl_mask() >> 1) & 1;
    cfg.attrs = attr;
    cfg.numAttrs = 1;
    with_spec(d, [&](auto sp) { cudaLaunchKernelEx(&cfg, mala_accept_kernel<decltype(sp)>, d, descs, k, finalize_prop, fuse_next, flags); });
}
void launch_chol_factor(double *S, double *L, int n, int64_t stride, int64_t count, cudaStream_t st) {
    chol_factor_kernel<<<(int)((count + 127) / 128), 128, 0, st>>>(S, L, n, stride, count);
}
void launch_prepare_current(const DevState &d, cudaStream_t st) {
    prepare_current_kernel<<<blocks_for(d.C), 256, 0, st>>>(d);
}
void launch_reduce_group_sums(const DevState &d, double *out, cudaStream_t st) {
    const int64_t n = (int64_t)2 * d.G * d.C;
    reduce_group_sums_kernel<<<(int)((n + 255) / 256), 256, 0, st>>>(d, out);
}
void launch_reduce_partials(const DevState &d, cudaStream_t st) {
    if (d.S * d.G > 16)
        reduce_partials_kernel<8><<<red_blocks_for(d.C, 8), 256, 0, st>>>(d);
    else
        reduce_partials_kernel<1><<<red_blocks_for(d.C, 1), 256, 0, st>>>(d);
}
void launch_reduce_push(const DevState &d, const StepDesc *descs, int k, cudaStream_t st) {
    cudaLaunchConfig_t cfg{};
    cfg.blockDim = dim3(256);
    cfg.stream = st;
    cudaLaunchAttribute attr[1];
    attr[0].id = cudaLaunchAttributeProgrammaticStreamSerialization;
    attr[0].val.programmaticStreamSerializationAllowed = (pdl_mask() >> 1) & 1;
    cfg.attrs = attr;
    cfg.numAttrs = 1;
    if (d.S * d.G > 16) {
        cfg.gridDim = dim3(red_blocks_for(d.C, 8));
        cudaLaunchKernelEx(&cfg, reduce_push_kernel<8>, d, descs, k);
    } else {
        cfg.gridDim = dim3(red_blocks_for(d.C, 1));
        cudaLaunchKernelEx(&cfg, reduce_push_kernel<1>, d, descs, k);
    }
}
void launch_finalize_loglik(const DevState &d, double *ll_out, cudaStream_t st) {
    finalize_loglik_kernel<<<blocks_for(d.C), 256, 0, st>>>(d, ll_out);
}
void launch_generate_obs_normal(double *obs, int64_t first, int64_t n, double mean, double sd,
                                uint64_t seed, int num_sms, cudaStream_t st) {
    generate_obs_normal_kernel<<<num_sms * 8, 256, 0, st>>>(obs, first, n, mean, sd, seed);
}
void launch_flush_l2(double *buf, int64_t n, int num_sms, cudaStream_t st) {
    flush_l2_kernel<<<num_sms * 8, 256, 0, st>>>(buf, n, 1.0);
}
void launch_dmma_peak(double *out, int iters, int num_sms, cudaStream_t st) {
    dmma_peak_kernel<<<num_sms * 8, 256, 0, st>>>(out, iters, 1.0000001, 1e-9);
}
void launch_fp64_peak(double *out, int iters, int num_sms, cudaStream_t st) {
    fp64_peak_kernel<<<num_sms * 8, 256, 0, st>>>(out, iters, 1.0000001, 1e-9);
}

}
```

extensiblemcmc.jl_b200/csrc/step_kernels.h:

```cpp
#pragma once
#include <cstdint>
#include <cuda_runtime.h>
#include "dev_state.cuh"

namespace extmcmc {
void launch_propose(const DevState &d, const StepDesc *descs, int k, cudaStream_t st);
int step_deferral_flags(const DevState &d, int k, int n_steps);
void launch_accept(const DevState &d, const StepDesc *descs, int k, int fuse_next, int flags, cudaStream_t st,
                   bool from_cache = false);
void launch_prepare_current(const DevState &d, cudaStream_t st);
void launch_chol_factor(double *S, double *L, int n, int64_t stride, int64_t count, cudaStream_t st);
void launch_grad_finalize(const DevState &d, const double *src, double *ll_out, double *grad_out, cudaStream_t st);
void launch_mala_propose(const DevState &d, const StepDesc *descs, int k, int finalize_cur, double *ll_scratch,
                         int flags, cudaStream_t st);
void launch_mala_accept(const DevState &d, const StepDesc *descs, int k, int finalize_prop, int fuse_next,
                        int flags, cudaStream_t st);
void launch_reduce_partials(const DevState &d, cudaStream_t st);
void launch_reduce_group_sums(const DevState &d, double *out, cudaStream_t st);
void launch_reduce_push(const DevState &d, const StepDesc *descs, int k, cudaStream_t st);
void launch_finalize_loglik(const DevState &d, double *ll_out, cudaStream_t st);
void launch_generate_obs_normal(double *obs, int64_t first, int64_t n, double mean, double sd,
                                uint64_t seed, int num_sms, cudaStream_t st);
void launch_flush_l2(double *buf, int64_t n, int num_sms, cudaStream_t st);
void launch_fp64_peak(double *out, int iters, int num_sms, cudaStream_t st);
void launch_dmma_peak(double *out, int iters, int num_sms, cudaStream_t st);
}
```

Measured before the change: 8524 billion.

## Carry fused next-step proposal across batch boundaries and draw proposals before grid wait

Adds a look-ahead descriptor so the last RW accept kernel of a batch also proposes the first step of the following batch. The next batch then skips its standalone propose kernel, and the scale-validity error check is deferred into the consuming accept. Separately, when the next update touches a single coordinate disjoint from the current one, the proposal draw and the Gaussian constants for both accept and reject outcomes are computed before griddep_wait, overlapping them with the prior kernel's tail. This adds carry-state invalidation across many API entry points and extra descriptor capacity, with some risk of stale carries if any invalidation is missed.

```diff
diff --git a/extensiblemcmc.jl_b200/csrc/api.cu b/extensiblemcmc.jl_b200/csrc/api.cu
--- a/extensiblemcmc.jl_b200/csrc/api.cu
+++ b/extensiblemcmc.jl_b200/csrc/api.cu
@@ -89,6 +89,9 @@
     bool plan_valid = false;
     Slot slot[2];
     int next_slot = 0;
+    bool carry_valid = false;
+    int32_t carry_pidx = 0;
+    int64_t carry_iter = 0;
     std::map<long long, cudaGraphExec_t> graphs;
     std::map<long long, int64_t> graph_launches;
     int64_t seq_next = 0;
@@ -174,6 +177,7 @@
 }
 
 void invalidate_graphs(extmcmc_t h) {
+    h->carry_valid = false;
     for (auto &kv : h->graphs) cudaGraphExecDestroy(kv.second);
     h->graphs.clear();
     h->graph_launches.clear();
@@ -426,14 +430,14 @@
 }
 
 int32_t enqueue_steps(extmcmc_t h, const StepDesc *d_descs, const int *kinds, int n_steps,
-                      bool instrument, bool &grad_valid, bool &dc_valid) {
-    bool fused = false;
+                      bool instrument, bool &grad_valid, bool &dc_valid, bool carry_in, bool look_ahead) {
+    bool fused = carry_in;
     bool cur_prepared = false;
     for (int k = 0; k < n_steps; ++k) {
         int32_t rc;
-        const int dflags = step_deferral_flags(h->d, k, n_steps);
+        int dflags = step_deferral_flags(h->d, k, n_steps);
         const bool next_mala = k + 1 < n_steps && kind_is_mala(kinds[k + 1]);
-        const bool next_rw = k + 1 < n_steps && !kind_is_mala(kinds[k + 1]);
+        const bool next_rw = k + 1 < n_steps ? !kind_is_mala(kinds[k + 1]) : look_ahead;
         const int mode = step_advance(h->dcache, kinds[k], grad_valid, dc_valid);
         if (kind_is_mala(kinds[k])) {
             const bool logi = law_self_finished(h->cfg.law);
@@ -475,6 +479,8 @@
                 if ((rc = enqueue_sweep(h, instrument, false, h->d.prop_full, h->d.ssum, nullptr, d_descs, k))) return rc;
             fused = next_rw;
             cur_prepared = next_mala && !law_self_finished(h->cfg.law) && h->cfg.law != EXTMCMC_LAW_HIER_NORMAL;
+            if (k == 0 && carry_in) dflags |= kStepFlagCarryIn;
+            if (k + 1 == n_steps && look_ahead) dflags |= kStepFlagLookAhead;
             launch_accept(h->d, d_descs, k, fused ? 1 : (cur_prepared ? 2 : 0), dflags, h->stream, from_cache);
             h->launches += 1;
         }
@@ -554,14 +560,14 @@
     Slot &sl = h->slot[si];
     h->next_slot ^= 1;
     if (sl.in_flight) { CK(h, cudaEventSynchronize(sl.done)); sl.in_flight = false; }
-    if (sl.cap < n_steps) {
+    if (sl.cap < n_steps + 1) {
         if (sl.h_descs) cudaFreeHost(sl.h_descs);
         if (sl.d_descs) cudaFree(sl.d_descs);
         for (auto it = h->graphs.begin(); it != h->graphs.end();) {
             if ((it->first & 1) == si) { cudaGraphExecDestroy(it->second); it = h->graphs.erase(it); }
             else ++it;
         }
-        const int cap = std::max(n_steps, 64);
+        const int cap = std::max(n_steps + 1, 64);
         CK(h, cudaMallocHost(&sl.h_descs, sizeof(StepDesc) * cap));
         CK(h, cudaMalloc(&sl.d_descs, sizeof(StepDesc) * cap));
         sl.cap = cap;
@@ -610,6 +616,25 @@
         kinds[s] = step_kind(h, steps[s].pidx);
         hash = (hash ^ (unsigned long long)kinds[s]) * 1099511628211ull;
     }
+    static const bool carry_on = [] { const char *e = getenv("EXTMCMC_CARRY"); return !e || atoi(e) != 0; }();
+    const bool carry_ok = carry_on && rng_mode == EXTMCMC_RNG_PHILOX && !(h->res_ok || h->obsblk_ok) &&
+                          !obs_sharded(h) && step_carry_supported(h->d);
+    const bool carry_in = carry_ok && h->carry_valid && steps[0].pidx == h->carry_pidx &&
+                          steps[0].mcmciter == h->carry_iter;
+    int32_t succ_pidx = steps[n_steps - 1].pidx + 1;
+    int64_t succ_iter = steps[n_steps - 1].mcmciter;
+    if (succ_pidx == h->cfg.n_updates) { succ_pidx = 0; ++succ_iter; }
+    const bool look_ahead = carry_ok && !kind_is_mala(kinds[n_steps - 1]) && !kind_is_mala(step_kind(h, succ_pidx));
+    h->carry_valid = false;
+    if (look_ahead) {
+        StepDesc &sd = sl.h_descs[n_steps];
+        sd = StepDesc{};
+        sd.mcmciter = succ_iter;
+        sd.pidx = succ_pidx;
+        sd.lambda = h->lambda[succ_pidx];
+    }
+    const int n_descs = n_steps + (look_ahead ? 1 : 0);
+    hash = (hash ^ (unsigned long long)((carry_in ? 32 : 0) + (look_ahead ? 64 : 0))) * 1099511628211ull;
     hash = (hash ^ (unsigned long long)((h->grad_valid ? 7 : 3) + (h->dc_valid ? 16 : 0))) * 1099511628211ull;
     hash = (hash ^ (unsigned long long)n_steps) * 1099511628211ull;
     const bool instrument = h->cfg.instrument != 0;
@@ -653,9 +678,11 @@
         h->grad_valid = kind_is_mala(kinds[n_steps - 1]);
         h->dc_valid = false;
     } else if (!use_graph) {
-        CK(h, cudaMemcpyAsync(sl.d_descs, sl.h_descs, sizeof(StepDesc) * n_steps,
+        CK(h, cudaMemcpyAsync(sl.d_descs, sl.h_descs, sizeof(StepDesc) * n_descs,
                               cudaMemcpyHostToDevice, h->stream));
-        if ((rc = enqueue_steps(h, sl.d_descs, kinds.data(), n_steps, instrument, h->grad_valid, h->dc_valid))) return rc;
+        if ((rc = enqueue_steps(h, sl.d_descs, kinds.data(), n_steps, instrument, h->grad_valid, h->dc_valid,
+                                carry_in, look_ahead)))
+            return rc;
     } else {
         const long long key = (long long)((hash << 1) | (unsigned long long)si);
         auto it = h->graphs.find(key);
@@ -664,9 +691,11 @@
             bool gv = h->grad_valid, dc = h->dc_valid;
             cudaGraph_t g = nullptr;
             CK(h, cudaStreamBeginCapture(h->stream, cudaStreamCaptureModeThreadLocal));
-            cudaError_t e1 = cudaMemcpyAsync(sl.d_descs, sl.h_descs, sizeof(StepDesc) * n_steps,
+            cudaError_t e1 = cudaMemcpyAsync(sl.d_descs, sl.h_descs, sizeof(StepDesc) * n_descs,
                                              cudaMemcpyHostToDevice, h->stream);
-            int32_t rc2 = e1 == cudaSuccess ? enqueue_steps(h, sl.d_descs, kinds.data(), n_steps, false, gv, dc) : EXTMCMC_ECUDA;
+            int32_t rc2 = e1 == cudaSuccess ? enqueue_steps(h, sl.d_descs, kinds.data(), n_steps, false, gv, dc,
+                                                            carry_in, look_ahead)
+                                            : EXTMCMC_ECUDA;
             cudaError_t e2 = cudaStreamEndCapture(h->stream, &g);
             h->graph_launches[key] = h->launches - launches_before;
             h->launches = launches_before;
@@ -687,6 +716,9 @@
     }
     CK(h, cudaEventRecord(sl.done, h->stream));
     sl.in_flight = true;
+    h->carry_valid = look_ahead;
+    h->carry_pidx = succ_pidx;
+    h->carry_iter = succ_iter;
     h->seq_next += n_steps;
     h->xseq_next += n_steps;
     return EXTMCMC_OK;
@@ -910,6 +942,7 @@
 int32_t extmcmc_upload_obs(extmcmc_t h, const double *obs, int64_t n_obs, int32_t obs_dim,
                            const double *y) {
     if (!h) return EXTMCMC_EINVAL;
+    h->carry_valid = false;
     if (!obs || n_obs < 1) return fail(h, EXTMCMC_EINVAL, "need at least one observation");
     if (obs_dim != h->cfg.obs_dim) return fail(h, EXTMCMC_EINVAL, "obs_dim differs from the configuration");
     CK(h, cudaSetDevice(h->cfg.device));
@@ -982,6 +1015,7 @@
 int32_t extmcmc_generate_obs_normal(extmcmc_t h, int64_t first, int64_t n_obs, double mean, double sd,
                                     uint64_t seed) {
     if (!h) return EXTMCMC_EINVAL;
+    h->carry_valid = false;
     if (n_obs < 1 || first < 0 || !(sd > 0.0)) return fail(h, EXTMCMC_EINVAL, "bad generate_obs arguments");
     if (h->cfg.law != EXTMCMC_LAW_GSN_IID_1D) return fail(h, EXTMCMC_EUNSUPPORTED, "generate_obs_normal needs the GSN_IID_1D law");
     CK(h, cudaSetDevice(h->cfg.device));
@@ -1009,6 +1043,7 @@
 
 int32_t extmcmc_set_update(extmcmc_t h, int32_t u, const extmcmc_update_t *upd) {
     if (!h || !upd) return EXTMCMC_EINVAL;
+    h->carry_valid = false;
     if (u < 0 || u >= h->cfg.n_updates) return fail(h, EXTMCMC_EINVAL, "update index out of range");
     const bool gauss = upd->kernel == EXTMCMC_KERNEL_RW_GAUSS || upd->kernel == EXTMCMC_KERNEL_RW_GAUSS_MIX;
     const bool mala = upd->kernel == EXTMCMC_KERNEL_MALA;
@@ -1186,6 +1221,7 @@
 
 int32_t extmcmc_set_lambda_fn(extmcmc_t h, int32_t u, extmcmc_lambda_fn f, void *user) {
     if (!h) return EXTMCMC_EINVAL;
+    h->carry_valid = false;
     if (u < 0 || u >= h->cfg.n_updates) return fail(h, EXTMCMC_EINVAL, "update index out of range");
     h->lambda_fn[u] = f;
     h->lambda_user[u] = user;
@@ -1194,6 +1230,7 @@
 
 int32_t extmcmc_set_state(extmcmc_t h, const double *theta) {
     if (!h || !theta) return EXTMCMC_EINVAL;
+    h->carry_valid = false;
     CK(h, cudaSetDevice(h->cfg.device));
     CK(h, cudaStreamSynchronize(h->stream));
     const DevState &d = h->d;
@@ -1355,6 +1392,7 @@
         if (hash != h->ulaw.hash) return fail(h, EXTMCMC_EINVAL, "checkpoint was written under another user law");
         in += sizeof hash;
     }
+    h->carry_valid = false;
     CK(h, cudaSetDevice(h->cfg.device));
     CK(h, cudaStreamSynchronize(h->stream));
     rc = ckpt_walk(h, [&](void *dev, void *host, size_t b) -> int32_t {
@@ -1386,6 +1424,7 @@
 
 int32_t extmcmc_comm_init(extmcmc_t h, const uint8_t id_in[128]) {
     if (!h || !id_in) return EXTMCMC_EINVAL;
+    h->carry_valid = false;
     if (h->comm) return fail(h, EXTMCMC_EINVAL, "communicator already initialised");
     if (!g_nccl.load(h->err)) return EXTMCMC_ENCCL;
     CK(h, cudaSetDevice(h->cfg.device));
@@ -1633,6 +1672,7 @@
 
 int32_t extmcmc_eval_loglik(extmcmc_t h, double *ll_out) {
     if (!h || !ll_out) return EXTMCMC_EINVAL;
+    h->carry_valid = false;
     if (!h->obs_dev || !h->state_set) return fail(h, EXTMCMC_EINVAL, "observations and state required");
     CK(h, cudaSetDevice(h->cfg.device));
     int32_t rc;
@@ -1655,6 +1695,7 @@
 
 int32_t extmcmc_eval_grad(extmcmc_t h, double *ll_out, double *grad_out) {
     if (!h || !grad_out) return EXTMCMC_EINVAL;
+    h->carry_valid = false;
     if (!h->obs_dev || !h->state_set) return fail(h, EXTMCMC_EINVAL, "observations and state required");
     if ((h->cfg.law != EXTMCMC_LAW_GSN_IID_1D && h->cfg.law != EXTMCMC_LAW_HIER_NORMAL &&
          h->cfg.law != EXTMCMC_LAW_LOGISTIC && h->cfg.law != EXTMCMC_LAW_USER) ||
diff --git a/extensiblemcmc.jl_b200/csrc/step_device.cuh b/extensiblemcmc.jl_b200/csrc/step_device.cuh
--- a/extensiblemcmc.jl_b200/csrc/step_device.cuh
+++ b/extensiblemcmc.jl_b200/csrc/step_device.cuh
@@ -242,26 +242,43 @@
     return log((1.0 - lambda) * exp(lpA) + lambda * exp(lpB));
 }
 
+struct Gsn1dConsts {
+    double c0, inv2;
+    bool bad;
+};
+__device__ __forceinline__ Gsn1dConsts gsn1d_consts(double var) {
+    Gsn1dConsts k;
+    k.bad = !(var > 0.0) || isinf(var);
+    if (k.bad) {
+        k.c0 = NAN; k.inv2 = NAN;
+    } else {
+        k.c0 = -(kLog2Pi + 2.0 * log(sqrt(var))) / 2.0;
+        k.inv2 = 0.5 / var;
+    }
+    return k;
+}
+
+template <class SP = SpecAny>
+__device__ __forceinline__ bool law_scale_bad(const DevState &d, const double *full, int64_t stride) {
+    const int law = sp_law<SP>(d);
+    if (law != EXTMCMC_LAW_GSN_IID_1D && law != EXTMCMC_LAW_HIER_NORMAL) return false;
+    const double v = full[(law == EXTMCMC_LAW_GSN_IID_1D ? 1 : (int64_t)(d.G + 1)) * stride];
+    return !(v > 0.0) || isinf(v);
+}
+
 template <class SP = SpecAny>
 __device__ __forceinline__ void law_prepare(const DevState &d, int64_t c, const double *full,
-                                            int64_t stride) {
+                                            int64_t stride, bool raise = true, const Gsn1dConsts *k = nullptr) {
     const int law = sp_law<SP>(d);
     if (law == EXTMCMC_LAW_GSN_IID_1D) {
-        const double mu = full[0], var = full[stride];
-        double c0, inv2;
-        if (!(var > 0.0) || isinf(var)) {
-            c0 = NAN; inv2 = NAN;
-            *d.err_flag = 1;
-        } else {
-            c0 = -(kLog2Pi + 2.0 * log(sqrt(var))) / 2.0;
-            inv2 = 0.5 / var;
-        }
+        const double mu = full[0];
+        const Gsn1dConsts kk = k ? *k : gsn1d_consts(full[stride]);
+        if (kk.bad && raise) *d.err_flag = 1;
         d.lawc[c] = mu;
-        d.lawc[d.C + c] = c0;
-        d.lawc[2 * d.C + c] = inv2;
+        d.lawc[d.C + c] = kk.c0;
+        d.lawc[2 * d.C + c] = kk.inv2;
     } else if (law == EXTMCMC_LAW_HIER_NORMAL) {
-        const double tau = full[(int64_t)(d.G + 1) * stride];
-        if (!(tau > 0.0) || isinf(tau)) *d.err_flag = 1;
+        if (raise && law_scale_bad<SP>(d, full, stride)) *d.err_flag = 1;
     } else if (law == EXTMCMC_LAW_GSN_MV) {
         const int n = d.obs_dim;
         const int64_t C = d.C;
@@ -338,18 +355,28 @@
 }
 struct CtaSync { __device__ __forceinline__ void operator()() const { __syncthreads(); } };
 
-template <class SP = SpecAny>
-__device__ __forceinline__ void propose_draw(const DevState &d, const StepDesc &sd, const DevUpdate &u, int64_t c) {
+struct StrideOut {
+    double *p;
+    int64_t stride;
+    __device__ __forceinline__ void set(int i, double v) const { p[(int64_t)i * stride] = v; }
+    __device__ __forceinline__ double operator()(int i) const { return p[(int64_t)i * stride]; }
+};
+struct OneOut {
+    double *v;
+    __device__ __forceinline__ void set(int, double x) const { *v = x; }
+    __device__ __forceinline__ double operator()(int) const { return *v; }
+};
+template <class SP = SpecAny, class Out>
+__device__ __forceinline__ uint32_t propose_draw_to(const DevState &d, const StepDesc &sd, const DevUpdate &u, int64_t c,
+                                                    Out pl) {
     const int kern = sp_rw_kernel<SP>(u);
     const int n = u.n_coords;
     const int64_t C = d.C;
     const CoordGet th{d.theta + c, u.coords, C};
-    const StrideGet prop{d.prop_loc + c, C};
-    double *pl = d.prop_loc + c;
 
     uint32_t used = 0;
     if (d.rng_mode == EXTMCMC_RNG_REPLAY) {
-        for (int i = 0; i < n; ++i) pl[(int64_t)i * C] = d.rp_prop[((int64_t)sd.replay_row * d.p_u_max + i) * d.gC + d.g0 + c];
+        for (int i = 0; i < n; ++i) pl.set(i, d.rp_prop[((int64_t)sd.replay_row * d.p_u_max + i) * d.gC + d.g0 + c]);
     } else {
         ChainStepStream rng(d.seed, (uint64_t)(d.chain_offset + c), sd.mcmciter, sd.pidx);
         for (;;) {
@@ -360,7 +387,7 @@
                     const double a = -e, b = e;
                     const double U = a + (b - a) * r;
                     const double t = th(i);
-                    pl[(int64_t)i * C] = u.pos[i] ? t * exp(U) : t + U;
+                    pl.set(i, u.pos[i] ? t * exp(U) : t + U);
                 }
             } else {
                 bool useB = false;
@@ -377,7 +404,7 @@
                 const MatRef L = useB ? mat_LB(u, C, c) : mat_LA(u);
                 if (isnan(L.get(0))) {
                     *d.err_flag = 1;
-                    for (int i = 0; i < n; ++i) pl[(int64_t)i * C] = NAN;
+                    for (int i = 0; i < n; ++i) pl.set(i, NAN);
                     break;
                 }
                 for (int i = 0; i < n; ++i) {
@@ -386,19 +413,24 @@
                     double a = 0.0;
                     for (int k = 0; k <= i; ++k) a += L.get(i + k * n) * z[(int64_t)k * C];
                     t = a + t;
-                    pl[(int64_t)i * C] = u.pos[i] ? exp(t) : t;
+                    pl.set(i, u.pos[i] ? exp(t) : t);
                 }
             }
-            if (!(log_prior<SP>(d, u, prop, c) == -INFINITY)) break;
+            if (!(log_prior<SP>(d, u, pl, c) == -INFINITY)) break;
             if (rng.j > 60000u) break;
         }
         used = rng.j;
     }
-    d.n_used[c] = used;
-}
-
-template <class SP = SpecAny>
-__device__ __forceinline__ void propose_set(const DevState &d, const DevUpdate &u, int64_t c) {
+    return used;
+}
+template <class SP = SpecAny>
+__device__ __forceinline__ void propose_draw(const DevState &d, const StepDesc &sd, const DevUpdate &u, int64_t c) {
+    d.n_used[c] = propose_draw_to<SP>(d, sd, u, c, StrideOut{d.prop_loc + c, d.C});
+}
+
+template <class SP = SpecAny>
+__device__ __forceinline__ void propose_set(const DevState &d, const DevUpdate &u, int64_t c, bool raise = true,
+                                            const Gsn1dConsts *k = nullptr) {
     const int n = u.n_coords;
     const int64_t C = d.C;
     const double *pl = d.prop_loc + c;
@@ -410,13 +442,14 @@
         for (int q = 0; q < 4; ++q) if (j0 + q < d.p) d.prop_full[(int64_t)(j0 + q) * C + c] = t[q];
     }
     for (int i = 0; i < n; ++i) d.prop_full[(int64_t)u.coords[i] * C + c] = pl[(int64_t)i * C];
-    law_prepare<SP>(d, c, d.prop_full + c, C);
-}
-
-template <class SP = SpecAny>
-__device__ __forceinline__ void propose_chain(const DevState &d, const StepDesc &sd, const DevUpdate &u, int64_t c) {
+    law_prepare<SP>(d, c, d.prop_full + c, C, raise, k);
+}
+
+template <class SP = SpecAny>
+__device__ __forceinline__ void propose_chain(const DevState &d, const StepDesc &sd, const DevUpdate &u, int64_t c,
+                                              bool raise = true) {
     propose_draw<SP>(d, sd, u, c);
-    propose_set<SP>(d, u, c);
+    propose_set<SP>(d, u, c, raise);
 }
 
 constexpr int kCoopP = 32;
diff --git a/extensiblemcmc.jl_b200/csrc/step_kernels.cu b/extensiblemcmc.jl_b200/csrc/step_kernels.cu
--- a/extensiblemcmc.jl_b200/csrc/step_kernels.cu
+++ b/extensiblemcmc.jl_b200/csrc/step_kernels.cu
@@ -191,8 +191,26 @@
     const bool coop = stage && d.stats_mode == 0;
     RwPre pre{};
     if (worker) pre = rw_accept_prologue<SP>(d, sd, u, c);
+    if (worker && (flags & kStepFlagCarryIn) && law_scale_bad<SP>(d, d.prop_full + c, d.C)) *d.err_flag = 1;
+    const bool raise_next = !(flags & kStepFlagLookAhead);
     if (may_consume && !dead && ctx_prev.sd.pidx != sd.pidx)
         run_deferred<SP>(d, ctx_prev, (int64_t)blockIdx.x * kRedChains, kRedChains, stage, sh_t, sh_m, sh_n);
+    const bool split = SL >= 8 && SP::kLean && fuse_next == 1 && ctx_next.sd.pidx != sd.pidx;
+    const bool prop_lane = split && (threadIdx.x >> 5) == 1 && (threadIdx.x & 31) < kRedChains && c < d.C;
+    bool early = split && d.rng_mode == EXTMCMC_RNG_PHILOX && ctx_next.u.n_coords == 1;
+    for (int i = 0; early && i < u.n_coords; ++i) early = u.coords[i] != ctx_next.u.coords[0];
+    double e_pl = 0.0;
+    uint32_t e_used = 0;
+    Gsn1dConsts e_rej{}, e_acc{};
+    if (early && prop_lane && !dead) {
+        e_used = propose_draw_to<SP>(d, ctx_next.sd, ctx_next.u, c, OneOut{&e_pl});
+        if (sp_law<SP>(d) == EXTMCMC_LAW_GSN_IID_1D) {
+            const bool own = ctx_next.u.coords[0] == 1;
+            e_rej = gsn1d_consts(own ? e_pl : d.theta[d.C + c]);
+            e_acc = gsn1d_consts(own ? e_pl : d.prop_full[d.C + c]);
+        }
+    }
+    __shared__ uint8_t sh_acc[kRedChains];
 
     griddep_wait();
     if (dead) return;
@@ -207,42 +225,53 @@
         S = reduce_segments<SL>(d, sh);
     }
     const CoopStage cs{sh_t, coop ? sh_m : nullptr, sh_n, kRedChains, (int)(threadIdx.x % kRedChains)};
-    const bool split = SL >= 8 && SP::kLean && fuse_next == 1 && ctx_next.sd.pidx != sd.pidx;
+    auto propose_rest = [&](bool second_half) {
+        if (!early) {
+            if (second_half) propose_set<SP>(d, ctx_next.u, c, raise_next);
+            else propose_draw<SP>(d, ctx_next.sd, ctx_next.u, c);
+        } else if (!second_half) {
+            d.prop_loc[c] = e_pl;
+            d.n_used[c] = e_used;
+        } else {
+            const Gsn1dConsts k = sh_acc[threadIdx.x % kRedChains] ? e_acc : e_rej;
+            propose_set<SP>(d, ctx_next.u, c, raise_next, sp_law<SP>(d) == EXTMCMC_LAW_GSN_IID_1D ? &k : nullptr);
+        }
+    };
     const bool defer = may_defer && ctx_next.sd.pidx != sd.pidx;
     if (defer) {
-        const bool prop_lane = fuse_next == 1 && (threadIdx.x >> 5) == 1 && (threadIdx.x & 31) < kRedChains && c < d.C;
-        Decision dec{};
-        if (worker) dec = rw_decide_commit<SP>(d, u, c, pre, S);
-        __syncthreads();
-        const int wv = threadIdx.x >> 5, n_grp = (int)(blockDim.x >> 5) - 1;
-        const bool hist_lane = wv >= 2 && (threadIdx.x & 31) < kRedChains && c < d.C;
-        if (worker) post_decision_moments<SP, true, false>(d, sd, c, dec.accepted, dec.ll_new, dec.ll_prop, nullptr, 0, n_grp);
-        else if (prop_lane) propose_draw<SP>(d, ctx_next.sd, ctx_next.u, c);
-        else if (hist_lane) post_decision_moments<SP, true, false>(d, sd, c, false, 0.0, 0.0, nullptr, wv - 1, n_grp);
-        if (fuse_next == 1) {
-            __syncthreads();
-            if (prop_lane) propose_set<SP>(d, ctx_next.u, c);
-        } else if (fuse_next == 2 && worker) {
-            law_prepare<SP>(d, c, d.theta + c, d.C);
-        }
-        return;
-    }
-    if (split) {
-        const bool lane_ok = (threadIdx.x & 31) < kRedChains && c < d.C;
-        const bool prop_lane = (threadIdx.x >> 5) == 1 && lane_ok;
-        const bool cnt_lane = (threadIdx.x >> 5) == 2 && lane_ok;
-        __shared__ uint8_t sh_acc[kRedChains];
         Decision dec{};
         if (worker) {
             dec = rw_decide_commit<SP>(d, u, c, pre, S);
             sh_acc[threadIdx.x % kRedChains] = dec.accepted ? 1 : 0;
         }
         __syncthreads();
+        const int wv = threadIdx.x >> 5, n_grp = (int)(blockDim.x >> 5) - 1;
+        const bool hist_lane = wv >= 2 && (threadIdx.x & 31) < kRedChains && c < d.C;
+        if (worker) post_decision_moments<SP, true, false>(d, sd, c, dec.accepted, dec.ll_new, dec.ll_prop, nullptr, 0, n_grp);
+        else if (prop_lane) propose_rest(false);
+        else if (hist_lane) post_decision_moments<SP, true, false>(d, sd, c, false, 0.0, 0.0, nullptr, wv - 1, n_grp);
+        if (fuse_next == 1) {
+            __syncthreads();
+            if (prop_lane) propose_rest(true);
+        } else if (fuse_next == 2 && worker) {
+            law_prepare<SP>(d, c, d.theta + c, d.C);
+        }
+        return;
+    }
+    if (split) {
+        const bool lane_ok = (threadIdx.x & 31) < kRedChains && c < d.C;
+        const bool cnt_lane = (threadIdx.x >> 5) == 2 && lane_ok;
+        Decision dec{};
+        if (worker) {
+            dec = rw_decide_commit<SP>(d, u, c, pre, S);
+            sh_acc[threadIdx.x % kRedChains] = dec.accepted ? 1 : 0;
+        }
+        __syncthreads();
         if (worker) post_decision_moments<SP>(d, sd, c, dec.accepted, dec.ll_new, dec.ll_prop, stage ? &cs : nullptr);
-        else if (prop_lane) propose_draw<SP>(d, ctx_next.sd, ctx_next.u, c);
+        else if (prop_lane) propose_rest(false);
         else if (cnt_lane) post_decision_counters<SP>(d, sd, u, c, sh_acc[threadIdx.x % kRedChains] != 0, rw_n_eps<SP>(u));
         __syncthreads();
-        if (prop_lane) propose_set<SP>(d, ctx_next.u, c);
+        if (prop_lane) propose_rest(true);
         if (coop)
             update_cov_coop(d, sd.stat_n, (int64_t)blockIdx.x * kRedChains, kRedChains, sh_t, sh_m, sh_n, threadIdx.x, blockDim.x);
         return;
@@ -254,7 +283,7 @@
     }
     if (!worker) return;
     if (fuse_next == 2) law_prepare<SP>(d, c, d.theta + c, d.C);
-    else if (fuse_next) propose_chain<SP>(d, ctx_next.sd, ctx_next.u, c);
+    else if (fuse_next) propose_chain<SP>(d, ctx_next.sd, ctx_next.u, c, raise_next);
 }
 
 constexpr int kMalaChains = 32, kMalaSlices = 8;
@@ -526,6 +555,11 @@
     if (!stage && (d.use_ssum || d.S * d.G <= 16) && d.C >= 32768) return 1;
     return d.C <= 8 ? 32 : 8;
 }
+bool step_carry_supported(const DevState &d) {
+    bool lean = false;
+    with_spec(d, [&](auto sp) { lean = decltype(sp)::kLean; });
+    return lean;
+}
 int step_deferral_flags(const DevState &d, int k, int n_steps) {
     static const bool on = [] { const char *e = getenv("EXTMCMC_DEFER"); return !e || atoi(e) != 0; }();
     if (!(on && d.lean && slices_for(d) >= 8)) return 0;
diff --git a/extensiblemcmc.jl_b200/csrc/step_kernels.h b/extensiblemcmc.jl_b200/csrc/step_kernels.h
--- a/extensiblemcmc.jl_b200/csrc/step_kernels.h
+++ b/extensiblemcmc.jl_b200/csrc/step_kernels.h
@@ -6,6 +6,8 @@
 namespace extmcmc {
 void launch_propose(const DevState &d, const StepDesc *descs, int k, cudaStream_t st);
 int step_deferral_flags(const DevState &d, int k, int n_steps);
+constexpr int kStepFlagCarryIn = 8, kStepFlagLookAhead = 16;
+bool step_carry_supported(const DevState &d);
 void launch_accept(const DevState &d, const StepDesc *descs, int k, int fuse_next, int flags, cudaStream_t st,
                    bool from_cache = false);
 void launch_prepare_current(const DevState &d, cudaStream_t st);
```

New measurement: 8600 billion, median of 6. About the same (+0.9%).
